# siddC/nbmf_mm

Hardware: AMD Instinct MI355X
Metric: MM-iterations/sec (higher is better)
Workload: dtype f64

## Files before the change

nbmf_mm_amd/csrc/nbmf_hip.hip:

```cpp

#include <hip/hip_runtime.h>
#include <hip/hip_ext.h>

#include <dlfcn.h>
#include <unistd.h>
#include <algorithm>
#include <atomic>
#include <cmath>
#include <cstdarg>
#include <cstdint>
#include <cstdio>
#include <cstdlib>
#include <cstring>
#include <chrono>
#include <condition_variable>
#include <map>
#include <mutex>
#include <string>
#include <type_traits>
#include <vector>

#include "../../include/nbmf_hip.h"

#ifndef NBMF_NO_MFMA
#define NBMF_NO_MFMA 0
#endif
#ifndef NBMF_HAZARD_SEED
#define NBMF_HAZARD_SEED 0
#endif

namespace {

thread_local std::string g_err;
std::atomic<long long> g_engine_persistent_served{0}, g_engine_persistent_aborted{0}, g_engine_persistent_declined{0},
    g_engine_launches_served{0};

int fail(int code, const char* fmt, ...) {
  char buf[1024];
  va_list ap;
  va_start(ap, fmt);
  vsnprintf(buf, sizeof buf, fmt, ap);
  va_end(ap);
  g_err = buf;
  if (code == NBMF_ERR_HIP) (void)hipGetLastError();
  return code;
}

#define HIPCHK(call)                                                                              \
  do {                                                                                            \
    hipError_t e_ = (call);                                                                       \
    if (e_ != hipSuccess)                                                                         \
      return fail(NBMF_ERR_HIP, "%s failed: %s (%s:%d)", #call, hipGetErrorString(e_), __FILE__,  \
                  __LINE__);                                                                      \
  } while (0)

inline int64_t round_up(int64_t x, int64_t a) { return (x + a - 1) / a * a; }

inline bool env_set(const char* name) { return getenv(name) != nullptr; }
template <typename T>
T env_int(const char* name, T dflt) {
  const char* e = getenv(name);
  return e ? (T)atoll(e) : dflt;
}
inline double env_double(const char* name, double dflt) {
  const char* e = getenv(name);
  return e ? atof(e) : dflt;
}

typedef double d4 __attribute__((ext_vector_type(4)));

enum { DATA_BIN = 0, DATA_F64 = 1, DATA_F64M = 2 };
enum { MODE_H = 0, MODE_W = 1, MODE_L = 2, MODE_T = 3 };

enum : unsigned { CB_YM = 1u, CB_ZOBS = 2u, CB_VALID = 4u };

constexpr int SLICE_K = 128;
constexpr int PAD = 128;
constexpr int WG_WAVES = 4;
constexpr size_t PASS_SLACK = 65536;
constexpr int STAGE_BYTES = 32768;

__device__ __forceinline__ double rcp_nr(double d) {
  double r = __builtin_amdgcn_rcp(d);
  const double e = __builtin_fma(-d, r, 1.0);
  const double p = __builtin_fma(e, e, e);
  return __builtin_fma(r, p, r);
}

__device__ __forceinline__ double mk_double(uint32_t lo, uint32_t hi) {
  return __hiloint2double((int)hi, (int)lo);
}

__device__ __forceinline__ double max0(double x) {
  double r;
  __asm__("v_max_f64 %0, %1, 0" : "=v"(r) : "v"(x));
  return r;
}
constexpr int LOG_TABLE_BYTES = 256 * 16;
template <int TB>
__device__ __forceinline__ double2 log_table_entry(int j) {
  const double c = 1.0 / (0.5 + ((double)j + 0.5) * (1.0 / (double)(2 << TB)));
  return double2{c, -log(c)};
}
__device__ __forceinline__ void log_table_fill(double2* tab ) {
  if (threadIdx.x < 256) tab[threadIdx.x] = log_table_entry<8>(threadIdx.x);
}
template <bool GUARD, int TB = 8, bool LDS_ABS = false, typename TAB = const double2*>
__device__ __forceinline__ double log_tab(double x, TAB tab, double c3 = 0.33333333333333331483, double c4 = -0.25) {
  static_assert(TB == 8 || TB == 10, "256 or 1024 entries");
  if (GUARD && __builtin_expect(!__builtin_amdgcn_class(x, 0x100), 0)) return log(x);
  const uint32_t hi = (uint32_t)__double2hiint(x);
  const double m = __builtin_amdgcn_frexp_mant(x);
  const uint32_t off = (hi >> (16 - TB)) & (((1u << TB) - 1u) << 4);
  double2 e;
  if constexpr (LDS_ABS) {
    typedef double d2raw __attribute__((ext_vector_type(2)));
    const d2raw v = *(const __attribute__((address_space(3))) d2raw*)(uintptr_t)(off + (uint32_t)tab);
    e = double2{v[0], v[1]};
  } else {
    e = *(const double2*)((const char*)tab + off);
  }
  const double r = __builtin_fma(m, e.x, -1.0);
  double p;
  if (TB == 8) {
    p = __builtin_fma(r, 0.2, -0.25);
    p = __builtin_fma(r, p, c3);
  } else {
    p = __builtin_fma(r, c4, c3);
  }
  p = __builtin_fma(r, p, -0.5);
  p = __builtin_fma(r, p, 1.0);
  const double k = (double)__builtin_amdgcn_frexp_exp(x);
  return __builtin_fma(r, p, __builtin_fma(k, 0.69314718055994530942, e.y));
}
__global__ __launch_bounds__(256) void log_table_kernel(double2* tab) {
  const int j = blockIdx.x * 256 + threadIdx.x;
  tab[j] = log_table_entry<10>(j);
}

__device__ __forceinline__ double log_of_product(double prod, int pexp) {
  const double m = __builtin_amdgcn_frexp_mant(prod);
  if (__builtin_expect(!(m >= 0.5 && m < 1.0), 0))
    return log(prod) + (double)pexp * 0.6931471805599453094;
  int e = __builtin_amdgcn_frexp_exp(prod) + pexp;
  const bool low = m < 0.70710678118654752440;
  const double m2 = low ? m + m : m;
  e -= low ? 1 : 0;
  const double s = (m2 - 1.0) * rcp_nr(m2 + 1.0);
  const double w = s * s;
  double p = __builtin_fma(w, 1.0 / 19.0, 1.0 / 17.0);
  p = __builtin_fma(w, p, 1.0 / 15.0);
  p = __builtin_fma(w, p, 1.0 / 13.0);
  p = __builtin_fma(w, p, 1.0 / 11.0);
  p = __builtin_fma(w, p, 1.0 / 9.0);
  p = __builtin_fma(w, p, 1.0 / 7.0);
  p = __builtin_fma(w, p, 0.2);
  p = __builtin_fma(w, p, 0.33333333333333331483);
  p = __builtin_fma(w, p, 1.0);
  return __builtin_fma(s + s, p, (double)e * 0.69314718055994530942);
}

typedef unsigned long long lanemask_t;
__device__ __forceinline__ void byte_set4(uint32_t x, lanemask_t (&m)[4]) {
  const uint32_t zero = 0u;
  __asm__("v_cmp_ne_u32_sdwa %0, %4, %5 src0_sel:BYTE_0 src1_sel:DWORD\n\t"
          "v_cmp_ne_u32_sdwa %1, %4, %5 src0_sel:BYTE_1 src1_sel:DWORD\n\t"
          "v_cmp_ne_u32_sdwa %2, %4, %5 src0_sel:BYTE_2 src1_sel:DWORD\n\t"
          "v_cmp_ne_u32_sdwa %3, %4, %5 src0_sel:BYTE_3 src1_sel:DWORD"
          : "=&s"(m[0]), "=&s"(m[1]), "=&s"(m[2]), "=&s"(m[3])
          : "v"(x), "v"(zero));
}
__device__ __forceinline__ void byte_set8(uint32_t x, uint32_t y, lanemask_t (&m)[4], lanemask_t (&n)[4]) {
  const uint32_t zero = 0u;
  __asm__("v_cmp_ne_u32_sdwa %0, %8, %10 src0_sel:BYTE_0 src1_sel:DWORD\n\t"
          "v_cmp_ne_u32_sdwa %1, %8, %10 src0_sel:BYTE_1 src1_sel:DWORD\n\t"
          "v_cmp_ne_u32_sdwa %2, %8, %10 src0_sel:BYTE_2 src1_sel:DWORD\n\t"
          "v_cmp_ne_u32_sdwa %3, %8, %10 src0_sel:BYTE_3 src1_sel:DWORD\n\t"
          "v_cmp_ne_u32_sdwa %4, %9, %10 src0_sel:BYTE_0 src1_sel:DWORD\n\t"
          "v_cmp_ne_u32_sdwa %5, %9, %10 src0_sel:BYTE_1 src1_sel:DWORD\n\t"
          "v_cmp_ne_u32_sdwa %6, %9, %10 src0_sel:BYTE_2 src1_sel:DWORD\n\t"
          "v_cmp_ne_u32_sdwa %7, %9, %10 src0_sel:BYTE_3 src1_sel:DWORD"
          : "=&s"(m[0]), "=&s"(m[1]), "=&s"(m[2]), "=&s"(m[3]), "=&s"(n[0]), "=&s"(n[1]), "=&s"(n[2]), "=&s"(n[3])
          : "v"(x), "v"(y), "v"(zero));
}
__device__ __forceinline__ lanemask_t byte_set(uint32_t x, int byte) {
  lanemask_t m;
  const uint32_t zero = 0u;
  switch (byte) {
    case 0: __asm__("v_cmp_ne_u32_sdwa %0, %1, %2 src0_sel:BYTE_0 src1_sel:DWORD" : "=s"(m) : "v"(x), "v"(zero)); break;
    case 1: __asm__("v_cmp_ne_u32_sdwa %0, %1, %2 src0_sel:BYTE_1 src1_sel:DWORD" : "=s"(m) : "v"(x), "v"(zero)); break;
    case 2: __asm__("v_cmp_ne_u32_sdwa %0, %1, %2 src0_sel:BYTE_2 src1_sel:DWORD" : "=s"(m) : "v"(x), "v"(zero)); break;
    default: __asm__("v_cmp_ne_u32_sdwa %0, %1, %2 src0_sel:BYTE_3 src1_sel:DWORD" : "=s"(m) : "v"(x), "v"(zero)); break;
  }
  return m;
}
__device__ __forceinline__ double sel64(lanemask_t m, double a, double b) { return __builtin_amdgcn_inverse_ballot_w64(m) ? a : b; }
__device__ __forceinline__ double sel64_or0(lanemask_t m, double a) { return __builtin_amdgcn_inverse_ballot_w64(m) ? a : 0.0; }
__device__ __forceinline__ double sel64_0or(lanemask_t m, double b) { return __builtin_amdgcn_inverse_ballot_w64(m) ? 0.0 : b; }
__device__ __forceinline__ double sel64_neg(lanemask_t m, double a, double b) {
  const uint32_t alo = (uint32_t)__double2loint(a), ahi = (uint32_t)__double2hiint(a);
  const uint32_t blo = (uint32_t)__double2loint(b), bhi = (uint32_t)__double2hiint(b);
  uint32_t lo, hi;
  __asm__("v_cndmask_b32_e64 %0, %1, %2, %3" : "=v"(lo) : "v"(blo), "v"(alo), "s"(m));
  __asm__("v_cndmask_b32_e64 %0, -%1, %2, %3" : "=v"(hi) : "v"(bhi), "v"(ahi), "s"(m));
  return mk_double(lo, hi);
}

__device__ __forceinline__ double wave_sum(double v) {
#pragma unroll
  for (int off = 32; off >= 1; off >>= 1) v += __shfl_xor(v, off, 64);
  return v;
}

#include "nbmf_pass_kernel.inc"
#include "nbmf_update_kernels.inc"
#include "nbmf_pack_kernels.inc"
#include "nbmf_peer_kernels.inc"
#include "nbmf_small_kernel.inc"
#include "nbmf_predict_kernels.inc"
#include "nbmf_score_kernels.inc"
#include "nbmf_hist_kernels.inc"
#include "nbmf_rank_kernels.inc"
#include "nbmf_eval_kernels.inc"
#include "nbmf_bits_kernels.inc"
#include "nbmf_theta_bits_kernels.inc"
#include "nbmf_holdout_kernels.inc"

}

struct nbmf_ctx {
  int device = 0;
  int cus = 256;
  hipStream_t stream = nullptr;
  int64_t m = 0, n = 0, mA = 0, nA = 0;
  int k = 0, KP = 0, KB = 0;
  int KS = 1;
  double* theta = nullptr;
  int data_kind = -1;
  int storage = NBMF_STORAGE_AUTO;
  void *dataA = nullptr, *dataB = nullptr, *maskA = nullptr, *maskB = nullptr;
  unsigned long long *bitsA = nullptr, *bitsB = nullptr;
  double n_obs = 0, n_obs_global = 0;
  double* rowcnt = nullptr;
  double *Wn = nullptr, *WT = nullptr, *WG = nullptr, *Hn = nullptr, *HT = nullptr, *HG = nullptr;
  bool have_factors = false;
  bool padB_ones = false;
  bool w_free = false;
  bool factors_in_range = false;
  int chunksH = 0, CH_H = 0, chunksW = 0, CH_W = 0;
  int *cstartH = nullptr, *cstartW = nullptr;
  double *slabH = nullptr, *slabW = nullptr, *Pbuf = nullptr, *lossbuf = nullptr, *prior = nullptr, *scal = nullptr;
  double* lossfin = nullptr;
  int n_prior_blocks = 0;
  int* flags = nullptr;
  double* losses_d = nullptr;
  int losses_cap = 0;
  double* stage = nullptr;
  size_t stage_bytes = 0;
  unsigned long long* stats = nullptr;
  double alpha = 1.2, beta = 1.2, eps = 1e-8;
  int projection = NBMF_PROJ_NORMALIZE;
  void* comm = nullptr;
  nbmf_host_allreduce_fn host_reduce = nullptr;
  void* host_reduce_user = nullptr;
  double* host_buf = nullptr;
  size_t host_buf_count = 0;
  int nranks = 1, rank = 0;
  int shard_axis = 0;
  double n_div_global = 0;
  double* Qbuf = nullptr;
  double* sbuf = nullptr;
  const double* ll_ptr = nullptr;
  int npanel = 1;
  int panels_wanted = 0;
  double peer_timeout_ms = 0;
  long long pc0[3] = {0, 0, 0};
  size_t pbase[2] = {0, 0};
  size_t ll_index = 0;
  int wsplit = 0;
  std::vector<int> bW_host;
  hipStream_t stream2 = nullptr;
  hipEvent_t evH = nullptr, evF = nullptr, ev1 = nullptr;
  const double* prior_src = nullptr;
  int n_prior_src = 0;
  double* arena = nullptr;
  unsigned long long* pflags = nullptr;
  size_t arena_doubles = 0;
  int arena_axis = -1;
  struct ArenaSlotRef { void* p = nullptr; } arena_slot;
  bool peer = false;
  PeerView pv{};
  std::vector<void*> peer_mapped;
  unsigned long long epoch = 0, hseq = 0;
  long long offHX = 0, offPR = 0, offSC = 0, x_doubles = 0;
  long long sl_c0 = 0, sl_wp = 0;
  long long psl_c0[2] = {0, 0}, psl_wp[2] = {0, 0};
  double *Pbuf_own = nullptr, *sbuf_own = nullptr, *Qbuf_own = nullptr;
  struct SmallWs {
    double *Wn = nullptr, *WT = nullptr, *WG = nullptr, *Hn = nullptr, *HT = nullptr, *HG = nullptr;
    double *snapW = nullptr, *snapH = nullptr, *ll_part = nullptr, *prior_part = nullptr;
    unsigned long long* sync = nullptr;
    int* result = nullptr;
    double *part_buf = nullptr, *part_ll = nullptr;
    unsigned long long* part_flag = nullptr;
    char* slab = nullptr;
    bool ready = false, disabled = false;
    int runs = 0, aborted = 0;
  } small;
  struct SmallBatchWs {
    char* slab = nullptr;
    double* table = nullptr;
    double* io = nullptr;
    int cap = 0, losses_cap = 0;
    size_t io_doubles = 0;
    int launches = 0, problems = 0;
  } small_batch;
  nbmf_progress_fn progress = nullptr;
  void* progress_user = nullptr;
  int progress_every = 0;
  struct EvalWs {
    int64_t count = 0;
    int every = 0, patience = 0;
    int *rows = nullptr, *cols = nullptr;
    unsigned char* x = nullptr;
    double *Wk = nullptr, *Hk = nullptr;
    double* partials = nullptr;
    double* eval_ll_d = nullptr;
    int ll_cap = 0;
    double *bestW = nullptr, *bestH = nullptr;
    bool have_best = false;
    std::vector<int> iters;
    std::vector<double> logliks;
    int best_iter = 0, stopped_early = 0;
    bool held_out = false;
  } eval;
  std::atomic<int> cancelled{0};
  bool timing = false;
  int timing_stride = 1;
  int timing_it = 0;
  std::vector<hipEvent_t> ev;
  std::vector<int> ev_kind;
  size_t ev_used = 0;
  double t_ms[2] = {0, 0};
  int t_n[2] = {0, 0};
};

namespace {

struct DevPool {
  std::mutex mu;
  struct Key {
    int device;
    size_t bytes;
    bool operator<(const Key& o) const { return device != o.device ? device < o.device : bytes < o.bytes; }
  };
  std::multimap<Key, void*> free_blocks;
  std::map<void*, Key> live;
  size_t held = 0;
} g_pool;

template <typename T>
hipError_t dmalloc(T** out, size_t bytes) {
  *out = nullptr;
  if (bytes == 0) bytes = 256;
  int dev = 0;
  hipGetDevice(&dev);
  const DevPool::Key key{dev, (bytes + 255) / 256 * 256};
  {
    std::lock_guard<std::mutex> lk(g_pool.mu);
    auto it = g_pool.free_blocks.find(key);
    if (it != g_pool.free_blocks.end()) {
      *out = (T*)it->second;
      g_pool.held -= key.bytes;
      g_pool.free_blocks.erase(it);
      g_pool.live[(void*)*out] = key;
      return hipSuccess;
    }
  }
  void* p = nullptr;
  hipError_t e = hipMalloc(&p, key.bytes);
  if (e != hipSuccess) {
    (void)hipGetLastError();
// ... 531 lines not shown
    }
  }
  c->ev_used = 0;
}

int all_reduce_inplace(nbmf_ctx* c, double* p, size_t count, hipStream_t st = nullptr) {
  if (c->comm) {
    NCCLCHK(g_rccl.AllReduce(p, p, count, kNcclFloat64, kNcclSum, c->comm, st ? st : c->stream));
  } else if (c->peer) {
    const long long off = p - c->arena;
    if (off < 0 || (size_t)off + count > c->arena_doubles) return fail(NBMF_ERR_STATE, "internal: peer exchange outside the arena");
    hipStream_t s = st ? st : c->stream;
    const unsigned long long e = ++c->epoch;
    const long long slice = ((long long)count + c->pv.nranks - 1) / c->pv.nranks;
    const unsigned grid = (unsigned)std::min<long long>(128, std::max<long long>(1, (slice + 1023) / 1024));
    static const bool fault = env_int("NBMF_PEER_FAULT", 0) != 0;
    if (!(fault && c->pv.nranks > 1 && c->pv.rank == c->pv.nranks - 1))
      hipLaunchKernelGGL(peer_reduce_kernel, dim3(grid), dim3(256), 0, s, c->pv, e, off, (long long)count, c->flags);
    HIPCHK(hipGetLastError());
    hipLaunchKernelGGL(peer_wait_kernel, dim3(1), dim3(64), 0, s, c->pv, e, c->flags);
    HIPCHK(hipGetLastError());
  } else if (c->host_reduce) {
    if (count > c->host_buf_count) return fail(NBMF_ERR_STATE, "internal: host exchange buffer too small");
    HIPCHK(hipMemcpyAsync(c->host_buf, p, count * sizeof(double), hipMemcpyDeviceToHost, c->stream));
    HIPCHK(hipStreamSynchronize(c->stream));
    if (c->host_reduce(c->host_reduce_user, c->host_buf, (int64_t)count) != 0)
      return fail(NBMF_ERR_COMM, "host all-reduce callback failed");
    HIPCHK(hipMemcpyAsync(p, c->host_buf, count * sizeof(double), hipMemcpyHostToDevice, c->stream));
  }
  return NBMF_OK;
}

inline bool is_sharded(const nbmf_ctx* c) { return c->comm || c->host_reduce || c->peer; }

inline const void* sweep_image(const nbmf_ctx* c, int image) {
  if (c->data_kind == DATA_BIN) return image == 0 ? (const void*)c->bitsA : (const void*)c->bitsB;
  return image == 0 ? c->dataA : c->dataB;
}

inline int wg_strips(const nbmf_ctx*) { return WG_WAVES; }

int tiny_a(const nbmf_ctx* c) {
  return c->eps < 1e-70 || !(c->eps >= 1e-12 && c->factors_in_range) || (c->data_kind == DATA_BIN && !(c->eps < 0x1p-22));
}
double pform_inv12(const nbmf_ctx* c) {
  if (c->data_kind != DATA_BIN || c->KS != 1 || tiny_a(c)) return 0.0;
  return 1.0 / ((1.0 + c->eps) + c->eps);
}

double ll_pad_of(const nbmf_ctx* c, int strict = 0) {
  if (strict) return 0.0;
  const double n_pad = (double)c->mA * (double)c->nA - (double)c->m * (double)c->n;
  return n_pad * log(1.0 + c->eps);
}

int enqueue_exchange_after_sweep(nbmf_ctx* c, const PassArgs& a, bool with_products, int strict) {
  const int n_loss = c->chunksH * (a.Cb / wg_strips(c));
  const double pad = ll_pad_of(c, strict);
  if (!is_sharded(c)) {
    c->ll_ptr = nullptr;
    return NBMF_OK;
  }
  if (c->shard_axis == 0 && with_products)
    return fail(NBMF_ERR_STATE, "internal: the row-split H-step exchange is driven by enqueue_iteration_rows");
  hipLaunchKernelGGL(ll_reduce_kernel, dim3(1), dim3(256), 0, c->stream, (const double*)c->lossbuf, n_loss, pad, c->sbuf,
                     c->flags);
  HIPCHK(hipGetLastError());
  size_t cnt = 1;
  if (c->shard_axis == 1) {
    hipLaunchKernelGGL(prior_reduce_kernel, dim3(1), dim3(256), 0, c->stream, (const double*)c->prior, c->n_prior_blocks,
                       c->sbuf + 1, c->flags);
    HIPCHK(hipGetLastError());
    cnt = 3;
  }
  if (int rc = all_reduce_inplace(c, c->sbuf, cnt)) return rc;
  c->ll_ptr = c->sbuf;
  return NBMF_OK;
}

PassArgs h_pass_args(nbmf_ctx* c) {
  PassArgs a{};
  a.data = sweep_image(c, 0);
  a.mask = c->maskA;
  a.LT = c->WT;
  a.LG = c->WG;
  a.RfT = c->HT;
  a.out1 = c->slabH;
  a.out2 = c->slabH + (size_t)c->chunksH * c->KP * c->nA;
  a.lossbuf = c->lossbuf;
  a.done = c->flags;
  a.Rb = (int)(c->mA / 16);
  a.Cb = (int)(c->nA / 16);
  a.chunk_start = c->cstartH;
  a.C_alloc = c->nA;
  a.eps = c->eps;
  a.tiny_eps = tiny_a(c);
  a.ksteps = (c->k + 3) / 4;
  a.kblocks = (c->k + 15) / 16;
  return a;
}
PassArgs w_pass_args(nbmf_ctx* c) {
  PassArgs a{};
  a.data = sweep_image(c, 1);
  a.mask = c->maskB;
  a.LT = c->HT;
  a.LG = c->HG;
  a.RfT = c->WT;
  a.out1 = c->slabW;
  a.out2 = nullptr;
  a.lossbuf = nullptr;
  a.done = c->flags;
  a.Rb = (int)(c->nA / 16);
  a.Cb = (int)(c->mA / 16);
  a.chunk_start = c->cstartW;
  a.C_alloc = c->mA;
  a.eps = c->eps;
  a.tiny_eps = tiny_a(c) || c->w_free;
  a.full = c->data_kind == DATA_BIN && c->n_obs == (double)c->m * (double)c->n && (c->nA == c->n || c->padB_ones);
  a.ksteps = (c->k + 3) / 4;
  a.kblocks = (c->k + 15) / 16;
  return a;
}

void at_slice(const nbmf_ctx* c, PassArgs& a, int image, int sl) {
  const size_t offW = (size_t)sl * SLICE_K * c->mA, offH = (size_t)sl * SLICE_K * c->nA;
  a.LT = image == 0 ? c->WT + offW : c->HT + offH;
  a.LG = image == 0 ? c->WG + offW : c->HG + offH;
  a.RfT = image == 0 ? c->HT + offH : c->WT + offW;
  const size_t slab_off = image == 0 ? (size_t)c->chunksH * offH : (size_t)c->chunksW * offW;
  if (a.out1) a.out1 += slab_off;
  if (a.out2) a.out2 += slab_off;
}

int enqueue_theta(nbmf_ctx* c, int image) {
  for (int sl = 0; sl < c->KS - 1; ++sl) {
    PassArgs a{};
    at_slice(c, a, image, sl);
    a.theta = c->theta;
    a.accum = sl > 0;
    a.done = c->flags;
    a.Rb = (int)((image == 0 ? c->mA : c->nA) / 16);
    a.Cb = (int)((image == 0 ? c->nA : c->mA) / 16);
    a.chunk_start = image == 0 ? c->cstartH : c->cstartW;
    a.C_alloc = image == 0 ? c->nA : c->mA;
    a.eps = c->eps;
    a.tiny_eps = c->eps < 1e-70;
    HIPCHK(launch_theta(a, image == 0 ? c->chunksH : c->chunksW, c->stream));
  }
  return NBMF_OK;
}

int enqueue_a_sweeps_sliced(nbmf_ctx* c, bool with_products, int strict, int clip) {
  if (int rc = enqueue_theta(c, 0)) return rc;
  const int last = c->KS - 1;
  for (int step = 0; step < (with_products ? c->KS : 1); ++step) {
    const int sl = step == 0 ? last : step - 1;
    PassArgs a = h_pass_args(c);
    at_slice(c, a, 0, sl);
    if (step != 0) a.lossbuf = nullptr;
    a.strict = strict;
    a.clip = clip;
    a.theta = c->theta;
    hipError_t e;
    if (with_products)
      e = step == 0 ? launch_pass_slice<MODE_H, 2>(c->data_kind, a, c->chunksH, c->stream)
                    : launch_pass_slice<MODE_H, 1>(c->data_kind, a, c->chunksH, c->stream);
    else
      e = launch_pass_slice<MODE_L, 2>(c->data_kind, a, c->chunksH, c->stream);
    HIPCHK(e);
  }
  return NBMF_OK;
}

__global__ void fill_u64_kernel(unsigned long long* p, size_t n, unsigned long long v) {
  const size_t i = (size_t)blockIdx.x * blockDim.x + threadIdx.x;
  if (i < n) p[i] = v;
}
int fill_ll_empty(nbmf_ctx* c) {
  const size_t n = (size_t)c->chunksH * (c->nA / 16 / WG_WAVES);
  if (!c->lossfin || !n) return NBMF_OK;
  hipLaunchKernelGGL(fill_u64_kernel, dim3((unsigned)((n + 255) / 256)), dim3(256), 0, c->stream, (unsigned long long*)c->lossfin, n, LL_EMPTY);
  HIPCHK(hipGetLastError());
  return NBMF_OK;
}
bool fin_fusable(const nbmf_ctx* c) { return !is_sharded(c) && c->KS == 1 && !env_set("NBMF_NO_FUSED_FINALIZE"); }
void fin_fill(nbmf_ctx* c, PassArgs& a, int t, double tol, int strict) {
  a.fin.on = 1;
  a.fin.wait_ticks = LL_WAIT_TICKS;
  const int fault = env_int("NBMF_PASSFIN_FAULT", 0);
  if (fault == 2) {
    a.fin.wait_ticks = 0;
  } else if (fault != 0) {
    a.fin.on = 2;
    a.fin.wait_ticks = 20000000ull;
  }
  a.lossbuf = c->lossfin;
  a.fin.t = t;
  a.fin.n_ll = c->chunksH * (int)(c->nA / 16 / wg_strips(c));
  a.fin.n_prior = c->n_prior_src;
  a.fin.ll_pad = ll_pad_of(c, strict);
  a.fin.am1 = c->alpha - 1.0;
  a.fin.bm1 = c->beta - 1.0;
  a.fin.n_obs = c->n_obs_global;
  a.fin.tol = tol;
  a.fin.prior = c->prior_src;
  a.fin.losses = c->losses_d;
  a.fin.scal = c->scal;
  a.fin.flags = c->flags;
}

int enqueue_a_sweep(nbmf_ctx* c, bool with_products, int strict = 0, int clip = 0, int fin_t = -1, double tol = 0.0) {
  PassArgs a = h_pass_args(c);
  if (c->KS > 1) {
    if (with_products) {
      EvScope ev(c, 0);
      if (int rc = enqueue_a_sweeps_sliced(c, true, 0, 0)) return rc;
    } else {
      if (int rc = enqueue_a_sweeps_sliced(c, false, strict, clip)) return rc;
    }
    return enqueue_exchange_after_sweep(c, a, with_products, strict);
  }
  a.strict = strict;
  a.clip = clip;
  if (!with_products) a.out2 = nullptr;
  if (fin_t >= 0) fin_fill(c, a, fin_t, tol, strict);
  if (with_products) {
    EvScope ev(c, 0, true, true);
    HIPCHK(launch_pass<MODE_H>(c->KB, c->data_kind, a, c->chunksH, c->stream));
  } else {
    HIPCHK(launch_pass<MODE_L>(c->KB, c->data_kind, a, c->chunksH, c->stream));
  }
  return enqueue_exchange_after_sweep(c, a, with_products, strict);
}

int enqueue_finalize(nbmf_ctx* c, int t, double tol, bool loglik_only = false, int strict = 0) {
  const bool sh = is_sharded(c) && c->ll_ptr;
  const double* ll_src = sh ? c->ll_ptr : c->lossbuf;
  const int n_ll = sh ? 1 : c->chunksH * (int)(c->nA / 16 / wg_strips(c));
  const double pad = sh ? 0.0 : ll_pad_of(c, strict);
  const bool prior_x = sh && c->shard_axis == 1;
  hipLaunchKernelGGL(finalize_kernel, dim3(1), dim3(256), 0, c->stream, ll_src, n_ll, pad,
                     prior_x ? (const double*)(c->sbuf + 1) : c->prior_src,
                     loglik_only ? 0 : (prior_x ? 1 : c->n_prior_src),
                     loglik_only ? 0.0 : c->alpha - 1.0, loglik_only ? 0.0 : c->beta - 1.0,
                     loglik_only ? -1.0 : c->n_obs_global, c->losses_d, t, tol, c->scal, c->flags);
  HIPCHK(hipGetLastError());
  return NBMF_OK;
}

void launch_h_update(nbmf_ctx* c, const double* src, int chunks, size_t chunk_stride, long long c0, long long wp, int sl,
                     double pform, hipStream_t st) {
  const int KSK = std::min(c->KP, SLICE_K);
  const size_t per = (size_t)KSK * c->nA;
  const long long blk0 = (long long)KSK * (sl * c->nA + c0) / 256;
  hipLaunchKernelGGL(h_update_kernel, dim3((unsigned)((long long)KSK * wp / 256)), dim3(256), 0, st, src,
                     src + (size_t)chunks * c->KP * wp, chunks, chunk_stride, wp, c0, c0, wp, c->Hn + sl * per, c->HT + sl * per,
                     c->HG + sl * per, c->prior + 2 * (size_t)blk0, std::min(KSK, c->k - sl * KSK), KSK, (long long)c->n,
                     (long long)c->nA, c->alpha - 1.0, c->beta - 1.0, c->eps, c->flags, pform);
}

void launch_reduce_h(nbmf_ctx* c, int sl, long long c0, long long wp, double* dst, long long dst_ld, double* ll_dst, hipStream_t st) {
  const int KSK = std::min(c->KP, SLICE_K);
  const size_t per = (size_t)KSK * c->nA;
  const int n_loss = c->chunksH * (int)(c->nA / 16 / wg_strips(c));
  hipLaunchKernelGGL(reduce_h_kernel, dim3((unsigned)(((long long)KSK * wp + 255) / 256)), dim3(256), 0, st,
                     (const double*)(c->slabH + (size_t)sl * c->chunksH * per),
                     (const double*)(c->slabH + (size_t)(c->KS + sl) * c->chunksH * per), c->chunksH, (long long)per,
                     (long long)c->nA, c0, wp, dst_ld, KSK, dst, dst + (size_t)c->KP * dst_ld, (const double*)c->lossbuf, n_loss,
                     ll_pad_of(c), ll_dst, c->flags, pform_inv12(c));
}

int enqueue_h_update_from(nbmf_ctx* c, const double* src, bool slabs, hipStream_t st) {
  const size_t per = (size_t)std::min(c->KP, SLICE_K) * c->nA;
  const int chunks = slabs ? c->chunksH : 1;
  for (int sl = 0; sl < c->KS; ++sl) {
    launch_h_update(c, src + (size_t)sl * chunks * per, chunks, slabs ? per : 0, 0, c->nA, sl, slabs ? pform_inv12(c) : 0.0, st);
    HIPCHK(hipGetLastError());
  }
  c->prior_src = c->prior;
  c->n_prior_src = c->n_prior_blocks;
  return NBMF_OK;
}
int enqueue_h_update(nbmf_ctx* c) { return enqueue_h_update_from(c, c->slabH, true, c->stream); }

template <int GROUPS>
int launch_w_update(nbmf_ctx* c, const double* q, int chunks, double n_div, int projection) {
  const size_t lds_bytes = sizeof(double) * ((size_t)c->KP + 2) * WU_COLS;
  if (lds_bytes > 65536)
    HIPCHK(hipFuncSetAttribute((const void*)w_update_kernel<GROUPS>, hipFuncAttributeMaxDynamicSharedMemorySize, (int)lds_bytes));
  hipLaunchKernelGGL(w_update_kernel<GROUPS>, dim3((unsigned)(c->mA / WU_COLS)), dim3(WU_COLS * GROUPS), lds_bytes, c->stream, q,
                     chunks, c->Wn, c->WT, c->WG, c->k, c->KP, std::min(c->KP, SLICE_K), (long long)c->m, (long long)c->mA, n_div,
                     c->rowcnt, projection, c->flags);
  HIPCHK(hipGetLastError());
  return NBMF_OK;
}
int enqueue_w_update(nbmf_ctx* c, const double* q, int chunks, double n_div, int projection) {
  return c->mA / WU_COLS <= 4LL * c->cus ? launch_w_update<32>(c, q, chunks, n_div, projection)
                                        : launch_w_update<8>(c, q, chunks, n_div, projection);
}

int enqueue_reduce_h_all(nbmf_ctx* c, double* dst, hipStream_t st) {
  const size_t per = (size_t)std::min(c->KP, SLICE_K) * c->nA, tot = (size_t)c->KP * c->nA;
  for (int sl = 0; sl < c->KS; ++sl) {
    launch_reduce_h(c, sl, 0, c->nA, dst + sl * per, c->nA, sl == 0 ? dst + 2 * tot : (double*)nullptr, st);
    HIPCHK(hipGetLastError());
  }
  return NBMF_OK;
}

int enqueue_w_step(nbmf_ctx* c, int projection);

int enqueue_iteration_rows_peer(nbmf_ctx* c, int it, double tol) {
  const size_t per = (size_t)c->KP * c->nA;
  {
    EvScope ev(c, 0, true, c->KS == 1);
    if (c->KS > 1) {
      if (int rc = enqueue_a_sweeps_sliced(c, true, 0, 0)) return rc;
    } else {
      HIPCHK(launch_pass<MODE_H>(c->KB, c->data_kind, h_pass_args(c), c->chunksH, c->stream));
    }
  }
  double* X = c->arena;
  const unsigned long long hs = ++c->hseq;
  const int slots_per_panel = PEER_H_WGS * c->pv.nranks;
  const long long offPR_now = c->offPR + (long long)(hs & 1) * 2 * 2 * PEER_H_WGS * PEER_MAX_RANKS;
  double* ll_slot = c->scal + 4;
  const long long offPR_prev = c->prior_src ? (long long)(c->prior_src - c->arena) : 0;
  const bool prev_in_arena = c->prior_src >= c->arena && c->prior_src < c->arena + c->arena_doubles;
  const int fin_t = (it > 0 && prev_in_arena) ? it - 1 : -1;
  auto exchange_panel = [&](int p, hipStream_t st, unsigned long long e) -> int {
    const long long c0 = c->pc0[p], wp = c->pc0[p + 1] - c0;
    if (c->KS > 1) {
      if (int rc = enqueue_reduce_h_all(c, X, st)) return rc;
    } else {
      launch_reduce_h(c, 0, c0, wp, X + c0, c->nA, p == 0 ? X + 2 * per : (double*)nullptr, st);
      HIPCHK(hipGetLastError());
    }
    PeerView pv = c->pv;
    pv.fbase = p * PF_SLOT;
    hipLaunchKernelGGL(peer_h_kernel, dim3(PEER_H_WGS), dim3(256), 0, st, pv, e, (long long)per, p == 0 ? (long long)(2 * per) : -1LL,
                       c->offHX, offPR_now, p * slots_per_panel + PEER_H_WGS * c->pv.rank, c->psl_c0[p], c->psl_wp[p],
                       (const double*)c->Hn, c->k, c->KP, (long long)c->n, (long long)c->nA, c->alpha - 1.0, c->beta - 1.0, c->eps,
                       ll_slot, c->flags, p == 0 ? fin_t : -1, offPR_prev, c->n_prior_src, c->n_obs_global, c->losses_d, tol,
                       c->scal, 0.0);
    HIPCHK(hipGetLastError());
    return NBMF_OK;
  };
  auto apply_panel = [&](int p, hipStream_t st, unsigned long long e) -> int {
    PeerView pv = c->pv;
    pv.fbase = p * PF_SLOT;
    hipLaunchKernelGGL(peer_h_apply_kernel, dim3(PEER_H_WGS), dim3(256), 0, st, pv, e, c->offHX, c->Hn, c->HT, c->HG, c->KP,
                       std::min(c->KP, SLICE_K), (long long)c->nA, c->pc0[p], c->pc0[p + 1] - c->pc0[p], c->flags);
    HIPCHK(hipGetLastError());
    return NBMF_OK;
  };
  const bool two = c->npanel == 2 && c->stream2;
  hipStream_t s0 = c->stream, s1 = two ? c->stream2 : c->stream;
  const unsigned long long e0 = ++c->epoch, e1 = two ? ++c->epoch : 0;
  if (int rc = exchange_panel(0, s0, e0)) return rc;
  c->ll_ptr = ll_slot;
  if (it > 0 && fin_t < 0)
    if (int rc = enqueue_finalize(c, it - 1, tol)) return rc;
  c->prior_src = c->arena + offPR_now;
  c->n_prior_src = c->npanel * slots_per_panel;
  if (!two) {
    if (int rc = apply_panel(0, s0, e0)) return rc;
    return enqueue_w_step(c, c->projection);
  }
  HIPCHK(hipEventRecord(c->evF, s0));
  HIPCHK(hipStreamWaitEvent(s1, c->evF, 0));
  if (int rc = exchange_panel(1, s1, e1)) return rc;
  if (int rc = apply_panel(1, s1, e1)) return rc;
  PassArgs w = w_pass_args(c);
  {
    PassArgs w1 = w;
    w1.chunk0 = c->wsplit;
    HIPCHK(launch_pass<MODE_W>(c->KB, c->data_kind, w1, c->chunksW - c->wsplit, s1));
    HIPCHK(hipEventRecord(c->ev1, s1));
  }
  if (int rc = apply_panel(0, s0, e0)) return rc;
  {
    EvScope ev(c, 1);
    HIPCHK(launch_pass<MODE_W>(c->KB, c->data_kind, w, c->wsplit, s0));
    HIPCHK(hipStreamWaitEvent(s0, c->ev1, 0));
  }
  return enqueue_w_update(c, c->slabW, c->chunksW, (double)c->n, c->projection);
}

int enqueue_iteration_rows(nbmf_ctx* c, int it, double tol) {
  if (c->peer) return enqueue_iteration_rows_peer(c, it, tol);
  if (c->KS > 1) {
    const size_t tot = (size_t)c->KP * c->nA;
    {
      EvScope ev(c, 0);
      if (int rc = enqueue_a_sweeps_sliced(c, true, 0, 0)) return rc;
    }
    if (int rc = enqueue_reduce_h_all(c, c->Pbuf, c->stream)) return rc;
    if (int rc = all_reduce_inplace(c, c->Pbuf, 2 * tot + 1)) return rc;
    c->ll_ptr = c->Pbuf + 2 * tot;
    if (it > 0)
      if (int rc = enqueue_finalize(c, it - 1, tol)) return rc;
    if (int rc = enqueue_h_update_from(c, c->Pbuf, false, c->stream)) return rc;
    return enqueue_w_step(c, c->projection);
  }
  hipStream_t s0 = c->stream;
  const bool two_streams = c->npanel == 2 && c->comm && c->stream2;
  hipStream_t s1 = two_streams ? c->stream2 : s0;
  {
    EvScope ev(c, 0, true, true);
    HIPCHK(launch_pass<MODE_H>(c->KB, c->data_kind, h_pass_args(c), c->chunksH, s0));
  }
  if (two_streams) HIPCHK(hipEventRecord(c->evH, s0));
  auto reduce_panel = [&](int p, hipStream_t st) -> int {
    const long long c0 = c->pc0[p], wp = c->pc0[p + 1] - c0;
    double* d1 = c->Pbuf + c->pbase[p];
    launch_reduce_h(c, 0, c0, wp, d1, wp, p == 0 ? c->Pbuf + c->ll_index : (double*)nullptr, st);
    HIPCHK(hipGetLastError());
    return all_reduce_inplace(c, d1, 2 * (size_t)c->KP * wp + (p == 0 ? 1 : 0), st);
  };
  auto update_panel = [&](int p, hipStream_t st) -> int {
    const long long c0 = c->pc0[p], wp = c->pc0[p + 1] - c0;
    launch_h_update(c, c->Pbuf + c->pbase[p], 1, 0, c0, wp, 0, 0.0, st);
    HIPCHK(hipGetLastError());
    c->prior_src = c->prior;
    c->n_prior_src = c->n_prior_blocks;
    return NBMF_OK;
  };
  if (int rc = reduce_panel(0, s0)) return rc;
  c->ll_ptr = c->Pbuf + c->ll_index;
  if (it > 0)
    if (int rc = enqueue_finalize(c, it - 1, tol)) return rc;
  if (two_streams) HIPCHK(hipEventRecord(c->evF, s0));
  PassArgs w = w_pass_args(c);
  const int first = c->npanel == 2 ? c->wsplit : c->chunksW;
  if (c->npanel == 2) {
    if (two_streams) HIPCHK(hipStreamWaitEvent(s1, c->evH, 0));
    if (int rc = reduce_panel(1, s1)) return rc;
    if (two_streams) HIPCHK(hipStreamWaitEvent(s1, c->evF, 0));
    if (int rc = update_panel(1, s1)) return rc;
    if (two_streams) {
      PassArgs w1 = w;
      w1.chunk0 = first;
      HIPCHK(launch_pass<MODE_W>(c->KB, c->data_kind, w1, c->chunksW - first, s1));
      HIPCHK(hipEventRecord(c->ev1, s1));
    }
  }
  if (int rc = update_panel(0, s0)) return rc;
  {
    EvScope ev(c, 1);
    HIPCHK(launch_pass<MODE_W>(c->KB, c->data_kind, w, first, s0));
    if (c->npanel == 2) {
      if (two_streams) {
        HIPCHK(hipStreamWaitEvent(s0, c->ev1, 0));
      } else {
        w.chunk0 = first;
        HIPCHK(launch_pass<MODE_W>(c->KB, c->data_kind, w, c->chunksW - first, s0));
      }
    }
  }
  return enqueue_w_update(c, c->slabW, c->chunksW, (double)c->n, c->projection);
}

int enqueue_w_step(nbmf_ctx* c, int projection) {
  if (c->KS > 1) {
    {
      EvScope ev(c, 1);
      if (int rc = enqueue_theta(c, 1)) return rc;
      for (int step = 0; step < c->KS; ++step) {
        const int sl = step == 0 ? c->KS - 1 : step - 1;
        PassArgs w = w_pass_args(c);
        at_slice(c, w, 1, sl);
        w.theta = c->theta;
        if (step == 0)
          HIPCHK((launch_pass_slice<MODE_W, 2>(c->data_kind, w, c->chunksW, c->stream)));
        else
          HIPCHK((launch_pass_slice<MODE_W, 1>(c->data_kind, w, c->chunksW, c->stream)));
      }
    }
    if (is_sharded(c) && c->shard_axis == 1) {
      const long long per = (long long)SLICE_K * c->mA;
      for (int sl = 0; sl < c->KS; ++sl) {
        hipLaunchKernelGGL(reduce_w_kernel, dim3((unsigned)((per + 255) / 256)), dim3(256), 0, c->stream,
                           (const double*)(c->slabW + (size_t)sl * c->chunksW * per), c->Qbuf + sl * per, c->chunksW, per, c->flags);
        HIPCHK(hipGetLastError());
      }
      if (int rc = all_reduce_inplace(c, c->Qbuf, (size_t)c->KP * c->mA)) return rc;
      return enqueue_w_update(c, c->Qbuf, 1, c->n_div_global, projection);
    }
    return enqueue_w_update(c, c->slabW, c->chunksW, (double)c->n, projection);
  }
  PassArgs a = w_pass_args(c);
  {
    EvScope ev(c, 1, true, true);
    HIPCHK(launch_pass<MODE_W>(c->KB, c->data_kind, a, c->chunksW, c->stream));
  }
  const double* q = c->slabW;
  int chunks = c->chunksW;
  double n_div = (double)c->n;
  if (is_sharded(c) && c->shard_axis == 1) {
    const long long per = (long long)c->KP * c->mA;
    hipLaunchKernelGGL(reduce_w_kernel, dim3((unsigned)((per + 255) / 256)), dim3(256), 0, c->stream,
                       (const double*)c->slabW, c->Qbuf, c->chunksW, per, c->flags);
    HIPCHK(hipGetLastError());
    if (int rc = all_reduce_inplace(c, c->Qbuf, (size_t)per)) return rc;
    q = c->Qbuf;
    chunks = 1;
    n_div = c->n_div_global;
  }
  return enqueue_w_update(c, q, chunks, n_div, projection);
}

__global__ void expand_factor_kernel(const double* __restrict__ Fn, double* __restrict__ FT, double* __restrict__ FG, int KP,
                                     int KS, long long lenA) {
  const long long idx = (long long)blockIdx.x * blockDim.x + threadIdx.x;
  if (idx >= (long long)KP * lenA) return;
  const long long k = idx / lenA, x = idx % lenA;
  FT[t_index(k, x, KS, lenA)] = Fn[idx];
  FG[g_index(k, x, KS, lenA)] = Fn[idx];
}

void launch_set_factor(const nbmf_ctx* c, bool h, const double* src, double* Fn, double* FT, double* FG) {
  const long long len = h ? c->n : c->m, lenA = h ? c->nA : c->mA, tot = (long long)c->KP * lenA;
  hipLaunchKernelGGL(set_factor_kernel, dim3((unsigned)((tot + 255) / 256)), dim3(256), 0, c->stream, src, Fn, FT, FG, c->k, c->KP,
                     std::min(c->KP, SLICE_K), len, lenA);
}
void launch_get_factor(const nbmf_ctx* c, bool h, const double* Fn, double* dst) {
  const long long len = h ? c->n : c->m, lenA = h ? c->nA : c->mA, tot = (long long)c->k * len;
  hipLaunchKernelGGL(get_factor_kernel, dim3((unsigned)((tot + 255) / 256)), dim3(256), 0, c->stream, Fn, dst, c->k, len, lenA);
}
void launch_expand_factor(const nbmf_ctx* c, bool h) {
  const long long lenA = h ? c->nA : c->mA, tot = (long long)c->KP * lenA;
  hipLaunchKernelGGL(expand_factor_kernel, dim3((unsigned)((tot + 255) / 256)), dim3(256), 0, c->stream, (const double*)(h ? c->Hn : c->Wn),
                     h ? c->HT : c->WT, h ? c->HG : c->WG, c->KP, c->KP, lenA);
}

constexpr int SMALL_MAX_WGS = 256;
int small_parts(const nbmf_ctx* c, long long sweep_blocks, long long strips) {
  const int NW = sm_waves(c->KB);
  long long pp = (sweep_blocks + 2 * NW - 1) / (2 * NW);
  pp = std::min<long long>(pp, std::min<long long>(8, std::min(c->cus, SMALL_MAX_WGS) / std::max<long long>(1, strips)));
  return (int)std::max<long long>(1, pp);
}

bool small_eligible(const nbmf_ctx* c, int cus) {
  if (is_sharded(c) || c->KS != 1 || c->KB > 2 || c->timing) return false;
  cus = std::min(cus, SMALL_MAX_WGS);
  if (env_int("NBMF_PERSISTENT", 1) == 0) return false;
  const long long Rbe = (c->m + 15) / 16, Cbe = (c->n + 15) / 16;
  const long long max_tiles = env_int("NBMF_SMALL_TILES", 32768LL);
  const int NW = sm_waves(c->KB), PH = small_parts(c, Rbe, Cbe), PW = small_parts(c, Cbe, Rbe);
  const bool fits = (Rbe + (long long)PH * NW - 1) / ((long long)PH * NW) <= SM_TPW && (Cbe + (long long)PW * NW - 1) / ((long long)PW * NW) <= SM_TPW;
  if (!(fits && Cbe <= 128 && Cbe * PH <= cus && Rbe * PW <= cus && Rbe * Cbe <= max_tiles)) return false;
  if (c->small.disabled) {
    g_engine_persistent_declined.fetch_add(1, std::memory_order_relaxed);
    return false;
  }
  return true;
}

struct SmallAdmission {
  std::mutex mu;
  std::condition_variable cv;
  int busy[64] = {0};
} g_small_admission;

struct SmallReservation {
  int device, n;
  SmallReservation(int device_, int n_, int capacity) : device(device_ & 63), n(n_) {
    std::unique_lock<std::mutex> lk(g_small_admission.mu);
    g_small_admission.cv.wait(lk, [&] { return g_small_admission.busy[device] + n <= capacity || g_small_admission.busy[device] == 0; });
    g_small_admission.busy[device] += n;
  }
  ~SmallReservation() {
    {
      std::lock_guard<std::mutex> lk(g_small_admission.mu);
      g_small_admission.busy[device] -= n;
    }
    g_small_admission.cv.notify_all();
  }
};

int small_prepare(nbmf_ctx* c) {
  if (c->small.ready) return NBMF_OK;
  const size_t fw = (size_t)c->KP * c->mA * sizeof(double), fh = (size_t)c->KP * c->nA * sizeof(double);
  const size_t g_max = 16 * SM_TPW;
  const size_t sync_b = round_up(sizeof(unsigned long long) * (SMALL_MAX_WGS + 8), 256), ll_b = round_up(sizeof(double) * 2 * g_max, 256),
               pr_b = sizeof(double) * 3 * g_max * 8 * 2, res_b = 256;
  const size_t g_all = SMALL_MAX_WGS;
  const size_t pb_b = sizeof(double) * g_all * 2 * 16 * (size_t)c->KP, pl_b = sizeof(double) * g_all, pf_b = sizeof(unsigned long long) * g_all;
  const size_t total = 4 * fw + 4 * fh + sync_b + ll_b + pr_b + res_b + pb_b + pl_b + pf_b;
  char* base = nullptr;
  HIPCHK(dmalloc(&base, total));
  HIPCHK(hipMemsetAsync(base, 0, total, c->stream));
  c->small.slab = base;
  char* p = base;
  for (double** q : {&c->small.Wn, &c->small.WT, &c->small.WG, &c->small.snapW}) {
    *q = (double*)p;
    p += fw;
  }
  for (double** q : {&c->small.Hn, &c->small.HT, &c->small.HG, &c->small.snapH}) {
    *q = (double*)p;
    p += fh;
  }
  c->small.sync = (unsigned long long*)p;
  p += sync_b;
  c->small.ll_part = (double*)p;
  p += ll_b;
  c->small.prior_part = (double*)p;
  p += pr_b;
  c->small.result = (int*)p;
  p += res_b;
  c->small.part_buf = (double*)p;
  p += pb_b;
  c->small.part_ll = (double*)p;
  p += pl_b;
  c->small.part_flag = (unsigned long long*)p;
  c->small.ready = true;
  return NBMF_OK;
}

struct SmallKernel {
  const void* f = nullptr;
  int NW = 0;
  size_t lds_bytes = 0;
};
template <int KB, bool SPLIT, bool BATCH>
const void* small_ptr(int data_kind) {
  switch (data_kind) {
    case DATA_BIN: return (const void*)small_fit_kernel<KB, DATA_BIN, SPLIT, BATCH>;
    case DATA_F64: return (const void*)small_fit_kernel<KB, DATA_F64, SPLIT, BATCH>;
    case DATA_F64M: return (const void*)small_fit_kernel<KB, DATA_F64M, SPLIT, BATCH>;
  }
  return nullptr;
}
template <int KB>
const void* small_ptr(int data_kind, bool split, bool batch) {
  if (batch) return split ? small_ptr<KB, true, true>(data_kind) : small_ptr<KB, false, true>(data_kind);
  return split ? small_ptr<KB, true, false>(data_kind) : small_ptr<KB, false, false>(data_kind);
}
int small_kernel(const nbmf_ctx* c, bool split, bool batch, SmallKernel* k) {
  k->f = c->KB == 1 ? small_ptr<1>(c->data_kind, split, batch) : small_ptr<2>(c->data_kind, split, batch);
  if (!k->f) return NBMF_OK;
  k->NW = sm_waves(c->KB);
  k->lds_bytes = sizeof(double) * ((size_t)k->NW * 2 * c->KB * 4 * 64 + k->NW * 16 + 64 + 2 * c->KP * 16) + LOG_TABLE_BYTES;
  HIPCHK(hipFuncSetAttribute(k->f, hipFuncAttributeMaxDynamicSharedMemorySize, (int)k->lds_bytes));
  return NBMF_OK;
}

void small_common_args(const nbmf_ctx* c, int max_iter, double tol, SmallArgs* out) {
  SmallArgs& a = *out;
  a.dataA = c->dataA;
  a.maskA = c->maskA;
  a.dataB = c->dataB;
  a.maskB = c->maskB;
  a.rowcnt = c->rowcnt;
  a.m = c->m; a.n = c->n; a.mA = c->mA; a.nA = c->nA;
  a.K = c->k;
  a.RbA = (int)(c->mA / 16);
  a.CbA = (int)(c->nA / 16);
  a.Rbe = (int)((c->m + 15) / 16);
  a.Cbe = (int)((c->n + 15) / 16);
  a.PH = small_parts(c, a.Rbe, a.Cbe);
  a.PW = small_parts(c, a.Cbe, a.Rbe);
  if (const char* e = getenv("NBMF_SMALL_PARTS")) {
    int x = 0, y = 0;
    const int cap = std::min(c->cus, SMALL_MAX_WGS);
    if (sscanf(e, "%d,%d", &x, &y) == 2 && x >= a.PH && y >= a.PW && x <= 8 && y <= 8 && a.Cbe * x <= cap && a.Rbe * y <= cap) {
      a.PH = x;
      a.PW = y;
    }
  }
  a.G = std::max(a.Cbe * a.PH, a.Rbe * a.PW);
  a.max_iter = max_iter;
  a.projection = c->projection;
  a.tiny_eps = c->eps < 1e-70;
  a.tol = tol;
  a.eps = c->eps;
  a.am1 = c->alpha - 1.0;
  a.bm1 = c->beta - 1.0;
  a.n_obs = c->n_obs_global;
  a.n_div = (double)c->n;
  a.ll_pad = (256.0 * a.Rbe * a.Cbe - (double)c->m * (double)c->n) * log(1.0 + c->eps);
  a.timeout = (unsigned long long)(std::max(1.0, env_double("NBMF_SMALL_TIMEOUT_MS", 2000.0)) * 1e5);
  a.fenced = env_int("NBMF_SMALL_FENCED", 0) != 0;
}

int loss_by_launches(nbmf_ctx* c, double* out);
bool small_guard_on() {
  static const bool on = env_int("NBMF_SMALL_GUARD", 1) != 0;
  return on;
}
int small_guard(nbmf_ctx* c, double reported, bool* ok) {
  double chk = 0.0;
  if (int rc = loss_by_launches(c, &chk)) return rc;
  if (env_set("NBMF_SMALL_GUARD_FAULT")) chk += 1e-6 * std::max(std::fabs(chk), 1.0);
  *ok = (std::isnan(chk) && std::isnan(reported)) || chk == reported ||
        std::fabs(chk - reported) <= 1e-12 * std::max({std::fabs(chk), std::fabs(reported), 1.0});
  if (!*ok && env_set("NBMF_DEBUG"))
    fprintf(stderr, "[nbmf] single-launch guard: reported loss %.17g, recomputed %.17g: redone by the launches\n", reported, chk);
  return NBMF_OK;
}

void small_give_up(nbmf_ctx* c, bool disable, const char* fmt = nullptr, ...) {
  ++c->small.aborted;
  g_engine_persistent_aborted.fetch_add(1, std::memory_order_relaxed);
  if (disable) c->small.disabled = true;
  if (fmt && env_set("NBMF_DEBUG")) {
    va_list ap;
    va_start(ap, fmt);
    vfprintf(stderr, fmt, ap);
    va_end(ap);
  }
}

struct DrainGuard {
  hipStream_t st;
  ~DrainGuard() { hipStreamSynchronize(st); }
};

int run_small(nbmf_ctx* c, int max_iter, double tol, double* losses, int* n_iter, bool* handled) {
  *handled = false;
  if (!small_eligible(c, c->cus)) return NBMF_OK;
  if (int rc = small_prepare(c)) return rc;
  auto& w = c->small;
  const size_t fw = (size_t)c->KP * c->mA * sizeof(double), fh = (size_t)c->KP * c->nA * sizeof(double);
  SmallArgs a{};
  small_common_args(c, max_iter, tol, &a);
  a.Wn[0] = w.Wn; a.WT[0] = w.WT; a.WG[0] = w.WG; a.Hn[0] = w.Hn; a.HT[0] = w.HT; a.HG[0] = w.HG;
  a.Wn[1] = c->Wn; a.WT[1] = c->WT; a.WG[1] = c->WG; a.Hn[1] = c->Hn; a.HT[1] = c->HT; a.HG[1] = c->HG;
  a.sync = w.sync;
  a.ll_part = w.ll_part;
  a.prior_part = w.prior_part;
  a.losses = c->losses_d;
  a.result = w.result;
  a.part_buf = w.part_buf;
  a.part_ll = w.part_ll;
  a.part_flag = w.part_flag;
  SmallKernel k;
  if (int rc = small_kernel(c, a.PH > 1 || a.PW > 1, false, &k)) return rc;
  if (!k.f) return NBMF_OK;
  HIPCHK(hipMemcpyAsync(w.snapW, c->Wn, fw, hipMemcpyDeviceToDevice, c->stream));
  HIPCHK(hipMemcpyAsync(w.snapH, c->Hn, fh, hipMemcpyDeviceToDevice, c->stream));
  HIPCHK(hipMemsetAsync(w.sync, 0, sizeof(unsigned long long) * (a.G + 1), c->stream));
  HIPCHK(hipMemsetAsync(w.part_flag, 0, sizeof(unsigned long long) * SMALL_MAX_WGS, c->stream));
  HIPCHK(hipMemsetAsync(w.result, 0, sizeof(int) * 4, c->stream));
  if (env_set("NBMF_SMALL_FORCE_ABORT")) {
    const unsigned long long one = 1;
    HIPCHK(hipMemcpyAsync(w.sync + a.G, &one, sizeof one, hipMemcpyHostToDevice, c->stream));
  }
  unsigned long long *dbg = nullptr, *place = nullptr;
  struct DiagGuard {
    unsigned long long *&a, *&b;
    ~DiagGuard() {
      if (a) dfree(a);
      if (b) dfree(b);
    }
  } diag_guard{dbg, place};
  if (env_set("NBMF_SMALL_DEBUG")) {
    HIPCHK(dmalloc(&dbg, sizeof(unsigned long long) * 64 * 16));
    HIPCHK(hipMemsetAsync(dbg, 0, sizeof(unsigned long long) * 64 * 16, c->stream));
    a.dbg = dbg;
  }
  if (env_set("NBMF_SMALL_PLACEMENT")) {
    HIPCHK(dmalloc(&place, sizeof(unsigned long long) * a.G));
    a.place = place;
  }
  void* params[] = {&a};
  SmallReservation cus_held(c->device, a.G, std::min(c->cus, SMALL_MAX_WGS));
  DrainGuard drain_guard{c->stream};
  HIPCHK(hipLaunchKernel(k.f, dim3(a.G), dim3(64 * k.NW), params, k.lds_bytes, c->stream));
  if (place) {
    std::vector<unsigned long long> h(a.G);
    HIPCHK(hipMemcpyAsync(h.data(), place, sizeof(unsigned long long) * a.G, hipMemcpyDeviceToHost, c->stream));
    HIPCHK(hipStreamSynchronize(c->stream));
    fprintf(stderr, "[nbmf] placement (xcd.se.cu):");
    for (int i = 0; i < a.G; ++i)
      fprintf(stderr, " %u.%u.%u", (unsigned)(h[i] >> 32) & 15u, (unsigned)(h[i] >> 13) & 7u, (unsigned)(h[i] >> 8) & 15u);
    fprintf(stderr, "\n");
  }
  if (dbg) {
    unsigned long long h[64 * 16];
    HIPCHK(hipMemcpyAsync(h, dbg, sizeof h, hipMemcpyDeviceToHost, c->stream));
    HIPCHK(hipStreamSynchronize(c->stream));
    double acc[8] = {0}, fine[7] = {0};
    int cnt = 0;
    for (int t = 8; t < 63 && t + 1 < max_iter; ++t) {
      if (!h[t * 16 + 7] || !h[(t + 1) * 16]) continue;
      for (int p = 0; p < 7; ++p) acc[p] += (double)(h[t * 16 + p + 1] - h[t * 16 + p]) * 0.01;
      acc[7] += (double)(h[(t + 1) * 16] - h[t * 16 + 7]) * 0.01;
      fine[0] += (double)(h[t * 16 + 8] - h[t * 16 + 3]) * 0.01;
      fine[1] += (double)(h[t * 16 + 9] - h[t * 16 + 8]) * 0.01;
      fine[2] += (double)(h[t * 16 + 10] - h[t * 16 + 9]) * 0.01;
      fine[3] += (double)(h[t * 16 + 11] - h[t * 16 + 10]) * 0.01;
      fine[4] += (double)(h[t * 16 + 12] - h[t * 16 + 1]) * 0.01;
      fine[5] += (double)(h[t * 16 + 13] - h[t * 16 + 12]) * 0.01;
      fine[6] += (double)(h[t * 16 + 2] - h[t * 16 + 13]) * 0.01;
      ++cnt;
    }
    if (cnt)
      fprintf(stderr, "[nbmf]   W tiles of wave 0 in detail: issue %.2f | operands land %.2f | tile A %.2f | tile B %.2f;  H reduce+update: "
                      "wait for all waves %.2f | update %.2f | prior sums %.2f\n", fine[0] / cnt, fine[1] / cnt, fine[2] / cnt, fine[3] / cnt,
              fine[4] / cnt, fine[5] / cnt, fine[6] / cnt);
    if (h[15] && h[63 * 16 + 15] > h[15])
      fprintf(stderr, "[nbmf]   on the device from the first instruction to the last: %.3f ms\n", (double)(h[63 * 16 + 15] - h[15]) * 1e-5);
    if (h[8 * 16 + 14] && h[62 * 16 + 14] && h[62 * 16] > h[8 * 16])
      fprintf(stderr, "[nbmf]   shader clock over iterations 8..62: %.0f MHz (%llu cycles in %.2f us)\n",
              (double)(h[62 * 16 + 14] - h[8 * 16 + 14]) / ((double)(h[62 * 16] - h[8 * 16]) * 0.01),
              (unsigned long long)(h[62 * 16 + 14] - h[8 * 16 + 14]), (double)(h[62 * 16] - h[8 * 16]) * 0.01);
    if (cnt)
      fprintf(stderr, "[nbmf] persistent fit, workgroup 0, us per iteration part (mean of %d): H tiles %.2f | H reduce+update %.2f | barrier %.2f | "
                      "W tiles %.2f | W reduce+update %.2f | loss %.2f | barrier %.2f | loop %.2f\n", cnt, acc[0] / cnt, acc[1] / cnt,
              acc[2] / cnt, acc[3] / cnt, acc[4] / cnt, acc[5] / cnt, acc[6] / cnt, acc[7] / cnt);
  }
  int res[4] = {0, 0, 0, 0};
  unsigned long long abort_word = 0;
  HIPCHK(hipMemcpyAsync(res, w.result, sizeof res, hipMemcpyDeviceToHost, c->stream));
  HIPCHK(hipMemcpyAsync(&abort_word, w.sync + a.G, sizeof abort_word, hipMemcpyDeviceToHost, c->stream));
  HIPCHK(stream_wait_spin(c->stream));
  ++w.runs;
  auto back_to_entry = [&]() -> int {
    HIPCHK(hipMemcpyAsync(c->Wn, w.snapW, fw, hipMemcpyDeviceToDevice, c->stream));
    HIPCHK(hipMemcpyAsync(c->Hn, w.snapH, fh, hipMemcpyDeviceToDevice, c->stream));
    launch_expand_factor(c, false);
    HIPCHK(hipGetLastError());
    launch_expand_factor(c, true);
    HIPCHK(hipGetLastError());
    HIPCHK(hipStreamSynchronize(c->stream));
    return NBMF_OK;
  };
  if (res[2] != 0 || abort_word != 0 || res[0] < 1 || res[0] > max_iter) {
    small_give_up(c, true, "[nbmf] persistent fit abandoned (status %d, abort word %llu): five-kernel path\n", res[2], abort_word);
    return back_to_entry();
  }
  if (res[1] == 0) {
    HIPCHK(hipMemcpyAsync(c->Wn, w.Wn, fw, hipMemcpyDeviceToDevice, c->stream));
    HIPCHK(hipMemcpyAsync(c->WT, w.WT, fw, hipMemcpyDeviceToDevice, c->stream));
    HIPCHK(hipMemcpyAsync(c->WG, w.WG, fw, hipMemcpyDeviceToDevice, c->stream));
    HIPCHK(hipMemcpyAsync(c->Hn, w.Hn, fh, hipMemcpyDeviceToDevice, c->stream));
    HIPCHK(hipMemcpyAsync(c->HT, w.HT, fh, hipMemcpyDeviceToDevice, c->stream));
    HIPCHK(hipMemcpyAsync(c->HG, w.HG, fh, hipMemcpyDeviceToDevice, c->stream));
  }
  HIPCHK(hipMemcpyAsync(losses, c->losses_d, sizeof(double) * (size_t)res[0], hipMemcpyDeviceToHost, c->stream));
  HIPCHK(stream_wait_spin(c->stream));
  if (small_guard_on()) {
    bool ok = true;
    if (int rc = small_guard(c, losses[res[0] - 1], &ok)) return rc;
    if (!ok) {
      small_give_up(c, false);
      return back_to_entry();
    }
  }
  *n_iter = res[0];
  *handled = true;
  g_engine_persistent_served.fetch_add(1, std::memory_order_relaxed);
  if (c->progress && c->progress_every > 0)
    for (int first = 0; first < res[0]; first += c->progress_every)
      c->progress(c->progress_user, first, std::min(c->progress_every, res[0] - first), losses + first);
  return NBMF_OK;
}

struct SmallBatchLayout {
  size_t fw, fh, factors, ll_b, pr_b, pb_b, pl_b, sync_b, res_b, pf_b, control, off_partials, off_control, off_losses, stride;
};
SmallBatchLayout small_batch_layout(const nbmf_ctx* c, int losses_cap) {
  SmallBatchLayout L{};
  const size_t g_max = 16 * SM_TPW;
  L.fw = (size_t)c->KP * c->mA * sizeof(double);
  L.fh = (size_t)c->KP * c->nA * sizeof(double);
  L.factors = 2 * (3 * L.fw + 3 * L.fh);
  L.ll_b = round_up(sizeof(double) * 2 * g_max, 256);
  L.pr_b = sizeof(double) * 3 * g_max * 8 * 2;
  L.pb_b = sizeof(double) * SMALL_MAX_WGS * 2 * 16 * (size_t)c->KP;
  L.pl_b = round_up(sizeof(double) * SMALL_MAX_WGS, 256);
  L.sync_b = round_up(sizeof(unsigned long long) * (SMALL_MAX_WGS + 8), 256);
  L.res_b = 256;
  L.pf_b = round_up(sizeof(unsigned long long) * SMALL_MAX_WGS, 256);
  L.control = L.sync_b + L.res_b + L.pf_b;
  L.off_partials = L.factors;
  L.off_control = L.off_partials + L.ll_b + L.pr_b + L.pb_b + L.pl_b;
  L.off_losses = L.off_control + L.control;
  L.stride = round_up(L.off_losses + sizeof(double) * (size_t)losses_cap, 256);
  return L;
}

int small_batch_prepare(nbmf_ctx* c, int cap, int max_iter) {
  auto& b = c->small_batch;
  if (cap > b.cap || max_iter > b.losses_cap) {
    cap = std::max(cap, b.cap);
    const int lcap = std::max(max_iter, b.losses_cap);
    for (void* p : {(void*)b.slab, (void*)b.table, (void*)b.io})
      if (p) HIPCHK(dfree(p));
    b.slab = nullptr;
    b.table = nullptr;
    b.io = nullptr;
    b.cap = b.losses_cap = 0;
    const SmallBatchLayout L = small_batch_layout(c, lcap);
    const size_t total = (size_t)cap * L.stride;
    HIPCHK(dmalloc(&b.slab, total));
    HIPCHK(hipMemsetAsync(b.slab, 0, total, c->stream));
    HIPCHK(dmalloc(&b.table, sizeof(double) * 2 * (size_t)cap));
    b.io_doubles = (size_t)cap * ((size_t)c->k * c->m + (size_t)c->k * c->n);
    HIPCHK(dmalloc(&b.io, sizeof(double) * b.io_doubles));
    b.cap = cap;
    b.losses_cap = lcap;
  }
  return NBMF_OK;
}

int run_small_batch(nbmf_ctx* c, int nprob, const double* alpha, const double* beta, const double* W0, const double* H0,
                    int max_iter, double tol, double* losses, int* n_iter, double* W_out, double* H_out, bool* handled) {
  *handled = false;
  if (!small_eligible(c, c->cus)) return NBMF_OK;
  SmallArgs a{};
  small_common_args(c, max_iter, tol, &a);
  const int cap_cus = std::min(c->cus, SMALL_MAX_WGS);
  int B = std::max(1, cap_cus / a.G);
  B = std::max(1, std::min(B, env_int("NBMF_BATCH_MAX", B)));
  B = std::min(B, nprob);
  if (int rc = small_batch_prepare(c, B, max_iter)) return rc;
  auto& b = c->small_batch;
  const SmallBatchLayout L = small_batch_layout(c, b.losses_cap);
  SmallKernel k;
  if (int rc = small_kernel(c, a.PH > 1 || a.PW > 1, true, &k)) return rc;
  if (!k.f) return NBMF_OK;
  const size_t wsz = (size_t)c->k * c->m, hsz = (size_t)c->k * c->n;
  {
    char* q = b.slab;
    for (int par = 0; par < 2; ++par) {
      a.Wn[par] = (double*)q; q += L.fw;
      a.WT[par] = (double*)q; q += L.fw;
      a.WG[par] = (double*)q; q += L.fw;
      a.Hn[par] = (double*)q; q += L.fh;
      a.HT[par] = (double*)q; q += L.fh;
      a.HG[par] = (double*)q; q += L.fh;
    }
    a.ll_part = (double*)q; q += L.ll_b;
    a.prior_part = (double*)q; q += L.pr_b;
    a.part_buf = (double*)q; q += L.pb_b;
    a.part_ll = (double*)q;
    char* ctl = b.slab + L.off_control;
    a.sync = (unsigned long long*)ctl;
    a.result = (int*)(ctl + L.sync_b);
    a.part_flag = (unsigned long long*)(ctl + L.sync_b + L.res_b);
    a.losses = (double*)(b.slab + L.off_losses);
    a.prob_stride = L.stride;
    a.am1s = (const double*)b.table;
    a.bm1s = (const double*)b.table + b.cap;
  }
  auto prob = [&](auto* p0, int p) { return (decltype(p0))((char*)p0 + (size_t)p * L.stride); };
  std::vector<int> res((size_t)B * 4);
  std::vector<unsigned long long> abort_words((size_t)B);
  std::vector<double> priors((size_t)2 * b.cap);
  for (int p0 = 0; p0 < nprob; p0 += B) {
    const int Bc = std::min(B, nprob - p0);
    for (int p = 0; p < Bc; ++p) {
      priors[(size_t)p] = alpha[p0 + p] - 1.0;
      priors[(size_t)b.cap + p] = beta[p0 + p] - 1.0;
    }
    HIPCHK(hipMemcpyAsync(b.table, priors.data(), sizeof(double) * priors.size(), hipMemcpyHostToDevice, c->stream));
    HIPCHK(hipMemcpyAsync(b.io, W0 + (size_t)p0 * wsz, sizeof(double) * wsz * Bc, hipMemcpyHostToDevice, c->stream));
    HIPCHK(hipMemcpyAsync(b.io + wsz * Bc, H0 + (size_t)p0 * hsz, sizeof(double) * hsz * Bc, hipMemcpyHostToDevice, c->stream));
    for (int p = 0; p < Bc; ++p) {
      launch_set_factor(c, false, b.io + wsz * p, prob(a.Wn[1], p), prob(a.WT[1], p), prob(a.WG[1], p));
      launch_set_factor(c, true, b.io + wsz * Bc + hsz * p, prob(a.Hn[1], p), prob(a.HT[1], p), prob(a.HG[1], p));
    }
    HIPCHK(hipGetLastError());
    HIPCHK(hipMemset2DAsync(b.slab + L.off_control, L.stride, 0, L.control, (size_t)Bc, c->stream));
    if (env_set("NBMF_SMALL_FORCE_ABORT")) {
      const unsigned long long one = 1;
      HIPCHK(hipMemcpyAsync(a.sync + a.G, &one, sizeof one, hipMemcpyHostToDevice, c->stream));
    }
    void* params[] = {&a};
    {
      SmallReservation cus_held(c->device, a.G * Bc, cap_cus);
      DrainGuard drain_guard{c->stream};
      HIPCHK(hipLaunchKernel(k.f, dim3(a.G, Bc), dim3(64 * k.NW), params, k.lds_bytes, c->stream));
      HIPCHK(hipMemcpy2DAsync(res.data(), sizeof(int) * 4, a.result, L.stride, sizeof(int) * 4, (size_t)Bc, hipMemcpyDeviceToHost, c->stream));
      HIPCHK(hipMemcpy2DAsync(abort_words.data(), sizeof(unsigned long long), a.sync + a.G, L.stride, sizeof(unsigned long long), (size_t)Bc,
                              hipMemcpyDeviceToHost, c->stream));
      HIPCHK(stream_wait_spin(c->stream));
    }
    ++b.launches;
    b.problems += Bc;
    for (int p = 0; p < Bc; ++p)
      if (res[(size_t)p * 4 + 2] != 0 || abort_words[(size_t)p] != 0 || res[(size_t)p * 4] < 1 || res[(size_t)p * 4] > max_iter) {
        small_give_up(c, true, "[nbmf] batched persistent fit abandoned (problem %d): one by one\n", p0 + p);
        return NBMF_OK;
      }
    if (small_guard_on()) {
      const int ps = (int)(b.launches % Bc), par = res[(size_t)ps * 4 + 1], nit = res[(size_t)ps * 4];
      double reported = 0.0;
      HIPCHK(hipMemcpyAsync(&reported, (const char*)a.losses + (size_t)ps * L.stride + sizeof(double) * (size_t)(nit - 1), sizeof(double),
                            hipMemcpyDeviceToHost, c->stream));
      HIPCHK(hipStreamSynchronize(c->stream));
      struct Lend {
        nbmf_ctx* c;
        double *Wn, *WT, *WG, *Hn, *HT, *HG, alpha, beta;
        ~Lend() {
          c->Wn = Wn; c->WT = WT; c->WG = WG; c->Hn = Hn; c->HT = HT; c->HG = HG;
          c->alpha = alpha; c->beta = beta;
        }
      } lend{c, c->Wn, c->WT, c->WG, c->Hn, c->HT, c->HG, c->alpha, c->beta};
      c->Wn = prob(a.Wn[par], ps); c->WT = prob(a.WT[par], ps); c->WG = prob(a.WG[par], ps);
      c->Hn = prob(a.Hn[par], ps); c->HT = prob(a.HT[par], ps); c->HG = prob(a.HG[par], ps);
      c->alpha = alpha[p0 + ps];
      c->beta = beta[p0 + ps];
      bool ok = true;
      if (int rc = small_guard(c, reported, &ok)) return rc;
      if (!ok) {
        small_give_up(c, false);
        return NBMF_OK;
      }
    }
    for (int p = 0; p < Bc; ++p) {
      const int par = res[(size_t)p * 4 + 1];
      launch_get_factor(c, false, prob(a.Wn[par], p), b.io + wsz * p);
      launch_get_factor(c, true, prob(a.Hn[par], p), b.io + wsz * Bc + hsz * p);
      n_iter[p0 + p] = res[(size_t)p * 4];
    }
    HIPCHK(hipGetLastError());
    HIPCHK(hipMemcpy2DAsync(losses + (size_t)p0 * max_iter, sizeof(double) * (size_t)max_iter, a.losses, L.stride, sizeof(double) * (size_t)max_iter,
                            (size_t)Bc, hipMemcpyDeviceToHost, c->stream));
    HIPCHK(hipMemcpyAsync(W_out + (size_t)p0 * wsz, b.io, sizeof(double) * wsz * Bc, hipMemcpyDeviceToHost, c->stream));
    HIPCHK(hipMemcpyAsync(H_out + (size_t)p0 * hsz, b.io + wsz * Bc, sizeof(double) * hsz * Bc, hipMemcpyDeviceToHost, c->stream));
    HIPCHK(stream_wait_spin(c->stream));
  }
  c->small.runs += nprob;
  g_engine_persistent_served.fetch_add(nprob, std::memory_order_relaxed);
  *handled = true;
  return NBMF_OK;
}

int ensure_losses(nbmf_ctx* c, int cap) {
  if (cap <= c->losses_cap) return NBMF_OK;
  if (c->losses_d) HIPCHK(dfree(c->losses_d));
  c->losses_d = nullptr;
  HIPCHK(dmalloc(&c->losses_d, sizeof(double) * (size_t)cap));
  c->losses_cap = cap;
  return NBMF_OK;
}

int ensure_eval_slots(nbmf_ctx* c, int cap) {
  auto& ev = c->eval;
  if (cap <= ev.ll_cap) return NBMF_OK;
  if (ev.eval_ll_d) HIPCHK(dfree(ev.eval_ll_d));
  ev.eval_ll_d = nullptr;
  ev.ll_cap = 0;
  HIPCHK(dmalloc(&ev.eval_ll_d, sizeof(double) * (size_t)cap));
  ev.ll_cap = cap;
  return NBMF_OK;
}

int enqueue_eval(nbmf_ctx* c, int slot) {
  auto& ev = c->eval;
  for (const bool h : {false, true}) {
    const long long len = h ? c->n : c->m, lenA = h ? c->nA : c->mA;
    hipLaunchKernelGGL(k_major_kernel, dim3((unsigned)((len + PT_TILE - 1) / PT_TILE), (unsigned)((c->k + PT_TILE - 1) / PT_TILE)),
                       dim3(PT_TILE * 8), 0, c->stream, (const double*)(h ? c->Hn : c->Wn), h ? ev.Hk : ev.Wk, c->k, len, lenA);
    HIPCHK(hipGetLastError());
  }
  const long long nparts = (ev.count + EV_PAIRS - 1) / EV_PAIRS;
  hipLaunchKernelGGL(eval_pairs_kernel, dim3((unsigned)nparts), dim3(EV_THREADS), 0, c->stream, (const double*)ev.Wk,
                     (const double*)ev.Hk, c->k, (const int*)ev.rows, (const int*)ev.cols, (const unsigned char*)ev.x,
                     (long long)ev.count, c->eps, ev.partials);
  HIPCHK(hipGetLastError());
  hipLaunchKernelGGL(eval_fold_kernel, dim3(1), dim3(EV_FOLD), 0, c->stream, (const double*)ev.partials, nparts,
                     ev.eval_ll_d + slot);
  HIPCHK(hipGetLastError());
  return NBMF_OK;
}

void eval_release(nbmf_ctx* c) {
  auto& ev = c->eval;
  void* ptrs[] = {ev.rows, ev.cols, ev.x, ev.Wk, ev.Hk, ev.partials};
  for (void* p : ptrs)
    if (p) dfree(p);
  ev.rows = ev.cols = nullptr;
  ev.x = nullptr;
  ev.Wk = ev.Hk = ev.partials = nullptr;
  ev.count = 0;
}

int mark_pad_rows_b(nbmf_ctx* c) {
  c->padB_ones = false;
  if (c->data_kind != DATA_BIN || !c->bitsB || c->n_obs != (double)c->m * (double)c->n || c->nA == c->n) return NBMF_OK;
  const long long RbB = c->nA / 16, CbB = c->mA / 16, nblk = RbB - (c->n >> 4);
  const long long threads = CbB * nblk * 4;
// ... 232 lines not shown
}

hipError_t launch_hist_panel(nbmf_ctx* c, const RowPanels& pl, long long p0, long long pn, int bins, const unsigned char* x_d,
                             const unsigned char* m_d, int copies, unsigned long long* total_d) {
  const size_t lds = sizeof(unsigned int) * PR_WAVES * (2 * (size_t)bins + 2);
  hipLaunchKernelGGL(theta_hist_kernel, pl.grid(p0, pn), dim3(PR_WAVES * 64), lds, c->stream, (const double*)c->Wn,
                     (const double*)c->Hn, c->k, (long long)c->mA, (long long)c->nA, (long long)c->n, p0, pn, pl.ldp, bins, x_d, m_d,
                     copies, total_d);
  return hipGetLastError();
}

}

extern "C" {

int nbmf_abi_version(void) { return 4; }
#ifndef NBMF_SRC_HASH
#define NBMF_SRC_HASH "unstamped"
#endif
const char* nbmf_source_hash(void) { return NBMF_SRC_HASH; }

const char* nbmf_last_error(void) { return g_err.c_str(); }

int nbmf_device_bus_id(int device, char* buf, int len) {
  if (!buf || len < 16) return fail(NBMF_ERR_ARG, "buffer of at least 16 bytes expected");
  int n = 0;
  if (hipGetDeviceCount(&n) != hipSuccess || device < 0 || device >= n) return fail(NBMF_ERR_HIP, "no HIP device %d", device);
  HIPCHK(hipDeviceGetPCIBusId(buf, len, device));
  return NBMF_OK;
}

int nbmf_device_count(int* count) {
  if (!count) return fail(NBMF_ERR_ARG, "count is NULL");
  int n = 0;
  hipError_t e = hipGetDeviceCount(&n);
  if (e != hipSuccess) {
    *count = 0;
    return fail(NBMF_ERR_HIP, "hipGetDeviceCount: %s", hipGetErrorString(e));
  }
  *count = n;
  return NBMF_OK;
}

int nbmf_create(int64_t m, int64_t n, int k, int device, nbmf_ctx** out) {
  if (!out) return fail(NBMF_ERR_ARG, "out is NULL");
  *out = nullptr;
  if (m < 1 || n < 1) return fail(NBMF_ERR_ARG, "m and n must be >= 1 (got %lld x %lld)", (long long)m, (long long)n);
  if (k < 1 || k > NBMF_MAX_K) return fail(NBMF_ERR_ARG, "n_components must be in [1, %d] (got %d)", NBMF_MAX_K, k);
  int ndev = 0;
  hipError_t e = hipGetDeviceCount(&ndev);
  if (e != hipSuccess || ndev < 1)
    return fail(NBMF_ERR_HIP, "no HIP device available (%s): libnbmf_hip needs an MI355X (gfx950)",
                e == hipSuccess ? "device count 0" : hipGetErrorString(e));
  if (device < 0 || device >= ndev) return fail(NBMF_ERR_ARG, "device %d out of range (have %d)", device, ndev);
  HIPCHK(hipSetDevice(device));
  DevInfo info;
  HIPCHK(device_info(device, &info));
  if (!info.gfx950) return fail(NBMF_ERR_HIP, "device %d is %s; this library is built for gfx950 only", device, info.arch);

  nbmf_ctx* c = new nbmf_ctx();
  c->cus = info.cus;
  struct CtxGuard {
    nbmf_ctx* p;
    ~CtxGuard() {
      if (p) nbmf_destroy(p);
    }
  } ctx_guard{c};
  c->device = device;
  c->m = m;
  c->n = n;
  c->k = k;
  c->mA = round_up(m, PAD);
  c->nA = round_up(n, PAD);
  c->KB = k <= 16 ? 1 : k <= 32 ? 2 : k <= 64 ? 4 : 8;
  c->KS = (k + SLICE_K - 1) / SLICE_K;
  c->KP = c->KS > 1 ? SLICE_K * c->KS : 16 * c->KB;
  if (c->KS > 1) HIPCHK(dmalloc(&c->theta, sizeof(double) * (size_t)c->mA * c->nA));
  HIPCHK(stream_acquire(device, &c->stream));
  HIPCHK(log_table_build(device, c->stream));

  const size_t fw = (size_t)c->KP * c->mA * sizeof(double), fh = (size_t)c->KP * c->nA * sizeof(double);
  HIPCHK(dmalloc(&c->Wn, fw));
  HIPCHK(dmalloc(&c->WT, fw + PASS_SLACK));
  HIPCHK(dmalloc(&c->WG, fw + PASS_SLACK));
  HIPCHK(dmalloc(&c->Hn, fh));
  HIPCHK(dmalloc(&c->HT, fh + PASS_SLACK));
  HIPCHK(dmalloc(&c->HG, fh + PASS_SLACK));
  HIPCHK(dmalloc(&c->Pbuf, 2 * fh + 64));
  c->n_prior_blocks = (int)(((size_t)c->KP * c->nA + 255) / 256);
  HIPCHK(dmalloc(&c->prior, sizeof(double) * 2 * (size_t)c->n_prior_blocks));
  c->prior_src = c->prior;
  c->n_prior_src = c->n_prior_blocks;
  HIPCHK(dmalloc(&c->scal, sizeof(double) * 8));
  HIPCHK(dmalloc(&c->sbuf, sizeof(double) * 8));
  HIPCHK(dmalloc(&c->flags, sizeof(int) * 8));
  HIPCHK(dmalloc(&c->stats, sizeof(unsigned long long) * 8));
  HIPCHK(dmalloc(&c->rowcnt, sizeof(double) * (size_t)c->mA));
  HIPCHK(hipMemset(c->flags, 0, sizeof(int) * 8));
  HIPCHK(hipMemset(c->scal, 0, sizeof(double) * 8));
  c->stage_bytes = (fw > fh ? fw : fh);
  HIPCHK(dmalloc(&c->stage, c->stage_bytes));
  ctx_guard.p = nullptr;
  *out = c;
  return NBMF_OK;
}

int nbmf_destroy(nbmf_ctx* c) {
  if (!c) return NBMF_OK;
  hipSetDevice(c->device);
  if (c->stream) hipStreamSynchronize(c->stream);
  comm_release(c);
  if (c->host_buf) hipHostFree(c->host_buf);
  arena_release((ArenaSlot*)c->arena_slot.p);
  void* ptrs[] = {c->dataA, c->dataB, c->maskA, c->maskB, c->rowcnt, c->Wn, c->WT, c->WG, c->Hn, c->HT, c->HG,
                  c->slabH, c->slabW, c->Pbuf, c->lossbuf, c->lossfin, c->prior, c->scal, c->flags, c->losses_d, c->stage, c->stats,
                  c->sbuf, c->Qbuf, c->cstartH, c->cstartW, c->theta, c->small.slab, c->small_batch.slab, c->small_batch.table,
                  c->small_batch.io, c->bitsA, c->bitsB, c->eval.rows, c->eval.cols, c->eval.x, c->eval.Wk, c->eval.Hk,
                  c->eval.partials, c->eval.eval_ll_d, c->eval.bestW, c->eval.bestH};
  for (void* p : ptrs)
    if (p) dfree(p);
  for (hipEvent_t e : c->ev) hipEventDestroy(e);
  for (hipEvent_t e : {c->evH, c->evF, c->ev1})
    if (e) hipEventDestroy(e);
  if (c->stream2) {
    hipStreamSynchronize(c->stream2);
    hipStreamDestroy(c->stream2);
  }
  if (c->stream) stream_release(c->device, c->stream);
  delete c;
  return NBMF_OK;
}

int nbmf_set_hyper(nbmf_ctx* c, double alpha, double beta, double eps, int projection) {
  if (!c) return fail(NBMF_ERR_ARG, "null context");
  if (projection != NBMF_PROJ_NORMALIZE && projection != NBMF_PROJ_DUCHI)
    return fail(NBMF_ERR_ARG, "unknown projection %d", projection);
  if (!(eps >= 2.2250738585072014e-308 && eps <= 1.7976931348623157e308))
    return fail(NBMF_ERR_ARG, "eps must be a positive normal number");
  c->alpha = alpha;
  c->beta = beta;
  c->eps = eps;
  c->projection = projection;
  return NBMF_OK;
}

int nbmf_upload(nbmf_ctx* c, const double* x, int64_t ldx, int transposed, const void* mask, int mask_kind,
                int64_t ldmask, int* out_flags) {
  return nbmf_upload_v(c, x, NBMF_DATA_F64, ldx, transposed, mask, mask_kind, ldmask, out_flags);
}

int nbmf_upload_v(nbmf_ctx* c, const void* xv, int x_kind, int64_t ldx, int transposed, const void* mask, int mask_kind,
                  int64_t ldmask, int* out_flags) {
  if (!c || !xv) return fail(NBMF_ERR_ARG, "null context or data");
  if (x_kind != NBMF_DATA_F64 && x_kind != NBMF_DATA_U8 && x_kind != NBMF_DATA_F32 && x_kind != NBMF_DATA_BITS)
    return fail(NBMF_ERR_ARG, "x_kind must be NBMF_DATA_F64, NBMF_DATA_U8, NBMF_DATA_F32 or NBMF_DATA_BITS");
  if (mask && (mask_kind < NBMF_MASK_NONE || mask_kind > NBMF_MASK_BITS)) return fail(NBMF_ERR_ARG, "unknown mask_kind %d", mask_kind);
  const bool xbits = x_kind == NBMF_DATA_BITS, mbits = mask && mask_kind == NBMF_MASK_BITS;
  const size_t xsz = x_kind == NBMF_DATA_U8 || xbits ? 1 : (x_kind == NBMF_DATA_F32 ? 4 : 8);
  const double* x = (const double*)xv;
  const unsigned char* xb = (const unsigned char*)xv;
  if (mask_kind != NBMF_MASK_NONE && !mask) return fail(NBMF_ERR_ARG, "mask_kind set but mask is NULL");
  if (!mask) mask_kind = NBMF_MASK_NONE;
  if (is_sharded(c)) return fail(NBMF_ERR_STATE, "upload before attaching a communicator");
  if (int rc = set_device(c)) return rc;
  const int64_t U = transposed ? c->n : c->m, V = transposed ? c->m : c->n;
  if (xbits && ldx < packed_ld(V))
    return fail(NBMF_ERR_ARG, "ldx %lld is less than ceil(n / 8) = %lld", (long long)ldx, (long long)packed_ld(V));
  if (mbits && ldmask < packed_ld(V))
    return fail(NBMF_ERR_ARG, "ldmask %lld is less than ceil(n / 8) = %lld", (long long)ldmask, (long long)packed_ld(V));
  if ((!xbits && ldx < V) || (mask && !mbits && ldmask < V)) return fail(NBMF_ERR_ARG, "leading dimension smaller than the row length");

  bool guess_bin = c->storage == NBMF_STORAGE_AUTO && env_int("NBMF_FORCE_F64", 0) == 0;
  bool guess_mask_bin = true;
  {
    const int64_t rows = U < 8 ? U : 8;
    for (int64_t u = 0; u < rows && (guess_bin || guess_mask_bin); ++u) {
      const int64_t uu = (U - 1) * u / (rows > 1 ? rows - 1 : 1);
      for (int64_t v = 0; v < V && v < 4096; ++v) {
        const double xe = xbits ? 0.0
                          : x_kind == NBMF_DATA_U8 ? (double)xb[uu * ldx + v]
                          : x_kind == NBMF_DATA_F32 ? (double)((const float*)xv)[uu * ldx + v] : x[uu * ldx + v];
        if (xe != 0.0 && xe != 1.0) guess_bin = false;
        if (mask_kind == NBMF_MASK_F64) {
          const double mk = ((const double*)mask)[uu * ldmask + v];
          if (mk != 0.0 && mk != 1.0) guess_mask_bin = false;
        }
      }
    }
    if (!guess_mask_bin) guess_bin = false;
  }

  const bool up_trace = env_set("NBMF_UPLOAD_TRACE");
  auto up_t0 = std::chrono::steady_clock::now();
  double up_copy = 0, up_pack = 0;
  auto up_mark = [&](const char* what) {
    if (!up_trace) return;
    hipStreamSynchronize(c->stream);
// ... 207 lines not shown
    *p = nullptr;
  }
  c->data_kind = -1;
  c->eval.held_out = false;
  const long long RbA = c->mA / 16, RbB = c->nA / 16;
  const size_t tiles = (size_t)RbA * RbB;
  HIPCHK(dmalloc(&c->dataA, tiles * 256 + PASS_SLACK));
  HIPCHK(dmalloc(&c->dataB, tiles * 256 + PASS_SLACK));
  HIPCHK(hipMemsetAsync(c->stats, 0, sizeof(unsigned long long) * 8, c->stream));
  const long long dwords = (long long)tiles * 64;
  hipLaunchKernelGGL(csr_fill_kernel, dim3((unsigned)((dwords + 255) / 256)), dim3(256), 0, c->stream, (uint32_t*)c->dataA,
                     (uint32_t*)c->dataB, RbA, RbB, (long long)c->m, (long long)c->n,
                     masked ? (unsigned)CB_VALID : (unsigned)(CB_VALID | CB_ZOBS));
  HIPCHK(hipGetLastError());
  struct DevBuf {
    void* p = nullptr;
    ~DevBuf() {
      if (p) dfree(p);
    }
  } d_ptr, d_idx;
  HIPCHK(dmalloc(&d_ptr.p, sizeof(int64_t) * (size_t)(U + 1)));
  const int64_t piece = std::max<int64_t>(1, env_int<int64_t>("NBMF_CSR_PIECE", 64ll << 20));
  HIPCHK(dmalloc(&d_idx.p, sizeof(int32_t) * (size_t)std::max<int64_t>(1, std::min<int64_t>(piece, std::max(nnz, mask_nnz)))));
  for (int what = masked ? 0 : 1; what <= 1; ++what) {
    const int64_t* ip = what == 0 ? mask_indptr : indptr;
    const int32_t* ix = what == 0 ? mask_indices : indices;
    const int64_t cnt = what == 0 ? mask_nnz : nnz;
    HIPCHK(hipMemcpyAsync(d_ptr.p, ip, sizeof(int64_t) * (size_t)(U + 1), hipMemcpyHostToDevice, c->stream));
    for (int64_t e0 = 0; e0 < cnt; e0 += piece) {
      const int64_t ne = std::min(piece, cnt - e0);
      HIPCHK(hipMemcpyAsync(d_idx.p, ix + e0, sizeof(int32_t) * (size_t)ne, hipMemcpyHostToDevice, c->stream));
      hipLaunchKernelGGL(csr_scatter_kernel, dim3((unsigned)((ne + 255) / 256)), dim3(256), 0, c->stream,
                         (const long long*)d_ptr.p, (const int*)d_idx.p - e0, (long long)U, (long long)V, (long long)e0,
                         (long long)(e0 + ne), transposed, what, (unsigned char*)c->dataA, (unsigned char*)c->dataB, RbA, RbB, c->stats);
      HIPCHK(hipGetLastError());
      HIPCHK(hipStreamSynchronize(c->stream));
    }
  }
  if (masked) {
    hipLaunchKernelGGL(count_observed_kernel, dim3(1024), dim3(256), 0, c->stream, (const uint32_t*)c->dataA, dwords, c->stats);
    HIPCHK(hipGetLastError());
  }
  unsigned long long st[2] = {0, 0};
  HIPCHK(hipMemcpyAsync(st, c->stats, sizeof st, hipMemcpyDeviceToHost, c->stream));
  HIPCHK(hipStreamSynchronize(c->stream));
  if (st[1] != 0) return fail(NBMF_ERR_ARG, "%llu column indices outside [0, %lld)", st[1], (long long)V);
  c->data_kind = DATA_BIN;
  if (int rc2 = setup_workspaces(c)) return rc2;
  c->n_obs = masked ? (double)st[0] : (double)c->m * (double)c->n;
  if (int rc2 = mark_pad_rows_b(c)) return rc2;
  c->n_obs_global = c->n_obs;
  hipLaunchKernelGGL(rowcount_kernel, dim3((unsigned)((c->m + 255) / 256)), dim3(256), 0, c->stream, c->dataB, c->maskB,
                     c->data_kind, (long long)(c->nA / 16), (long long)c->m, (long long)c->n, c->rowcnt);
  HIPCHK(hipGetLastError());
  HIPCHK(hipStreamSynchronize(c->stream));
  if (out_flags) *out_flags = NBMF_FLAG_BINARY_PATH;
  return NBMF_OK;
}

int nbmf_get_n_obs(nbmf_ctx* c, double* n_obs) {
  if (!c || !n_obs) return fail(NBMF_ERR_ARG, "null argument");
  if (c->data_kind < 0) return fail(NBMF_ERR_STATE, "nbmf_upload has not been called");
  *n_obs = c->n_obs;
  return NBMF_OK;
}

int check_factor_range(nbmf_ctx* c) {
  HIPCHK(hipMemsetAsync(c->flags + 5, 0, sizeof(int), c->stream));
  const long long tot = std::max((long long)c->mA, (long long)c->KP * c->nA);
  hipLaunchKernelGGL(factor_range_kernel, dim3((unsigned)((tot + 255) / 256)), dim3(256), 0, c->stream, (const double*)c->Wn,
                     (const double*)c->Hn, c->k, (long long)c->m, (long long)c->mA, (long long)c->n, (long long)c->nA, c->flags + 5);
  HIPCHK(hipGetLastError());
  int out_of_range = 1;
  HIPCHK(hipMemcpyAsync(&out_of_range, c->flags + 5, sizeof(int), hipMemcpyDeviceToHost, c->stream));
  HIPCHK(hipStreamSynchronize(c->stream));
  c->factors_in_range = out_of_range == 0;
  return NBMF_OK;
}

int nbmf_set_factors(nbmf_ctx* c, const double* W, const double* H) {
  if (!c || !W || !H) return fail(NBMF_ERR_ARG, "null argument");
  if (int rc = set_device(c)) return rc;
  HIPCHK(hipMemcpyAsync(c->stage, W, sizeof(double) * (size_t)c->k * c->m, hipMemcpyHostToDevice, c->stream));
  launch_set_factor(c, false, c->stage, c->Wn, c->WT, c->WG);
  HIPCHK(hipGetLastError());
  HIPCHK(hipStreamSynchronize(c->stream));
  HIPCHK(hipMemcpyAsync(c->stage, H, sizeof(double) * (size_t)c->k * c->n, hipMemcpyHostToDevice, c->stream));
  launch_set_factor(c, true, c->stage, c->Hn, c->HT, c->HG);
  HIPCHK(hipGetLastError());
  hipLaunchKernelGGL(prior_kernel, dim3(c->n_prior_blocks), dim3(256), 0, c->stream, c->Hn, c->prior, c->k, c->KP,
                     (long long)c->n, (long long)c->nA, c->eps);
  HIPCHK(hipGetLastError());
  if (int rc = check_factor_range(c)) return rc;
  c->prior_src = c->prior;
  c->n_prior_src = c->n_prior_blocks;
  c->have_factors = true;
  return NBMF_OK;
}

int nbmf_get_factors(nbmf_ctx* c, double* W, double* H) {
  if (!c) return fail(NBMF_ERR_ARG, "null context");
  if (!c->have_factors) return fail(NBMF_ERR_STATE, "no factors on the device");
  if (int rc = set_device(c)) return rc;
  for (const bool h : {false, true}) {
    double* out = h ? H : W;
    if (!out) continue;
    launch_get_factor(c, h, h ? c->Hn : c->Wn, c->stage);
    HIPCHK(hipGetLastError());
    HIPCHK(hipMemcpyAsync(out, c->stage, sizeof(double) * (size_t)c->k * (h ? c->n : c->m), hipMemcpyDeviceToHost, c->stream));
    HIPCHK(hipStreamSynchronize(c->stream));
  }
  return NBMF_OK;
}

int nbmf_run(nbmf_ctx* c, int max_iter, double tol, double* losses, int* n_iter) {
  if (int rc = ready(c)) return rc;
  if (max_iter < 1) return fail(NBMF_ERR_ARG, "max_iter must be >= 1");
  if (!losses || !n_iter) return fail(NBMF_ERR_ARG, "null output");
  if (c->cancelled.load(std::memory_order_relaxed)) return fail(NBMF_ERR_STATE, "cancelled (nbmf_cancel)");
  if (int rc = set_device(c)) return rc;
  if (int rc = ensure_losses(c, max_iter)) return rc;
  HIPCHK(hipMemsetAsync(c->flags, 0, sizeof(int) * 8, c->stream));
  HIPCHK(hipMemsetAsync(c->scal, 0, sizeof(double) * 8, c->stream));
  auto& ev = c->eval;
  const bool evaling = ev.count > 0;
  ev.iters.clear();
  ev.logliks.clear();
  ev.best_iter = 0;
  ev.stopped_early = 0;
  ev.have_best = false;
  if (evaling)
    if (int rc = ensure_eval_slots(c, 3 + max_iter / ev.every)) return rc;
  if (!evaling) {
    bool handled = false;
    if (int rc = run_small(c, max_iter, tol, losses, n_iter, &handled)) return rc;
    if (handled) return NBMF_OK;
  }
  g_engine_launches_served.fetch_add(1, std::memory_order_relaxed);

  const bool progress = c->progress && c->progress_every > 0;
  const int batch = progress ? c->progress_every : (tol > 0.0) ? 8 : max_iter;
  int reported = 0;
  std::vector<double> fresh;
  auto report = [&](int n_final) -> int {
    if (!progress || n_final <= reported) return NBMF_OK;
    fresh.resize((size_t)(n_final - reported));
    HIPCHK(hipMemcpy(fresh.data(), c->losses_d + reported, sizeof(double) * fresh.size(), hipMemcpyDeviceToHost));
    c->progress(c->progress_user, reported, n_final - reported, fresh.data());
    reported = n_final;
    return NBMF_OK;
  };
  int host_done = 0;
  int it = 0;
  const bool use_graph = env_set("NBMF_USE_GRAPH") && !is_sharded(c) && !c->timing && !progress && max_iter >= 8 && !evaling;
  int limit = max_iter;
  int since_best = 0;
  double ev_val = 0.0, ev_best = 0.0;
  bool fused_fin = fin_fusable(c) && !use_graph;
  int recoveries = 0;
  int fl[8];
  auto settle = [&](bool at_end, bool* resume) -> int {
    *resume = false;
    HIPCHK(hipMemcpyAsync(fl, c->flags, sizeof fl, hipMemcpyDeviceToHost, c->stream));
    HIPCHK(hipStreamSynchronize(c->stream));
    if (c->timing) timing_collect(c);
    if (int rc = peer_check(c)) return rc;
    if (!fl[6] || !fused_fin || recoveries >= 4 || (at_end && c->cancelled.load(std::memory_order_relaxed))) return NBMF_OK;
    ++recoveries;
    g_loss_assembly_recoveries.fetch_add(1, std::memory_order_relaxed);
    if (env_set("NBMF_DEBUG")) fprintf(stderr, "[nbmf] loss %d could not be assembled inside its sweep within the bound: resuming with separate launches\n", fl[1]);
    fused_fin = false;
// ... 1279 lines not shown
```

nbmf_mm_amd/csrc/nbmf_pass_kernel.inc:

```

#define NBMF_DIV(y_, d_) ((y_) * rcp_nr(d_))
#define NBMF_DIV2(ya_, da_, yb_, db_, qa_, qb_) \
  {                                             \
    const double it_ = rcp_nr((da_) * (db_));   \
    qa_ = (ya_) * (it_ * (db_));                \
    qb_ = (yb_) * (it_ * (da_));                \
  }

#if NBMF_NO_MFMA
__device__ __forceinline__ d4 mfma_stub(double a, double b, d4 c) {
  __asm__ volatile("" : "+v"(c) : "v"(a), "v"(b));
  return c;
}
#define NBMF_MFMA(a_, b_, c_, x_, y_, z_) mfma_stub((a_), (b_), (c_))
#else
#define NBMF_MFMA(a_, b_, c_, x_, y_, z_) __builtin_amdgcn_mfma_f64_16x16x4f64((a_), (b_), (c_), (x_), (y_), (z_))
#endif

typedef __attribute__((address_space(3))) char lds_char;
typedef const __attribute__((address_space(1))) char glb_char;
typedef const __attribute__((address_space(1))) uint32_t glb_u32;
template <int PPW>
__device__ __forceinline__ void dma_run(glb_char* g, lds_char* l) {
  static_assert(PPW == 2 || PPW == 4, "2 KiB or 4 KiB per wave and image");
  __builtin_amdgcn_global_load_lds(g, l, 16, 0, 0);
  __builtin_amdgcn_global_load_lds(g, l, 16, 1024, 0);
  if (PPW == 4) {
    __builtin_amdgcn_global_load_lds(g, l, 16, 2048, 0);
    __builtin_amdgcn_global_load_lds(g, l, 16, 3072, 0);
  }
}
__device__ __forceinline__ void dma_pair_interleaved(glb_char* base, unsigned lane_off, unsigned lane_off_4k, lds_char* l) {
  __builtin_amdgcn_global_load_lds(base + lane_off, l, 16, 0, 0);
  __builtin_amdgcn_global_load_lds(base + lane_off_4k, l + 4096, 16, 0, 0);
}

typedef const __attribute__((address_space(4))) unsigned long long tile_masks_t;

constexpr unsigned long long LL_EMPTY = 0x7FF8DEADC0DE0001ull;
constexpr unsigned long long LL_WAIT_TICKS = 300000000ull;
struct PassFin {
  int on;
  unsigned long long wait_ticks;
  int t;
  int n_ll, n_prior;
  double ll_pad, am1, bm1, n_obs, tol;
  const double* prior;
  double* losses;
  double* scal;
  int* flags;
};
template <bool SC1>
__device__ __forceinline__ void finalize_block(const double* ll_src, int n_ll, double ll_pad, const double* prior, int n_prior,
                                               double am1, double bm1, double n_obs, double* __restrict__ losses, int t,
                                               double tol, double* __restrict__ scal, int* __restrict__ flags, double (*sh)[4]);

struct PassArgs {
  const void* data;
  const void* mask;
  const double2* ltab_g;
  const double* LT;
  const double* LG;
  const double* RfT;
  double* out1;
  double* out2;
  double* lossbuf;
  const int* done;
  int Rb;
  int Cb;
  const int* chunk_start;
  int chunk0;
  long long C_alloc;
  double eps;
  int strict;
  int clip;
  double* theta;
  int accum;
  int tiny_eps;
  int ksteps, kblocks;
  int full;
  PassFin fin;
  unsigned long long* trace;
};

constexpr int pass_log_bits(int KB) { return KB == 8 ? 8 : 10; }
constexpr int pass_lds_bytes(int KB, int DATA, int MODE) {
  return (KB <= 4 ? STAGE_BYTES : 2 * STAGE_BYTES) + ((DATA != DATA_BIN && MODE != MODE_W && MODE != MODE_T) ? (16 << pass_log_bits(KB)) : 0);
}
constexpr int pass_wgs_per_cu(int KB, int DATA, int MODE) {
  if (KB == 8) return (MODE == MODE_H && DATA != DATA_BIN) ? 1 : 2;
  if (DATA != DATA_BIN && MODE == MODE_H) return 2;
  if (DATA == DATA_F64 && MODE == MODE_L && KB == 1) return 2;
  return 3;
}
template <int KB, int DATA, int MODE, int TH = 0, bool TINY = false, bool RAG = false, bool FULL = false>
__global__ __launch_bounds__(64 * WG_WAVES, pass_wgs_per_cu(KB, DATA, MODE)) void pass_kernel(PassArgs a) {
  static_assert(TH == 0 || MODE != MODE_T, "a Theta sweep does not read Theta");
  static_assert(!FULL || (MODE == MODE_W && DATA == DATA_BIN && TH == 0 && !TINY), "the two-state variant: W sweeps of the binary path's plain variant");
  static_assert(!TINY || MODE != MODE_T, "eps does not change the code of the Theta sweeps");
  static_assert(!RAG || (TH == 0 && !TINY && MODE != MODE_T && KB <= 4), "the ragged-K variant: one slice, plain variant, fused sweeps, up to the K = 64 layout");
  [[maybe_unused]] const int ksteps = a.ksteps, kblocks = a.kblocks;
  constexpr bool PRODUCTS = (MODE == MODE_H || MODE == MODE_W);
  constexpr int K = 16 * KB;
  constexpr int S = K / 4;
  constexpr int NB = (KB >= 4) ? 1 : 4 / KB;
  constexpr int BLK = K * 16;
  constexpr int STAGE_D = 2 * NB * BLK;
  constexpr int N2 = NB * BLK / 2;
  extern __shared__ __attribute__((aligned(16))) double lds[];

  [[maybe_unused]] unsigned long long tr0 = 0, tr1 = 0, tr2 = 0, trc = 0;
  if (a.trace) tr0 = wall_clock64();
  const int stop_now = *a.done;
  constexpr bool GEN = DATA != DATA_BIN && MODE != MODE_T;
  constexpr int TB = pass_log_bits(KB);
  constexpr uint32_t LTAB_BYTE = 2u * STAGE_D * 8u;
  if (GEN && __builtin_amdgcn_groupstaticsize() != 0) return;
  if (GEN && MODE != MODE_W) {
    if (TB == 8) {
      log_table_fill((double2*)(lds + 2 * STAGE_D));
    } else {
      for (int i = threadIdx.x; i < (1 << TB); i += 64 * WG_WAVES) ((double2*)(lds + 2 * STAGE_D))[i] = a.ltab_g[i];
    }
  }
  constexpr bool ZE_K = DATA == DATA_BIN && !TINY && TH == 0 && (MODE == MODE_H || MODE == MODE_L);
  constexpr bool ZE_W = DATA == DATA_BIN && !TINY && TH == 0 && MODE == MODE_W;
  constexpr bool EPSACC = (GEN && TH == 0) || ZE_K || ZE_W;
  [[maybe_unused]] const double c12 = (1.0 + a.eps) + a.eps;
  [[maybe_unused]] const bool l_plain = MODE == MODE_L && (a.clip || (DATA == DATA_BIN && a.strict));
  [[maybe_unused]] const double addeps = (MODE == MODE_L && a.clip) ? a.eps : 0.0;
  const double acc0 = (EPSACC && !l_plain) ? a.eps : 0.0;

  const int lane = threadIdx.x & 63;
  const int wave = __builtin_amdgcn_readfirstlane(threadIdx.x >> 6);
  unsigned bx = blockIdx.x, by = blockIdx.y;
  if ((gridDim.y & 7u) == 0u) {
    const unsigned id = blockIdx.x + gridDim.x * blockIdx.y;
    const unsigned xcd = id & 7u, slot = id >> 3;
    bx = slot % gridDim.x;
    by = xcd + 8u * (slot / gridDim.x);
  }
  const int cb = (int)bx * WG_WAVES + wave;
  const int chunk = (int)by + a.chunk0;
  const int rb0 = a.chunk_start[chunk];
  const int rb1 = a.chunk_start[chunk + 1];
  if (stop_now) return;
  const double eps = a.eps;

  double rf[S];
  if (TH != 1) {
#pragma unroll
    for (int s = 0; s < S; ++s) rf[s] = a.RfT[((size_t)cb * S + s) * 64 + lane];
  }

  d4 acc1[KB], acc2[KB];
#pragma unroll
  for (int i = 0; i < KB; ++i) {
    acc1[i] = d4{0, 0, 0, 0};
    acc2[i] = d4{0, 0, 0, 0};
  }
  double prod = 1.0;
  int pexp = 0;
  bool negative = false;
  int t2hmin = 0x3FF00000;
  double llsum = 0.0;
  double s2 = 0.0;

  [[maybe_unused]] tile_masks_t* tmask = (tile_masks_t*)a.data + (size_t)cb * a.Rb * 8;
  const d4* yv = (const d4*)a.data + (size_t)cb * a.Rb * 64 + lane;
  const d4* mv = (const d4*)a.mask + (size_t)cb * a.Rb * 64 + lane;
  [[maybe_unused]] unsigned lane32 = (unsigned)lane * 32u;
  d4* thp = (d4*)a.theta + (size_t)cb * a.Rb * 64 + lane;
  const bool th_in = (TH != 0) || (MODE == MODE_T && a.accum != 0);

  d4 tnext[NB];
  [[maybe_unused]] d4 ybuf[2], mbuf[2];
  unsigned lane16 = (unsigned)lane * 16u;
  constexpr int PPW = N2 * 16 / WG_WAVES / 1024;
  constexpr bool ILV = PPW == 2;
  constexpr int PW_BYTES = ILV ? 1024 : N2 * 16 / WG_WAVES;
  [[maybe_unused]] unsigned lane16b = (unsigned)lane * 16u + 4096u;
  constexpr unsigned long long STRIDE_TG = (unsigned long long)NB * BLK * 8;
  auto scalar64 = [](unsigned long long v) {
    return ((unsigned long long)(unsigned)__builtin_amdgcn_readfirstlane((int)(v >> 32)) << 32) |
           (unsigned long long)(unsigned)__builtin_amdgcn_readfirstlane((int)(unsigned)v);
  };
  unsigned long long pT = scalar64((unsigned long long)(a.LT + (size_t)rb0 * BLK) + (unsigned long long)wave * PW_BYTES);
  unsigned long long pG = scalar64((unsigned long long)(a.LG + (size_t)rb0 * BLK) + (unsigned long long)wave * PW_BYTES);
#define STAGE_DMA(RB, BUF)                                                                         \
  {                                                                                                \
    lds_char* lT_ = (lds_char*)(lds + (BUF) * STAGE_D) + wave * PW_BYTES;                          \
     \
     \
     \
    __asm__ volatile("" : "+s"(pT), "+s"(pG));                                                     \
    __asm__ volatile("" : "+v"(lane16));                                                           \
    if (ILV) __asm__ volatile("" : "+v"(lane16b));                                                 \
    const unsigned l16_ = lane16;                                                                  \
    if (TH != 1) {                                   \
      if (ILV) dma_pair_interleaved((glb_char*)pT, l16_, lane16b, lT_);                            \
      else dma_run<PPW>((glb_char*)pT + l16_, lT_);                                                \
    }                                                                                              \
    if (PRODUCTS) {                              \
      if (ILV) dma_pair_interleaved((glb_char*)pG, l16_, lane16b, lT_ + N2 * 16);                  \
      else dma_run<PPW>((glb_char*)pG + l16_, lT_ + N2 * 16);                                      \
    }                                                                                              \
    if (TH != 0 || MODE == MODE_T) {                                                               \
      if (th_in) {                                                                                 \
        _Pragma("unroll") for (int b_ = 0; b_ < NB; ++b_) tnext[b_] = thp[(size_t)((RB) + b_) * 64]; \
      }                                                                                            \
    }                                                                                              \
  }

  d4 tcurT[NB];
  if (DATA != DATA_BIN && MODE != MODE_T) {
    ybuf[0] = yv[(size_t)rb0 * 64];
    if (DATA == DATA_F64M) mbuf[0] = mv[(size_t)rb0 * 64];
  }
  STAGE_DMA(rb0, 0);
#pragma unroll
  for (int b = 0; b < NB; ++b) {
    tcurT[b] = tnext[b];
  }
  __syncthreads();

  [[maybe_unused]] lanemask_t lm[2][8];
#define MASKS_REQUEST(DST, PTR)                                                           \
  if (DATA == DATA_BIN && MODE != MODE_T) {                                               \
    tile_masks_t* rec_ = (PTR);                                                           \
    _Pragma("unroll") for (int r_ = 0; r_ < (((MODE == MODE_W && !FULL) || MODE == MODE_L) ? 8 : 4); ++r_) DST[r_] = rec_[r_]; \
  }
  [[maybe_unused]] tile_masks_t* pM = tmask + (size_t)rb0 * 8;
  MASKS_REQUEST(lm[0], pM);
  pM += 8;
  constexpr int MASK_PREFETCH = 8;
  [[maybe_unused]] double zc[4] = {0.0, 0.0, 0.0, 0.0}, cc[4] = {0.0, 0.0, 0.0, 0.0};
  if ((MODE == MODE_H || MODE == MODE_W || ZE_K) && DATA == DATA_BIN && !TINY) {
#pragma unroll
    for (int r = 0; r < 4; ++r) {
      if (ZE_K || ZE_W) zc[r] = mk_double((uint32_t)__double2loint(c12), 0u);
      __asm__ volatile("" : "+v"(zc[r]));
      if (MODE == MODE_W) __asm__ volatile("" : "+v"(cc[r]));
    }
  }
  [[maybe_unused]] uint32_t pf_val = 0, pf_sink = 0;
  [[maybe_unused]] unsigned lane4 = (unsigned)lane * 4u;
  [[maybe_unused]] unsigned long long pPF = 0;
  if (DATA == DATA_BIN && MODE != MODE_T)
    pPF = scalar64((unsigned long long)((const unsigned long long*)a.data + ((size_t)cb * a.Rb + rb0 + MASK_PREFETCH) * 8));
  constexpr int UNR = (MODE != MODE_T && TH == 0 && NB <= 2) ? 2 : 1;
  [[maybe_unused]] unsigned long long pY = 0, pMk = 0;
  typedef const __attribute__((address_space(1))) d4 glb_d4;
  if (GEN) {
    pY = scalar64((unsigned long long)((const d4*)a.data + ((size_t)cb * a.Rb + rb0 + 1) * 64));
    if (DATA == DATA_F64M) pMk = scalar64((unsigned long long)((const d4*)a.mask + ((size_t)cb * a.Rb + rb0 + 1) * 64));
  }
  [[maybe_unused]] double third = 0.33333333333333331483, mquarter = -0.25;
  [[maybe_unused]] d4 acc0q = {acc0, acc0, acc0, acc0};
  if (GEN) __asm__ volatile("" : "+v"(third), "+v"(mquarter));
  if (EPSACC) __asm__ volatile("" : "+v"(acc0q));
  constexpr bool RENORM_TRIP = !TINY && UNR * NB <= 4 && (MODE == MODE_H || MODE == MODE_L);
  [[maybe_unused]] int bufv = 0;
  if (a.trace) {
    tr1 = wall_clock64();
    trc = (unsigned long long)clock64();
  }
  for (int rbo = rb0; rbo < rb1; rbo += UNR * NB) {
#pragma unroll
  for (int u = 0; u < UNR; ++u) {
    const int rb = rbo + u * NB;
    if (u > 0 && rb >= rb1) break;
    const int buf = (UNR == 2) ? u : bufv;
    if (DATA == DATA_BIN && MODE != MODE_T) {
      pf_sink ^= pf_val;
      __asm__ volatile("" : "+v"(pf_sink));
      __asm__ volatile("" : "+s"(pPF));
      __asm__ volatile("" : "+v"(lane4));
      pf_val = *(glb_u32*)((glb_char*)pPF + lane4);
      pPF += 64ull * NB;
    }
    pT += STRIDE_TG;
    pG += STRIDE_TG;
    STAGE_DMA(min(rb + NB, a.Rb - NB), buf ^ 1);
    __builtin_amdgcn_sched_barrier(0);
    const double* base = lds + buf * STAGE_D;

    constexpr int GRP = 2;
    constexpr int GT = (S < GRP) ? S : GRP;
    constexpr int NGT = S / GT;
    constexpr int PB = 4 * KB;
    constexpr int GB = (PB < GRP) ? PB : GRP;
    constexpr int NGB = PB / GB;
    double tcur[GT];
    if (TH != 1) {
#pragma unroll
      for (int i = 0; i < GT; ++i) tcur[i] = base[i * 64 + lane];
    }

#pragma unroll
    for (int b = 0; b < NB; ++b) {
      constexpr bool LM_ALT = (NB % 2 == 0) || (UNR == 2);
      const int lm_i = (NB % 2 == 0) ? (b & 1) : u;
      [[maybe_unused]] lanemask_t(&lmcur)[8] = lm[LM_ALT ? lm_i : 0];
      [[maybe_unused]] lanemask_t(&lmnxt)[8] = lm[LM_ALT ? (lm_i ^ 1) : 1];
      [[maybe_unused]] d4& ycur = ybuf[LM_ALT ? lm_i : 0];
      [[maybe_unused]] d4& ynx = ybuf[LM_ALT ? (lm_i ^ 1) : 1];
      [[maybe_unused]] d4& mcur = mbuf[LM_ALT ? lm_i : 0];
      [[maybe_unused]] d4& mnx = mbuf[LM_ALT ? (lm_i ^ 1) : 1];
      const double* ldsT = base + b * BLK;
      const double* ldsG = base + NB * BLK + b * BLK;

      constexpr bool DUAL = KB == 8 && MODE == MODE_H && DATA != DATA_BIN;
      d4 th = EPSACC ? acc0q : d4{0, 0, 0, 0}, th2 = {0, 0, 0, 0};
      if (DATA != DATA_BIN && MODE != MODE_T) {
        __asm__ volatile("" : "+s"(pY));
        __asm__ volatile("" : "+v"(lane32));
        ynx = *(glb_d4*)((glb_char*)pY + lane32);
        pY += 2048ull;
        if (DATA == DATA_F64M) {
          __asm__ volatile("" : "+s"(pMk));
          mnx = *(glb_d4*)((glb_char*)pMk + lane32);
          pMk += 2048ull;
        }
      }
      if (TH != 0 || MODE == MODE_T) {
        if (th_in) th = tcurT[b];
      }
#pragma unroll
      for (int g = 0; g < NGT && TH != 1; ++g) {
        double tnxt[GT];
        if (g + 1 < NGT) {
#pragma unroll
          for (int i = 0; i < GT; ++i) tnxt[i] = ldsT[((g + 1) * GT + i) * 64 + lane];
          __builtin_amdgcn_sched_barrier(0);
        }
#pragma unroll
        for (int i = 0; i < GT; i += 2) {
          if (RAG) {
            if (g * GT + i < ksteps) th = NBMF_MFMA(tcur[i], rf[g * GT + i], th, 0, 0, 0);
            if (g * GT + i + 1 < ksteps) th = NBMF_MFMA(tcur[i + 1], rf[g * GT + i + 1], th, 0, 0, 0);
            continue;
          }
          th = NBMF_MFMA(tcur[i], rf[g * GT + i], th, 0, 0, 0);
          if (DUAL) {
            th2 = NBMF_MFMA(tcur[i + 1], rf[g * GT + i + 1], th2, 0, 0, 0);
          } else {
            th = NBMF_MFMA(tcur[i + 1], rf[g * GT + i + 1], th, 0, 0, 0);
          }
        }
        if (g + 1 < NGT) {
#pragma unroll
          for (int i = 0; i < GT; ++i) tcur[i] = tnxt[i];
        }
      }
      if (DUAL) th += th2;
      if (TH == 2) thp[(size_t)(rb + b) * 64] = th;
      if (MODE == MODE_T) {
        thp[(size_t)(rb + b) * 64] = th;
        if (b + 1 < NB) {
#pragma unroll
          for (int i = 0; i < GT; ++i) tcur[i] = base[(b + 1) * BLK + i * 64 + lane];
        }
        continue;
      }
      if (MODE == MODE_L && a.clip) {
#pragma unroll
        for (int r = 0; r < 4; ++r) th[r] = fmin(fmax(th[r], 0.0), 1.0);
      }

      double gcur[GB];
      if (PRODUCTS) {
#pragma unroll
        for (int i = 0; i < GB; ++i) gcur[i] = ldsG[((i % KB) * 4 + (i / KB)) * 64 + lane];
      } else if (b + 1 < NB && TH != 1) {
#pragma unroll
        for (int i = 0; i < GT; ++i) tcur[i] = base[(b + 1) * BLK + i * 64 + lane];
      }
      __builtin_amdgcn_sched_barrier(0);

      constexpr bool PRIO = KB <= 2 || (MODE == MODE_W && KB == 4);
      if (PRIO) __builtin_amdgcn_s_setprio(1);
      double R1[4], R2[4];
      {
      if (DATA == DATA_BIN) {
        {
          MASKS_REQUEST(lmnxt, pM);
          pM += 8;
          __builtin_amdgcn_sched_barrier(0);
        }
        lanemask_t ym[4], zo[4];
#pragma unroll
        for (int r = 0; r < 4; ++r) {
          ym[r] = lmcur[r];
          zo[r] = lmcur[((MODE == MODE_W && !FULL) || MODE == MODE_L) ? 4 + r : r];
        }
        double dd[4];
        if (MODE == MODE_L) {
          if (ZE_K && !l_plain) {
#pragma unroll
            for (int r = 0; r < 4; ++r) {
              zc[r] = mk_double((uint32_t)__double2loint(zc[r]), __builtin_amdgcn_inverse_ballot_w64(ym[r]) ? 0u : 0x3FF00000u);
              dd[r] = __builtin_fabs(th[r] - zc[r]);
            }
          } else {
#pragma unroll
            for (int r = 0; r < 4; ++r) {
              const double dr = sel64(ym[r], th[r], 1.0 - th[r]) + eps;
              dd[r] = a.strict ? sel64(ym[r] | zo[r], dr, 1.0) : dr;
            }
          }
        } else {
          double d[4], r0[4], e[4], rr[4];
          constexpr bool ZT = (MODE == MODE_H || MODE == MODE_W) && !TINY;
          [[maybe_unused]] double z[4];
#pragma unroll
          for (int r = 0; r < 4; ++r) {
            if (ZT) {
              const uint32_t zhi = ZE_W ? (FULL ? (__builtin_amdgcn_inverse_ballot_w64(ym[r]) ? 0u : 0xBFF00000u)
                                                : (__builtin_amdgcn_inverse_ballot_w64(zo[r]) ? 0xBFF00000u : 0u))
                                   : (MODE == MODE_W) ? (__builtin_amdgcn_inverse_ballot_w64(zo[r]) ? 0x3FF00000u : 0u)
                                                      : (__builtin_amdgcn_inverse_ballot_w64(ym[r]) ? 0u : 0x3FF00000u);
              zc[r] = mk_double((uint32_t)__double2loint(zc[r]), zhi);
              z[r] = zc[r];
              d[r] = ZE_W ? th[r] + z[r] : ZE_K ? __builtin_fabs(th[r] - z[r]) : __builtin_fabs(th[r] - z[r]) + eps;
            } else {
              d[r] = sel64(ym[r], th[r], 1.0 - th[r]) + eps;
            }
          }
          constexpr bool batch = !TINY;
          if (batch) {
            const double p01 = d[0] * d[1], p23 = d[2] * d[3];
            const double ip = rcp_nr(p01 * p23);
            const double i01 = ip * p23, i23 = ip * p01;
            rr[0] = i01 * d[1];
            rr[1] = i01 * d[0];
            rr[2] = i23 * d[3];
            rr[3] = i23 * d[2];
          } else {
#pragma unroll
            for (int r = 0; r < 4; ++r) r0[r] = __builtin_amdgcn_rcp(d[r]);
#pragma unroll
            for (int r = 0; r < 4; ++r) e[r] = __builtin_fma(-d[r], r0[r], 1.0);
#pragma unroll
            for (int r = 0; r < 4; ++r) e[r] = __builtin_fma(e[r], e[r], e[r]);
#pragma unroll
            for (int r = 0; r < 4; ++r) rr[r] = __builtin_fma(r0[r], e[r], r0[r]);
          }
#pragma unroll
          for (int r = 0; r < 4; ++r) {
            dd[r] = d[r];
            if (ZT && MODE == MODE_H) {
              double rr_ = rr[r];
              __asm__("" : "+v"(rr_));
              if (ZE_K) {
                R2[r] = rr_ * z[r];
                R1[r] = rr_;
              } else {
                R2[r] = rr_ * z[r];
                R1[r] = rr_ - R2[r];
// ... 139 lines not shown
            }
            p = __builtin_fma(rr_, p, -0.5);
            p = __builtin_fma(rr_, p, 1.0);
            const double lg = __builtin_fma(rr_, p, __builtin_fma(kk[r], 0.69314718055994530942, ev[r][1]));
            llsum = __builtin_fma(ymv[r], lg, llsum);
          }
        } else
#pragma unroll
        for (int r = 0; r < 4; ++r) {
          const double y = y4[r];
          const double it1 = ipp[r] * t2v[r];
          const double it2 = ipp[r] * t1v[r];
          if (MODE == MODE_L || MODE == MODE_H) {
            double ym;
            if (MODE == MODE_L && a.strict) {
              if (DATA == DATA_F64M) {
                ym = y * m4[r];
                llsum = __builtin_fma(m4[r], log_tab<false, TB, true>(t2v[r], LTAB_BYTE, third, mquarter), llsum);
                t2p[r] = 1.0;
              } else {
                ym = y;
                t2p[r] = __double2hiint(y) >= 0 ? t2v[r] : 1.0;
              }
            } else {
              ym = (DATA == DATA_F64M) ? y * m4[r] : y;
              t2p[r] = t2v[r];
            }
            if (MODE == MODE_H) {
              R1[r] = ym * it1;
              R2[r] = __builtin_fma(-ym, it2, it2);
            }
            llsum = __builtin_fma(ym, log_tab<false, TB, true>(t1v[r] * it2, LTAB_BYTE, third, mquarter), llsum);
          } else {
            const double yo = (DATA == DATA_F64M) ? y * m4[r] : max0(y);
            double s2e;
            if (DATA == DATA_F64M) {
              s2e = ((1.0 - y) * m4[r]) * it2;
              __asm__("" : "+v"(s2e));
            } else {
              if (TINY) {
                s2e = max0(1.0 - y) * it2;
                __asm__("" : "+v"(s2e));
              } else {
                s2e = max0(__builtin_fma(-y, it2, it2));
              }
            }
            R1[r] = __builtin_fma(yo, it1, -s2e);
            s2 += s2e;
          }
        }
        if (MODE == MODE_L || MODE == MODE_H) {
          if (TINY) {
#pragma unroll
            for (int r = 0; r < 4; ++r) {
              int e;
              prod = frexp(prod * t2p[r], &e);
              pexp += e;
            }
          } else {
            prod *= (t2p[0] * t2p[1]) * (t2p[2] * t2p[3]);
            if (!RENORM_TRIP) {
              int e;
              prod = frexp(prod, &e);
              pexp += e;
            }
          }
        }
      }
      }
      if (DATA == DATA_BIN && !LM_ALT) {
#pragma unroll
        for (int r = 0; r < 8; ++r) lmcur[r] = lmnxt[r];
      }

      if (PRIO) __builtin_amdgcn_s_setprio(0);
      if (PRODUCTS) {
#pragma unroll
      for (int g = 0; g < NGB; ++g) {
        double gnxt[GB];
        if (g + 1 < NGB) {
#pragma unroll
          for (int i = 0; i < GB; ++i) {
            const int p = (g + 1) * GB + i;
            gnxt[i] = ldsG[((p % KB) * 4 + (p / KB)) * 64 + lane];
          }
          __builtin_amdgcn_sched_barrier(0);
        } else if (b + 1 < NB && TH != 1) {
#pragma unroll
          for (int i = 0; i < GT; ++i) tcur[i] = base[(b + 1) * BLK + i * 64 + lane];
          __builtin_amdgcn_sched_barrier(0);
        }
#pragma unroll
        for (int i = 0; i < GB; ++i) {
          const int p = g * GB + i, r = p / KB, kb = p % KB;
          if (RAG && KB >= 4 && kb >= kblocks) continue;
          acc1[kb] = NBMF_MFMA(gcur[i], R1[r], acc1[kb], 0, 0, 0);
          if (MODE == MODE_H) acc2[kb] = NBMF_MFMA(gcur[i], R2[r], acc2[kb], 0, 0, 0);
        }
        if (g + 1 < NGB) {
#pragma unroll
          for (int i = 0; i < GB; ++i) gcur[i] = gnxt[i];
        }
      }
      }
    }

#pragma unroll
    for (int b = 0; b < NB; ++b) {
      tcurT[b] = tnext[b];
    }
    __syncthreads();
    bufv ^= 1;
  }
    if (RENORM_TRIP) {
      int e;
      prod = frexp(prod, &e);
      pexp += e;
    }
  }
  if (DATA == DATA_BIN && MODE != MODE_T && (pf_sink ^ pf_val) == 0x5A17C0DEu && a.Rb < 0)
    ((uint32_t*)a.out1)[lane] = pf_sink;

#undef STAGE_DMA
#undef MASKS_REQUEST
  if (a.trace) {
    tr2 = wall_clock64();
    trc = (unsigned long long)clock64() - trc;
  }
  constexpr bool LOSS = (MODE == MODE_H || MODE == MODE_L);
  if (LOSS && a.lossbuf) {
    double ll;
    if (DATA == DATA_BIN)
      ll = negative ? __builtin_nan("") : log_of_product(prod, pexp);
    else
      ll = t2hmin < 0 ? __builtin_nan("") : (t2hmin < 0x00100000 ? -__builtin_inf() : llsum + log_of_product(prod, pexp));
    ll = wave_sum(ll);
    __syncthreads();
    if (lane == 0) lds[wave] = ll;
    __syncthreads();
    if (threadIdx.x == 0) {
      double t = lds[0];
#pragma unroll
      for (int w_ = 1; w_ < WG_WAVES; ++w_) t += lds[w_];
      if (!(a.fin.on == 2 && blockIdx.x == 0 && blockIdx.y == 0))
        __hip_atomic_store(a.lossbuf + (size_t)chunk * gridDim.x + bx, t, __ATOMIC_RELAXED, __HIP_MEMORY_SCOPE_AGENT);
    }
  }

  [[maybe_unused]] unsigned long long tr3 = 0, tr4 = 0;
  if (a.trace) tr3 = wall_clock64();
  const int q = lane >> 4, c = lane & 15;
  {
    if (MODE == MODE_W) {
      s2 += __shfl_xor(s2, 16, 64);
      s2 += __shfl_xor(s2, 32, 64);
    }
    [[maybe_unused]] const double inv12 = 1.0 / c12;
    double* o1 = a.out1 + (size_t)chunk * K * a.C_alloc + (size_t)cb * 16 + c;
    double* o2 = (MODE == MODE_H) ? a.out2 + (size_t)chunk * K * a.C_alloc + (size_t)cb * 16 + c : nullptr;
    if (PRODUCTS) {
#pragma unroll
      for (int kb = 0; kb < KB; ++kb) {
#pragma unroll
        for (int r = 0; r < 4; ++r) {
          const size_t k = 16 * kb + 4 * r + q;
          if (MODE == MODE_H) {
            o1[k * a.C_alloc] = acc1[kb][r];
            o2[k * a.C_alloc] = acc2[kb][r];
          } else {
            o1[k * a.C_alloc] = ZE_W ? __builtin_fma(s2, inv12, acc1[kb][r]) : acc1[kb][r] + s2;
          }
        }
      }
    }
  }
  if (a.trace) tr4 = wall_clock64();
  if (LOSS && a.lossbuf && a.fin.on && blockIdx.x == gridDim.x - 1 && blockIdx.y == gridDim.y - 1) {
    const unsigned long long* slots = (const unsigned long long*)a.lossbuf;
    const unsigned long long t0 = (unsigned long long)wall_clock64();
    for (;;) {
      int missing = 0;
      for (int j = threadIdx.x; j < a.fin.n_ll; j += 64 * WG_WAVES)
        missing |= __hip_atomic_load(slots + j, __ATOMIC_RELAXED, __HIP_MEMORY_SCOPE_AGENT) == LL_EMPTY;
      const bool expired = (unsigned long long)wall_clock64() - t0 > a.fin.wait_ticks;
      volatile int* again = (volatile int*)lds + 17;
      volatile int* some_missing = (volatile int*)lds + 18;
      __syncthreads();
      if (threadIdx.x == 0) {
        *again = 0;
        *some_missing = 0;
      }
      __syncthreads();
      if (missing) {
        *some_missing = 1;
        if (!expired) *again = 1;
      }
      __syncthreads();
      if (!*again) {
        if (*some_missing) {
          if (threadIdx.x == 0) {
            a.fin.flags[0] = 1;
            a.fin.flags[6] = 1;
          }
          return;
        }
        break;
// ... 26 lines not shown
```

nbmf_mm_amd/csrc/nbmf_peer_kernels.inc:

```

constexpr int PEER_MAX_RANKS = 16;
constexpr int PEER_H_WGS = 128;
constexpr int PF_IN = 0, PF_OUT = PEER_MAX_RANKS, PF_COUNT = 2 * PEER_MAX_RANKS, PF_SLOT = 40, PF_ERR = 2 * PF_SLOT, PF_WORDS = 128;

struct PeerView {
  double* arena[PEER_MAX_RANKS];
  unsigned long long* flag[PEER_MAX_RANKS];
  int nranks, rank;
  int fbase;
  unsigned long long timeout;
};

__device__ __forceinline__ void peer_signal(const PeerView& pv, int word0, unsigned long long epoch) {
  const int j = threadIdx.x;
  if (j < pv.nranks) __hip_atomic_store(pv.flag[j] + pv.fbase + word0 + pv.rank, epoch, __ATOMIC_RELEASE, __HIP_MEMORY_SCOPE_SYSTEM);
}

__device__ __forceinline__ bool peer_wait(const PeerView& pv, int word0, unsigned long long epoch, int* stop_flags) {
  __shared__ int ok;
  if (threadIdx.x == 0) ok = 1;
  __syncthreads();
  if ((int)threadIdx.x < pv.nranks) {
    unsigned long long* f = pv.flag[pv.rank] + pv.fbase + word0 + threadIdx.x;
    const unsigned long long t0 = wall_clock64();
// ... 59 lines not shown
                                                     const double* __restrict__ Hn, int K, int KP, long long n, long long nA,
                                                     double am1, double bm1, double eps, double* __restrict__ ll_out,
                                                     int* stop_flags, int fin_t ,
                                                     long long offPR_prev, int n_prior_prev, double n_obs,
                                                     double* __restrict__ losses, double tol, double* __restrict__ scal,
                                                     double pform ) {
  if (stop_flags[0]) return;
  if (blockIdx.x == 0 && threadIdx.x < 64) peer_signal(pv, PF_IN, epoch);
  if (!peer_wait(pv, PF_IN, epoch, stop_flags)) return;
  double la = 0, lb = 0;
  for (long long idx = (long long)blockIdx.x * 256 + threadIdx.x; idx < (long long)KP * wp; idx += (long long)gridDim.x * 256) {
    const long long k = idx / wp, j = c0 + idx % wp;
    double h = 0.0;
    const long long nat = k * nA + j;
    if (k < K && j < n) {
      double p1 = 0, p2 = 0;
      for (int base = 0; base < pv.nranks; base += 8) {
        double v1[8], v2[8];
#pragma unroll
        for (int u = 0; u < 8; ++u) {
          const bool on = base + u < pv.nranks;
          v1[u] = on ? pv.arena[base + u][nat] : 0.0;
          v2[u] = on ? pv.arena[base + u][offP2 + nat] : 0.0;
        }
#pragma unroll
        for (int u = 0; u < 8; ++u)
          if (base + u < pv.nranks) {
            p1 += v1[u];
            p2 += v2[u];
          }
      }
      if (pform != 0.0) {
        p2 *= pform;
        p1 -= p2;
      }
      const double hold = Hn[nat];
      const double num = hold * p1 + am1;
      const double den = (1.0 - hold) * p2 + bm1;
      h = num / (num + den + eps);
      h = (h < eps) ? eps : ((h > 1.0 - eps) ? 1.0 - eps : h);
      la += log(h + eps);
      lb += log(1.0 - h + eps);
    }
    for (int r = 0; r < pv.nranks; ++r) pv.arena[r][offHX + nat] = h;
  }
  __shared__ double sh[2][4];
  __shared__ double shf[3][4];
  __shared__ double ll_total;
  la = wave_sum(la);
  lb = wave_sum(lb);
  if ((threadIdx.x & 63) == 0) {
    sh[0][threadIdx.x >> 6] = la;
    sh[1][threadIdx.x >> 6] = lb;
  }
  __syncthreads();
  if (threadIdx.x == 0) {
    double x = 0, y = 0;
    for (int i = 0; i < 4; ++i) {
      x += sh[0][i];
      y += sh[1][i];
    }
    const long long slot = offPR + 2 * (long long)(slot0 + blockIdx.x);
    for (int r = 0; r < pv.nranks; ++r) {
      pv.arena[r][slot] = x;
      pv.arena[r][slot + 1] = y;
    }
    if (blockIdx.x == 0 && ll_index >= 0) {
      double ll = 0.0;
      for (int r = 0; r < pv.nranks; ++r) ll += pv.arena[r][ll_index];
      *ll_out = ll;
      ll_total = ll;
    }
  }
  if (blockIdx.x == 0 && fin_t >= 0) {
    __syncthreads();
    finalize_block<false>(&ll_total, 1, 0.0, pv.arena[pv.rank] + offPR_prev, n_prior_prev, am1, bm1, n_obs, losses, fin_t, tol, scal,
                   stop_flags, shf);
  }
  peer_finish(pv, epoch);
}

__global__ __launch_bounds__(256) void peer_h_apply_kernel(PeerView pv, unsigned long long epoch, long long offHX,
                                                           double* __restrict__ Hn, double* __restrict__ HT,
                                                           double* __restrict__ HG, int KP,
                                                           int KS , long long nA,
                                                           long long c0, long long wp ,
                                                           int* stop_flags) {
  if (stop_flags[0]) return;
  if (!peer_wait(pv, PF_OUT, epoch, stop_flags)) return;
  const double* src = pv.arena[pv.rank] + offHX;
  for (long long i = (long long)blockIdx.x * 256 + threadIdx.x; i < (long long)KP * wp; i += (long long)gridDim.x * 256) {
    const long long k = i / wp, j = c0 + i % wp;
    const double h = src[k * nA + j];
    Hn[k * nA + j] = h;
    HT[t_index(k, j, KS, nA)] = h;
    HG[g_index(k, j, KS, nA)] = h;
  }
}

__global__ __launch_bounds__(256) void peer_selftest_fill_kernel(double* __restrict__ arena, long long cnt, int rank, int t) {
  for (long long i = (long long)blockIdx.x * 256 + threadIdx.x; i < cnt; i += (long long)gridDim.x * 256)
    arena[i] = (double)(rank + 1) * (double)((i + 7 * t) % 1021 + 1) + t;
}
__global__ __launch_bounds__(256) void peer_selftest_check_kernel(const double* __restrict__ arena, long long cnt, int nranks, int t,
                                                                  unsigned long long* __restrict__ bad) {
  const double tri = 0.5 * nranks * (nranks + 1);
  unsigned long long n = 0;
  for (long long i = (long long)blockIdx.x * 256 + threadIdx.x; i < cnt; i += (long long)gridDim.x * 256)
    n += arena[i] != tri * (double)((i + 7 * t) % 1021 + 1) + (double)t * nranks;
  if (n) atomicAdd(bad, n);
}
```

nbmf_mm_amd/csrc/nbmf_small_kernel.inc:

```

struct SmallArgs {
  unsigned long long prob_stride;
  const double *am1s, *bm1s;
  const void *dataA, *maskA, *dataB, *maskB;
  double *Wn[2], *WT[2], *WG[2];
  double *Hn[2], *HT[2], *HG[2];
  const double* rowcnt;
  unsigned long long* sync;
  double* ll_part;
  double* prior_part;
  double* losses;
  int* result;
  long long m, n, mA, nA;
  int K, RbA, CbA;
  int Rbe, Cbe;
  int G, max_iter, projection, tiny_eps;
  double tol, eps, am1, bm1, n_obs, n_div, ll_pad;
  unsigned long long timeout;
  int PH, PW;
  double* part_buf;
  double* part_ll;
  unsigned long long* part_flag;
  int fenced;
  unsigned long long* dbg;
  unsigned long long* place;
  __device__ int dbg_g() const { return 0; }
};

typedef const __attribute__((address_space(4))) struct SmallArgs sm_karg_t;
__device__ __forceinline__ sm_karg_t* sm_cold_args() {
  sm_karg_t* p = (sm_karg_t*)__builtin_amdgcn_kernarg_segment_ptr();
  __asm__ volatile("" : "+s"(p));
  return p;
}
#define SM_COLD(field_) (sm_cold_args()->field_)

constexpr int sm_waves(int KB) { return KB == 1 ? 16 : 8; }
constexpr int SM_TPW = 8;

__device__ __forceinline__ double ld_sc1(const double* p) {
  return __hip_atomic_load(p, __ATOMIC_RELAXED, __HIP_MEMORY_SCOPE_AGENT);
}
__device__ __forceinline__ void st_sc1(double* p, double v) {
  __hip_atomic_store(p, v, __ATOMIC_RELAXED, __HIP_MEMORY_SCOPE_AGENT);
}

__device__ __forceinline__ double dpp_add(double v, int ctrl_tag) {
  int lo = __double2loint(v), hi = __double2hiint(v), lo2, hi2;
  switch (ctrl_tag) {
    case 0: lo2 = __builtin_amdgcn_mov_dpp(lo, 0xB1, 0xF, 0xF, true); hi2 = __builtin_amdgcn_mov_dpp(hi, 0xB1, 0xF, 0xF, true); break;
    case 1: lo2 = __builtin_amdgcn_mov_dpp(lo, 0x4E, 0xF, 0xF, true); hi2 = __builtin_amdgcn_mov_dpp(hi, 0x4E, 0xF, 0xF, true); break;
    case 2: lo2 = __builtin_amdgcn_mov_dpp(lo, 0x141, 0xF, 0xF, true); hi2 = __builtin_amdgcn_mov_dpp(hi, 0x141, 0xF, 0xF, true); break;
    default: lo2 = __builtin_amdgcn_mov_dpp(lo, 0x140, 0xF, 0xF, true); hi2 = __builtin_amdgcn_mov_dpp(hi, 0x140, 0xF, 0xF, true); break;
  }
  return v + __hiloint2double(hi2, lo2);
}
__device__ __forceinline__ double wave_sum_fast(double v) {
  v = dpp_add(v, 0);
  v = dpp_add(v, 1);
  v = dpp_add(v, 2);
  v = dpp_add(v, 3);
  const int lo = __double2loint(v), hi = __double2hiint(v);
  const double r0 = __hiloint2double(__builtin_amdgcn_readlane(hi, 0), __builtin_amdgcn_readlane(lo, 0));
  const double r1 = __hiloint2double(__builtin_amdgcn_readlane(hi, 16), __builtin_amdgcn_readlane(lo, 16));
  const double r2 = __hiloint2double(__builtin_amdgcn_readlane(hi, 32), __builtin_amdgcn_readlane(lo, 32));
  const double r3 = __hiloint2double(__builtin_amdgcn_readlane(hi, 48), __builtin_amdgcn_readlane(lo, 48));
  return ((r0 + r1) + r2) + r3;
}

__device__ __forceinline__ void small_release() {
  __builtin_amdgcn_fence(__ATOMIC_RELEASE, "agent");
  __asm__ volatile("s_waitcnt vmcnt(0)" ::: "memory");
}
__device__ __forceinline__ void small_acquire() {
  __builtin_amdgcn_fence(__ATOMIC_ACQUIRE, "agent");
  __asm__ volatile("s_waitcnt vmcnt(0)" ::: "memory");
}
__device__ __forceinline__ void small_arrive(const SmallArgs& a, unsigned long long* sync, unsigned long long epoch, int* ok_lds) {
  __asm__ volatile("s_waitcnt vmcnt(0)" ::: "memory");
  __syncthreads();
  if (threadIdx.x == 0) {
    *ok_lds = 1;
    if (SM_COLD(fenced)) small_release();
    __hip_atomic_store(sync + blockIdx.x, epoch, __ATOMIC_RELAXED, __HIP_MEMORY_SCOPE_AGENT);
  }
}
__device__ __forceinline__ bool small_wait(const SmallArgs& a, unsigned long long* sync, unsigned long long epoch, int* ok_lds) {
  if (threadIdx.x < 64) {
    const unsigned long long t0 = wall_clock64();
    unsigned polls = 0;
    for (int j = threadIdx.x; j < a.G; j += 64) {
      while (__hip_atomic_load(sync + j, __ATOMIC_RELAXED, __HIP_MEMORY_SCOPE_AGENT) < epoch) {
        if ((++polls & 63u) == 0u && (wall_clock64() - t0 > SM_COLD(timeout) ||
                                      __hip_atomic_load(sync + a.G, __ATOMIC_RELAXED, __HIP_MEMORY_SCOPE_AGENT) != 0ull)) {
          __hip_atomic_store(sync + a.G, 1ull, __ATOMIC_RELAXED, __HIP_MEMORY_SCOPE_AGENT);
          *ok_lds = 0;
          break;
        }
      }
    }
    if (SM_COLD(fenced)) small_acquire();
  }
  __syncthreads();
  return *ok_lds != 0;
}
__device__ __forceinline__ bool small_barrier(const SmallArgs& a, unsigned long long* sync, unsigned long long epoch, int* ok_lds) {
  small_arrive(a, sync, epoch, ok_lds);
  return small_wait(a, sync, epoch, ok_lds);
}

template <int KB, bool WITH_G>
__device__ __forceinline__ void small_load(const double* __restrict__ LT, const double* __restrict__ LG, int rb, int lane,
                                           int n_components, double* lt, double* lg) {
  constexpr int S = 4 * KB;
#pragma unroll
  for (int s = 0; s < S; ++s) lt[s] = (4 * s < n_components) ? ld_sc1(LT + ((size_t)rb * S + s) * 64 + lane) : 0.0;
  if (WITH_G) {
#pragma unroll
    for (int i = 0; i < 4 * KB; ++i) lg[i] = ld_sc1(LG + ((size_t)rb * KB * 4 + i) * 64 + lane);
  }
}

struct SmallData {
  uint32_t code;
  const void *data, *mask;
  size_t index;
};
template <int DATA>
__device__ __forceinline__ SmallData small_data(const void* data, const void* mask, size_t tile_index) {
  SmallData d;
  d.data = data;
  d.mask = mask;
  d.index = tile_index;
  d.code = (DATA == DATA_BIN) ? ((const uint32_t*)data)[tile_index] : 0u;
  return d;
}

template <int KB, int DATA, int MODE>
__device__ __forceinline__ void small_tile(const SmallArgs& a, const double* lt, const double* lg, const double* rf,
                                           const SmallData& dt, const double2* ltab,
                                           d4* acc1, d4* acc2, double& s2, double& prod, int& pexp, double& llsum,
                                           double& t2min) {
  constexpr int K = 16 * KB, S = K / 4;
  const double eps = a.eps;
  const uint32_t code = dt.code;
  d4 y4 = {0, 0, 0, 0}, m4 = {1, 1, 1, 1};
  if (DATA != DATA_BIN) {
    y4 = ((const d4*)dt.data)[dt.index];
    if (DATA == DATA_F64M) m4 = ((const d4*)dt.mask)[dt.index];
  }
  d4 th = {0, 0, 0, 0};
#pragma unroll
  for (int s = 0; s < S; ++s)
    if (4 * s < a.K) th = __builtin_amdgcn_mfma_f64_16x16x4f64(lt[s], rf[s], th, 0, 0, 0);
  double R1[4], R2[4];
  if (DATA == DATA_BIN) {
    double dd[4];
    uint32_t ymb = code & 0x01010101u * CB_YM, zob = code & 0x01010101u * CB_ZOBS;
    __asm__("" : "+v"(ymb), "+v"(zob));
    lanemask_t ym[4], zo[4];
    if (MODE == MODE_W)
      byte_set8(ymb, zob, ym, zo);
    else
      byte_set4(ymb, ym);
#pragma unroll
    for (int r = 0; r < 4; ++r) dd[r] = sel64(ym[r], th[r], 1.0 - th[r]) + eps;
    if (MODE != MODE_L) {
      double rr[4];
      if (!a.tiny_eps) {
        const double p01 = dd[0] * dd[1], p23 = dd[2] * dd[3];
        const double ip = rcp_nr(p01 * p23);
        const double i01 = ip * p23, i23 = ip * p01;
        rr[0] = i01 * dd[1];
        rr[1] = i01 * dd[0];
        rr[2] = i23 * dd[3];
        rr[3] = i23 * dd[2];
      } else {
#pragma unroll
        for (int r = 0; r < 4; ++r) rr[r] = rcp_nr(dd[r]);
      }
#pragma unroll
      for (int r = 0; r < 4; ++r) {
        if (MODE == MODE_H) {
          R1[r] = sel64_or0(ym[r], rr[r]);
          double rr_ = rr[r];
          __asm__("" : "+v"(rr_));
          R2[r] = rr_ - R1[r];
        } else {
          const double nr = sel64_or0(zo[r], rr[r]);
          s2 += nr;
          R1[r] = sel64_neg(ym[r], rr[r], nr);
          __asm__("s_nop 1" : "+v"(R1[r]));
        }
      }
    }
    if (MODE != MODE_W) {
      if (a.tiny_eps) {
#pragma unroll
        for (int r = 0; r < 4; ++r) {
          int e;
          prod = frexp(prod * dd[r], &e);
          pexp += e;
// ... 55 lines not shown
        break;
      }
    }
  }
  if (threadIdx.x < 64 && SM_COLD(fenced)) small_acquire();
  __syncthreads();
  return *ok_lds != 0;
}
__device__ __forceinline__ void small_signal_part(unsigned long long* part_flag, int me, unsigned long long tag) {
  __asm__ volatile("s_waitcnt vmcnt(0)" ::: "memory");
  __syncthreads();
  if (threadIdx.x == 0) {
    if (SM_COLD(fenced)) small_release();
    __hip_atomic_store(part_flag + me, tag, __ATOMIC_RELAXED, __HIP_MEMORY_SCOPE_AGENT);
  }
}

template <typename T>
__device__ __forceinline__ T* small_pp(T* p, unsigned long long off) { return (T*)((char*)p + off); }

template <int KB, int DATA, bool SPLIT, bool BATCH>
__global__ __launch_bounds__(64 * sm_waves(KB), 1) void small_fit_kernel(SmallArgs a) {
  constexpr int K = 16 * KB, S = K / 4, SM_WAVES = sm_waves(KB);
  constexpr int RED = SM_WAVES * 2 * KB * 4 * 64;
  const unsigned long long poff = BATCH ? (unsigned long long)blockIdx.y * a.prob_stride : 0ull;
#define PP(ptr_) small_pp((ptr_), poff)
  const double am1 = BATCH ? SM_COLD(am1s)[blockIdx.y] : a.am1, bm1 = BATCH ? SM_COLD(bm1s)[blockIdx.y] : a.bm1;
  unsigned long long* const sync = PP(a.sync);
  const bool diag = !BATCH || blockIdx.y == 0;
  extern __shared__ __attribute__((aligned(16))) double lds[];
  double* red = lds;
  double* aux = lds + RED;
  double* ownH = aux + SM_WAVES * 16 + 64;
  double* ownW = ownH + K * 16;
  double2* ltab = (double2*)(ownW + K * 16);
  __shared__ int ok_lds;
  __shared__ double bc[4];
  const int g = blockIdx.x;
  const int PH = SPLIT ? a.PH : 1, PW = SPLIT ? a.PW : 1;
  const bool hrole = g < a.Cbe * PH, wrole = g < a.Rbe * PW;
  const int sh = g / PH, ph = g % PH, sw = g / PW, pw = g % PW;
  const bool hown = hrole && ph == 0, wown = wrole && pw == 0;
  const double eps = a.eps;
  if (SM_COLD(place) && diag && threadIdx.x == 0)
    SM_COLD(place)[g] = ((unsigned long long)__builtin_amdgcn_s_getreg((31 << 11) | 20) << 32) | (unsigned)__builtin_amdgcn_s_getreg((31 << 11) | 4);
  if (SM_COLD(dbg) && diag && g == a.dbg_g() && threadIdx.x == 0) SM_COLD(dbg)[15] = wall_clock64();
  log_table_fill(ltab);
  if (threadIdx.x < KB * 256) {
    const int k = threadIdx.x >> 4, cc = threadIdx.x & 15;
    ownH[threadIdx.x] = hown ? PP(a.Hn[1])[(size_t)k * a.nA + 16LL * sh + cc] : 0.0;
    ownW[threadIdx.x] = wown ? PP(a.Wn[1])[(size_t)k * a.mA + 16LL * sw + cc] : 0.0;
  }
  __syncthreads();

  unsigned long long epoch = 0;
  double prev_loss = 0.0;
  int p_cur = 1;
  for (int t = 0;; ++t) {
    int tid = threadIdx.x;
    __asm__ volatile("" : "+v"(tid));
    const int lane = tid & 63, wave = __builtin_amdgcn_readfirstlane(tid >> 6);
    const int q = lane >> 4, c = lane & 15;
    const int p_new = t & 1;
    const bool last = t == a.max_iter;
    const unsigned long long tagH = 2ull * t + 1, tagW = 2ull * t + 2;
    SM_MARK(0);
    if (SM_COLD(dbg) && diag && g == a.dbg_g() && threadIdx.x == 0 && t < 64) SM_COLD(dbg)[t * 16 + 14] = clock64();
    if (hrole) {
      double rf[S];
#pragma unroll
      for (int s = 0; s < S; ++s)
        rf[s] = (!SPLIT || hown) ? ownH[(4 * s + q) * 16 + c] : ((4 * s < a.K) ? ld_sc1(PP(a.HT[p_cur]) + ((size_t)sh * S + s) * 64 + lane) : 0.0);
      d4 acc1[KB], acc2[KB];
#pragma unroll
      for (int i = 0; i < KB; ++i) acc1[i] = acc2[i] = d4{0, 0, 0, 0};
      double s2 = 0.0, prod = 1.0, llsum = 0.0, t2min = 1.0;
      int pexp = 0;
      const int rb0 = ph + PH * wave;
#pragma unroll 1
      for (int rb = rb0; rb < a.Rbe; rb += PH * SM_WAVES) {
        double lt[S], lg[4 * KB];
        const size_t ti = ((size_t)sh * a.RbA + rb) * 64 + lane;
        if (last) {
          small_load<KB, false>(PP(a.WT[p_cur]), PP(a.WG[p_cur]), rb, lane, a.K, lt, lg);
          const SmallData dt = small_data<DATA>(a.dataA, a.maskA, ti);
          small_tile<KB, DATA, MODE_L>(a, lt, lg, rf, dt, ltab, acc1, acc2, s2, prod, pexp, llsum, t2min);
        } else {
          small_load<KB, true>(PP(a.WT[p_cur]), PP(a.WG[p_cur]), rb, lane, a.K, lt, lg);
          const SmallData dt = small_data<DATA>(a.dataA, a.maskA, ti);
          small_tile<KB, DATA, MODE_H>(a, lt, lg, rf, dt, ltab, acc1, acc2, s2, prod, pexp, llsum, t2min);
        }
      }
      SM_MARK(1);
      double ll;
      if (DATA == DATA_BIN)
        ll = log_tab<false>(prod, ltab) + (double)pexp * 0.6931471805599453094;
      else
        ll = t2min < 0.0 ? __builtin_nan("") : (t2min < 2.2250738585072014e-308 ? -__builtin_inf() : llsum);
      ll = wave_sum_fast(ll);
      if (lane == 0) aux[SM_WAVES * 16 + wave] = (rb0 < a.Rbe) ? ll : 0.0;
      if (!last) {
#pragma unroll
        for (int kb = 0; kb < KB; ++kb)
#pragma unroll
          for (int r = 0; r < 4; ++r) {
            red[(((size_t)wave * 2 + 0) * KB * 4 + kb * 4 + r) * 64 + lane] = acc1[kb][r];
            red[(((size_t)wave * 2 + 1) * KB * 4 + kb * 4 + r) * 64 + lane] = acc2[kb][r];
          }
      }
      __syncthreads();
      if (SM_COLD(dbg)) SM_MARK(12);
      const int e = tid >> 6, ln = tid & 63;
      const int k = 16 * (e >> 2) + 4 * (e & 3) + (ln >> 4), cc = ln & 15;
      double p1 = 0.0, p2 = 0.0, sacc = 0.0;
      if (!last && tid < KB * 256) {
        double v1[SM_WAVES], v2[SM_WAVES];
#pragma unroll
        for (int w = 0; w < SM_WAVES; ++w) {
          v1[w] = red[(((size_t)w * 2 + 0) * KB * 4 + e) * 64 + ln];
          v2[w] = red[(((size_t)w * 2 + 1) * KB * 4 + e) * 64 + ln];
        }
#pragma unroll
        for (int w = 0; w < SM_WAVES; ++w) {
          p1 += v1[w];
          p2 += v2[w];
        }
      }
      if (tid == 64 * (SM_WAVES - 1)) {
        double sll[SM_WAVES];
#pragma unroll
        for (int w = 0; w < SM_WAVES; ++w) sll[w] = aux[SM_WAVES * 16 + w];
#pragma unroll
        for (int w = 0; w < SM_WAVES; ++w) sacc += sll[w];
      }
      if (SPLIT && PH > 1) {
        double* mine = PP(SM_COLD(part_buf)) + (size_t)g * 2 * K * 16;
        if (ph != 0) {
          if (!last && tid < KB * 256) {
            st_sc1(mine + tid, p1);
            st_sc1(mine + K * 16 + tid, p2);
          }
          if (tid == 64 * (SM_WAVES - 1)) st_sc1(PP(SM_COLD(part_ll)) + g, sacc);
          small_signal_part(PP(SM_COLD(part_flag)), g, tagH);
        } else {
          if (!small_wait_parts(a, sync, PP(SM_COLD(part_flag)), g, PH, tagH, &ok_lds)) break;
          for (int p = 1; p < PH; ++p) {
            const double* theirs = PP(SM_COLD(part_buf)) + (size_t)(g + p) * 2 * K * 16;
            if (!last && tid < KB * 256) {
              p1 += ld_sc1(theirs + tid);
              p2 += ld_sc1(theirs + K * 16 + tid);
            }
            if (tid == 64 * (SM_WAVES - 1)) sacc += ld_sc1(PP(SM_COLD(part_ll)) + g + p);
          }
        }
      }
      if (!SPLIT || hown) {
        if (tid == 64 * (SM_WAVES - 1)) st_sc1(PP(a.ll_part) + (size_t)p_new * a.Cbe + sh, sacc);
        if (!last) {
          double la = 0.0, lb = 0.0;
          if (tid < KB * 256) {
            const long long j = 16LL * sh + cc;
            double h = 0.0;
            if (k < a.K && j < a.n) {
              const double hold = ownH[k * 16 + cc];
              const double num = hold * p1 + am1;
              const double den = (1.0 - hold) * p2 + bm1;
              h = num * rcp_nr(num + den + eps);
              h = (h < eps) ? eps : ((h > 1.0 - eps) ? 1.0 - eps : h);
              la = log_tab<false>(h + eps, ltab);
              lb = log_tab<false>(1.0 - h + eps, ltab);
            }
            ownH[k * 16 + cc] = h;
            st_sc1(PP(a.Hn[p_new]) + (size_t)k * a.nA + j, h);
            st_sc1(PP(a.HT[p_new]) + ((size_t)sh * K + k) * 16 + cc, h);
            st_sc1(PP(a.HG[p_new]) + (size_t)sh * K * 16 + (k >> 4) * 256 + cc * 16 + (k & 15), h);
          }
          if (SM_COLD(dbg)) SM_MARK(13);
          const double pr = wave_sum_fast(__builtin_fma(am1, la, bm1 * lb));
          if (lane == 0 && wave < KB * 4)
            st_sc1(PP(a.prior_part) + ((size_t)(t % 3) * a.Cbe + sh) * (KB * 4) + wave, pr);
        }
      }
    }
    SM_MARK(2);
    if (!small_barrier(a, sync, ++epoch, &ok_lds)) break;
    SM_MARK(3);
    constexpr int NPR = KB * 4;
    const bool loss_wave = (tid >> 6) == (SPLIT ? 0 : 1);
    double l0 = 0.0, l1[NPR];
#pragma unroll
    for (int w = 0; w < NPR; ++w) l1[w] = 0.0;
#define SM_REQUEST_LOSS()                                                                               \
    if (t > 0 && loss_wave && lane < a.Cbe) {                                                           \
      l0 = ld_sc1(PP(a.ll_part) + (size_t)p_new * a.Cbe + lane);                                            \
      _Pragma("unroll") for (int w = 0; w < NPR; ++w)                                                   \
        l1[w] = ld_sc1(PP(a.prior_part) + ((size_t)((t + 2) % 3) * a.Cbe + lane) * NPR + w);                \
    }
    if (last || !wrole) SM_REQUEST_LOSS();
    if (!last && wrole) {
      double rf[S];
#pragma unroll
      for (int s = 0; s < S; ++s)
        rf[s] = (!SPLIT || wown) ? ownW[(4 * s + q) * 16 + c] : ((4 * s < a.K) ? ld_sc1(PP(a.WT[p_cur]) + ((size_t)sw * S + s) * 64 + lane) : 0.0);
      d4 acc1[KB], acc2[KB];
#pragma unroll
      for (int i = 0; i < KB; ++i) acc1[i] = acc2[i] = d4{0, 0, 0, 0};
      double s2 = 0.0, prod = 1.0, llsum = 0.0, t2min = 1.0;
      int pexp = 0;
#pragma unroll 1
      for (int rb = pw + PW * wave; rb < a.Cbe; rb += PW * SM_WAVES) {
        double lt[S], lg[4 * KB];
        const size_t ti = ((size_t)sw * a.CbA + rb) * 64 + lane;
        small_load<KB, true>(PP(a.HT[p_new]), PP(a.HG[p_new]), rb, lane, a.K, lt, lg);
        const SmallData dt = small_data<DATA>(a.dataB, a.maskB, ti);
        if (SM_COLD(dbg)) {
          SM_MARK(8);
          __asm__ volatile("s_waitcnt vmcnt(0)" ::: "memory");
          SM_MARK(9);
        }
        small_tile<KB, DATA, MODE_W>(a, lt, lg, rf, dt, ltab, acc1, acc2, s2, prod, pexp, llsum, t2min);
        if (SM_COLD(dbg)) SM_MARK(10);
      }
      SM_MARK(4);
      SM_REQUEST_LOSS();
      s2 += __shfl_xor(s2, 16, 64);
      s2 += __shfl_xor(s2, 32, 64);
#pragma unroll
      for (int kb = 0; kb < KB; ++kb)
#pragma unroll
        for (int r = 0; r < 4; ++r) red[((size_t)wave * KB * 4 + kb * 4 + r) * 64 + lane] = acc1[kb][r];
      if (lane < 16) aux[wave * 16 + lane] = s2;
      __syncthreads();
      double* tile = red + (size_t)SM_WAVES * KB * 4 * 64;
      double* par = tile + K * 16;
      const int e = tid >> 6, ln = tid & 63;
      const int k = 16 * (e >> 2) + 4 * (e & 3) + (ln >> 4), cc = ln & 15;
      double qv = 0.0, sv = 0.0;
      if (tid < KB * 256) {
        double vq[SM_WAVES], vs[SM_WAVES];
#pragma unroll
        for (int ww = 0; ww < SM_WAVES; ++ww) {
          vq[ww] = red[((size_t)ww * KB * 4 + e) * 64 + ln];
          vs[ww] = aux[ww * 16 + cc];
        }
#pragma unroll
        for (int ww = 0; ww < SM_WAVES; ++ww) {
          qv += vq[ww];
          sv += vs[ww];
        }
      }
      if (SPLIT && PW > 1) {
        double* mine = PP(SM_COLD(part_buf)) + (size_t)g * 2 * K * 16;
        if (pw != 0) {
          if (tid < KB * 256) st_sc1(mine + tid, qv);
          if (tid < 16) st_sc1(mine + K * 16 + tid, sv);
          small_signal_part(PP(SM_COLD(part_flag)), g, tagW);
        } else {
          if (!small_wait_parts(a, sync, PP(SM_COLD(part_flag)), g, PW, tagW, &ok_lds)) break;
          for (int p = 1; p < PW; ++p) {
            const double* theirs = PP(SM_COLD(part_buf)) + (size_t)(g + p) * 2 * K * 16;
            if (tid < KB * 256) {
              qv += ld_sc1(theirs + tid);
              sv += ld_sc1(theirs + K * 16 + cc);
            }
          }
        }
      }
      if (!SPLIT || wown) {
        const long long i = 16LL * sw + cc;
        if (tid < KB * 256) {
          double w = 0.0;
          if (k < a.K && i < a.m) {
            double div = a.n_div;
            if (a.projection == NBMF_PROJ_DUCHI) div = fmax(SM_COLD(rowcnt)[i], 1.0);
            w = (ownW[k * 16 + cc] * (qv + sv)) / div;
          }
          tile[k * 16 + cc] = w;
        }
        __syncthreads();
        if (a.projection == NBMF_PROJ_DUCHI) {
          if (tid < 16) {
            const int c2i = tid;
            double sum = 0.0;
            for (int kk = 0; kk < a.K; ++kk) sum += tile[kk * 16 + c2i];
            double tau = (sum - 1.0) / a.K;
            int cnt = a.K;
            for (int it = 0; it < a.K; ++it) {
              double s = 0.0;
              int c2 = 0;
              for (int kk = 0; kk < a.K; ++kk) {
                const double v = tile[kk * 16 + c2i];
                if (v > tau) {
                  s += v;
                  ++c2;
                }
              }
              if (c2 == 0) break;
              const bool same = (c2 == cnt);
              tau = (s - 1.0) / c2;
              cnt = c2;
              if (same) break;
            }
            par[16 + c2i] = tau;
          }
          __syncthreads();
        }
        if (tid < KB * 256) {
          double w = 0.0;
          const double v = tile[k * 16 + cc];
          if (a.projection == NBMF_PROJ_DUCHI) {
            w = fmax(v - par[16 + cc], 0.0);
          } else {
            double col[K];
#pragma unroll
            for (int kk = 0; kk < K; ++kk) col[kk] = tile[kk * 16 + cc];
            double sum = 0.0;
#pragma unroll
            for (int kk = 0; kk < K; ++kk) sum += col[kk];
            w = v / sum;
          }
          if (!(k < a.K && i < a.m)) w = 0.0;
          ownW[k * 16 + cc] = w;
          st_sc1(PP(a.Wn[p_new]) + (size_t)k * a.mA + i, w);
          st_sc1(PP(a.WT[p_new]) + ((size_t)sw * K + k) * 16 + cc, w);
          st_sc1(PP(a.WG[p_new]) + (size_t)sw * K * 16 + (k >> 4) * 256 + cc * 16 + (k & 15), w);
        }
      }
    }
    SM_MARK(5);
    if (!last) small_arrive(a, sync, ++epoch, &ok_lds);
    if (t > 0 && loss_wave) {
      double v = l0;
#pragma unroll
      for (int w = 0; w < NPR; ++w) v += l1[w];
      if (lane + 64 < a.Cbe) {
        const int j = lane + 64;
        double b0 = ld_sc1(PP(a.ll_part) + (size_t)p_new * a.Cbe + j), b1[NPR];
#pragma unroll
        for (int w = 0; w < NPR; ++w) b1[w] = ld_sc1(PP(a.prior_part) + ((size_t)((t + 2) % 3) * a.Cbe + j) * NPR + w);
#pragma unroll
        for (int w = 0; w < NPR; ++w) b0 += b1[w];
        v += b0;
      }
      const double sv = wave_sum_fast(v);
      const double loss = -(sv - SM_COLD(ll_pad)) / SM_COLD(n_obs);
      const bool stop_now = t - 1 > 0 && fabs(prev_loss - loss) / fabs(prev_loss) < SM_COLD(tol);
      prev_loss = loss;
      if (lane == 0) {
        bc[0] = loss;
        bc[1] = stop_now ? 1.0 : 0.0;
      }
    }
    SM_MARK(6);
    if (last) {
      __syncthreads();
    } else if (!small_wait(a, sync, epoch, &ok_lds)) {
      break;
    }
    SM_MARK(7);
    bool stop = false;
    if (t > 0) {
      if (g == 0 && tid == 0) PP(SM_COLD(losses))[t - 1] = bc[0];
      stop = bc[1] != 0.0;
    }
    if (stop || last) {
      if (SM_COLD(dbg) && diag && g == a.dbg_g() && tid == 0) SM_COLD(dbg)[63 * 16 + 15] = wall_clock64();
      if (g == 0 && tid == 0) {
        PP(SM_COLD(result))[0] = t;
        PP(SM_COLD(result))[1] = p_cur;
      }
      return;
    }
    p_cur = p_new;
  }
#undef SM_REQUEST_LOSS
  if (threadIdx.x == 0) PP(SM_COLD(result))[2] = 1;
#undef PP
}
```

nbmf_mm_amd/csrc/nbmf_update_kernels.inc:

```

__device__ __forceinline__ size_t t_index(long long k, long long x, int KS, long long lenA) {
  return (size_t)(k / KS) * KS * lenA + (size_t)((x >> 4) * KS + (k % KS)) * 16 + (x & 15);
}
__device__ __forceinline__ size_t g_index(long long k, long long x, int KS, long long lenA) {
  const long long kk = k % KS;
  return (size_t)(k / KS) * KS * lenA + (size_t)(x >> 4) * KS * 16 + (kk >> 4) * 256 + (x & 15) * 16 + (kk & 15);
}

__device__ __forceinline__ double ordered_sum256(const double* __restrict__ p, int n, int stride, double* sh4) {
  double s = 0.0;
  for (int j = threadIdx.x; j < n; j += 256) s += p[(size_t)j * stride];
  s = wave_sum(s);
  __syncthreads();
  if ((threadIdx.x & 63) == 0) sh4[threadIdx.x >> 6] = s;
  __syncthreads();
  return ((sh4[0] + sh4[1]) + sh4[2]) + sh4[3];
}

__global__ __launch_bounds__(256) void reduce_h_kernel(const double* __restrict__ slab1, const double* __restrict__ slab2,
                                                       int chunks, long long per , long long nA,
                                                       long long c0, long long wp, long long dst_ld, int KP,
                                                       double* __restrict__ dst1, double* __restrict__ dst2,
                                                       const double* __restrict__ lossbuf,
                                                       int n_loss, double ll_pad, double* __restrict__ ll_dst,
                                                       const int* done,
                                                       double pform ) {
  __shared__ double sh4[4];
  if (*done) return;
  const long long i = (long long)blockIdx.x * blockDim.x + threadIdx.x;
  if (i < (long long)KP * wp) {
    const long long k = i / wp, jj = i % wp;
    const size_t src = (size_t)k * nA + c0 + jj;
    double s1 = 0, s2 = 0;
    for (int ch = 0; ch < chunks; ++ch) {
      s1 += slab1[(size_t)ch * per + src];
      s2 += slab2[(size_t)ch * per + src];
    }
    if (pform != 0.0) {
      s2 *= pform;
      s1 -= s2;
    }
    dst1[k * dst_ld + jj] = s1;
    dst2[k * dst_ld + jj] = s2;
  }
  if (ll_dst && blockIdx.x == 0) {
    const double s = ordered_sum256(lossbuf, n_loss, 1, sh4);
    if (threadIdx.x == 0) *ll_dst = s - ll_pad;
  }
}

__global__ __launch_bounds__(256) void prior_reduce_kernel(const double* __restrict__ prior, int n_prior,
                                                           double* __restrict__ out2, const int* done) {
  __shared__ double sh4[4];
  if (*done) return;
  const double a = ordered_sum256(prior, n_prior, 2, sh4);
  const double b = ordered_sum256(prior + 1, n_prior, 2, sh4);
  if (threadIdx.x == 0) {
    out2[0] = a;
    out2[1] = b;
  }
}

__global__ __launch_bounds__(256) void reduce_w_kernel(const double* __restrict__ slab, double* __restrict__ Qbuf,
                                                       int chunks, long long per, const int* done) {
  if (*done) return;
  const long long i = (long long)blockIdx.x * blockDim.x + threadIdx.x;
  if (i >= per) return;
  double s = 0;
  for (int ch = 0; ch < chunks; ++ch) s += slab[(size_t)ch * per + i];
  Qbuf[i] = s;
}

__global__ __launch_bounds__(256) void ll_reduce_kernel(const double* __restrict__ lossbuf, int n_loss, double ll_pad,
                                                        double* __restrict__ out, const int* done) {
  __shared__ double sh4[4];
  if (*done) return;
  const double s = ordered_sum256(lossbuf, n_loss, 1, sh4);
  if (threadIdx.x == 0) *out = s - ll_pad;
}

__device__ __forceinline__ void block_sum2(double a, double b, double* out2) {
  __shared__ double sh[2][8];
  a = wave_sum(a);
  b = wave_sum(b);
  const int w = threadIdx.x >> 6;
  if ((threadIdx.x & 63) == 0) {
    sh[0][w] = a;
    sh[1][w] = b;
  }
  __syncthreads();
  if (threadIdx.x == 0) {
    double x = 0, y = 0;
    for (int i = 0; i < (int)(blockDim.x >> 6); ++i) {
      x += sh[0][i];
      y += sh[1][i];
    }
    out2[0] = x;
    out2[1] = y;
  }
}

__global__ __launch_bounds__(256) void h_update_kernel(const double* __restrict__ src1, const double* __restrict__ src2,
                                                       int chunks, size_t chunk_stride, long long src_ld, long long src_c0,
                                                       long long c0, long long wp, double* __restrict__ Hn,
                                                       double* __restrict__ HT, double* __restrict__ HG,
                                                       double* __restrict__ prior, int K, int KP, long long n,
                                                       long long nA, double am1, double bm1, double eps, const int* done,
                                                       double pform ) {
  if (*done) return;
  const long long idx = (long long)blockIdx.x * blockDim.x + threadIdx.x;
  const long long k = idx / wp, j = c0 + idx % wp;
  double la = 0, lb = 0;
  if (k < KP) {
    double h = 0.0;
    const size_t nat = (size_t)k * nA + j;
    if (k < K && j < n) {
      const size_t src = (size_t)k * src_ld + (j - src_c0);
      double p1 = 0, p2 = 0;
      for (int ch = 0; ch < chunks; ++ch) {
        p1 += src1[(size_t)ch * chunk_stride + src];
        p2 += src2[(size_t)ch * chunk_stride + src];
      }
      if (pform != 0.0) {
        p2 *= pform;
        p1 -= p2;
      }
      const double hold = Hn[nat];
      const double num = hold * p1 + am1;
      const double den = (1.0 - hold) * p2 + bm1;
      h = num / (num + den + eps);
      h = (h < eps) ? eps : ((h > 1.0 - eps) ? 1.0 - eps : h);
      la = log(h + eps);
      lb = log(1.0 - h + eps);
    }
    Hn[nat] = h;
    const long long jb = j >> 4, c = j & 15;
    HT[(jb * KP + k) * 16 + c] = h;
    HG[jb * KP * 16 + (k >> 4) * 256 + c * 16 + (k & 15)] = h;
  }
  block_sum2(la, lb, prior + 2 * (size_t)blockIdx.x);
}

__global__ __launch_bounds__(256) void prior_kernel(const double* __restrict__ Hn, double* __restrict__ prior, int K,
                                                    int KP, long long n, long long nA, double eps) {
  const long long idx = (long long)blockIdx.x * blockDim.x + threadIdx.x;
  const long long k = idx / nA, j = idx % nA;
  double la = 0, lb = 0;
  if (k < K && j < n) {
    const double h = Hn[idx];
    la = log(h + eps);
    lb = log(1.0 - h + eps);
  }
  block_sum2(la, lb, prior + 2 * (size_t)blockIdx.x);
}

template <bool SC1>
__device__ __forceinline__ void finalize_block(const double* ll_src, int n_ll, double ll_pad, const double* prior, int n_prior,
                                               double am1, double bm1, double n_obs, double* __restrict__ losses, int t,
                                               double tol, double* __restrict__ scal, int* __restrict__ flags,
                                               double (*sh)[4] ) {
  double s0 = 0.0, s1 = 0.0, s2 = 0.0;
  const int n_max = n_ll > n_prior ? n_ll : n_prior;
#pragma unroll 4
  for (int j = threadIdx.x; j < n_max; j += 256) {
    if (j < n_ll) s0 += SC1 ? __hip_atomic_load(ll_src + j, __ATOMIC_RELAXED, __HIP_MEMORY_SCOPE_AGENT) : ll_src[j];
    if (j < n_prior) {
      s1 += prior[2 * (size_t)j];
      s2 += prior[2 * (size_t)j + 1];
    }
  }
  s0 = wave_sum(s0);
  s1 = wave_sum(s1);
  s2 = wave_sum(s2);
  if ((threadIdx.x & 63) == 0) {
    sh[0][threadIdx.x >> 6] = s0;
    sh[1][threadIdx.x >> 6] = s1;
    sh[2][threadIdx.x >> 6] = s2;
  }
  __syncthreads();
  const double ll = (((sh[0][0] + sh[0][1]) + sh[0][2]) + sh[0][3]) - ll_pad;
  const double sa = ((sh[1][0] + sh[1][1]) + sh[1][2]) + sh[1][3];
  const double sb = ((sh[2][0] + sh[2][1]) + sh[2][2]) + sh[2][3];
  if (threadIdx.x == 0) {
    const double A = am1 * sa;
    const double B = bm1 * sb;
    const double loss = -(ll + A + B) / n_obs;
    losses[t] = loss;
    flags[1] = t + 1;
    flags[2] = t + 1;
    if (t > 0) {
      const double prev = scal[0];
      if (fabs(prev - loss) / fabs(prev) < tol) flags[0] = 1;
    }
    scal[0] = loss;
  }
}

__global__ __launch_bounds__(256) void finalize_kernel(const double* __restrict__ ll_src, int n_ll, double ll_pad,
                                                       const double* __restrict__ prior, int n_prior, double am1,
                                                       double bm1, double n_obs, double* __restrict__ losses, int t,
                                                       double tol, double* __restrict__ scal, int* __restrict__ flags) {
  if (flags[0]) return;
  if (t < 0) {
    const int armed = flags[3];
    __syncthreads();
    if (!armed) {
      if (threadIdx.x == 0) flags[3] = 1;
      return;
    }
    t = flags[2];
  }
  __shared__ double sh[3][4];
  finalize_block<false>(ll_src, n_ll, ll_pad, prior, n_prior, am1, bm1, n_obs, losses, t, tol, scal, flags, sh);
}

constexpr int WU_COLS = 32;
template <int WU_GROUPS>
__global__ __launch_bounds__(WU_COLS * WU_GROUPS) void w_update_kernel(const double* __restrict__ slab, int chunks, double* __restrict__ Wn,
                                                       double* __restrict__ WT, double* __restrict__ WG, int K, int KP,
                                                       int KS , long long m,
                                                       long long mA, double n_div,
                                                       const double* __restrict__ rowcnt, int projection,
                                                       const int* done) {
  extern __shared__ __attribute__((aligned(16))) double tile[];
  if (*done) return;
  const int c = threadIdx.x & (WU_COLS - 1), g = threadIdx.x / WU_COLS;
  const long long i = (long long)blockIdx.x * WU_COLS + c;
  const size_t per = (size_t)KS * mA;
  const bool live = i < m;
  double div = n_div;
  if (live && projection == NBMF_PROJ_DUCHI && rowcnt) div = fmax(rowcnt[i], 1.0);
  for (int k = g; k < K; k += WU_GROUPS) {
    double w = 0.0;
    if (live) {
      double qv = 0.0;
      const double* sk = slab + (size_t)(k / KS) * chunks * per + (size_t)(k % KS) * mA + i;
      for (int ch = 0; ch < chunks; ++ch) qv += sk[(size_t)ch * per];
      w = (Wn[(size_t)k * mA + i] * qv) / div;
    }
    tile[k * WU_COLS + c] = w;
  }
  __syncthreads();
  double* par = tile + (size_t)KP * WU_COLS;
  if (g == 0) {
    double sum = 0.0;
    for (int k = 0; k < K; ++k) sum += tile[k * WU_COLS + c];
    double tau = 0.0, scale = 1.0;
    if (projection == NBMF_PROJ_DUCHI) {
      tau = (sum - 1.0) / K;
      int cnt = K;
      for (int it = 0; it < K; ++it) {
        double s = 0.0;
        int c2 = 0;
        for (int k = 0; k < K; ++k) {
          const double v = tile[k * WU_COLS + c];
          if (v > tau) {
            s += v;
            ++c2;
          }
        }
        if (c2 == 0) break;
        const bool same = (c2 == cnt);
        tau = (s - 1.0) / c2;
        cnt = c2;
        if (same) break;
      }
    } else {
      scale = sum;
    }
    par[c] = scale;
    par[WU_COLS + c] = tau;
  }
  __syncthreads();
  const double scale = par[c], tau = par[WU_COLS + c];
  for (int k = g; k < KP; k += WU_GROUPS) {
    double w = 0.0;
    if (live && k < K) {
      const double v = tile[k * WU_COLS + c];
      w = (projection == NBMF_PROJ_DUCHI) ? fmax(v - tau, 0.0) : v / scale;
    }
    Wn[(size_t)k * mA + i] = w;
    WT[t_index(k, i, KS, mA)] = w;
    WG[g_index(k, i, KS, mA)] = w;
  }
}

__global__ void set_factor_kernel(const double* __restrict__ src, double* __restrict__ Fn, double* __restrict__ FT,
                                  double* __restrict__ FG, int K, int KP, int KS, long long len, long long lenA) {
  const long long idx = (long long)blockIdx.x * blockDim.x + threadIdx.x;
  if (idx >= (long long)KP * lenA) return;
  const long long k = idx / lenA, x = idx % lenA;
  const double v = (k < K && x < len) ? src[k * len + x] : 0.0;
  Fn[idx] = v;
  FT[t_index(k, x, KS, lenA)] = v;
  FG[g_index(k, x, KS, lenA)] = v;
}

__global__ void factor_range_kernel(const double* __restrict__ Wn, const double* __restrict__ Hn, int K, long long m,
                                    long long mA, long long n, long long nA, int* bad) {
  const long long idx = (long long)blockIdx.x * blockDim.x + threadIdx.x;
  bool ok = true;
  if (idx < m) {
    double s = 0.0;
    for (int k = 0; k < K; ++k) {
      const double w = Wn[(size_t)k * mA + idx];
      ok = ok && (w >= 0.0);
      s += w;
    }
    ok = ok && (s <= 1.0 + 1e-12);
  }
  const long long k = idx / nA, j = idx % nA;
  if (k < K && j < n) {
    const double h = Hn[idx];
    ok = ok && (h >= 0.0) && (h <= 1.0 - 1e-9);
  }
  if (!ok) atomicOr(bad, 1);
}

__global__ void get_factor_kernel(const double* __restrict__ Fn, double* __restrict__ dst, int K, long long len,
                                  long long lenA) {
  const long long idx = (long long)blockIdx.x * blockDim.x + threadIdx.x;
  if (idx >= (long long)K * len) return;
  const long long k = idx / len, x = idx % len;
  dst[idx] = Fn[k * lenA + x];
}
```

Before: 201.4.

## Replace separate G operand image with XOR-swizzled S image and halve staging

Replaces the second transposed factor image (G, k-contiguous per column) with a swizzled image S that shares the T layout but XOR-permutes columns within each 16-wide block. The pass kernel now streams a single operand image per stage instead of both T and G, which halves the stage buffer and LDS footprint, and changes the stage count per k-block. It also rewrites the small-kernel loads and all update/set kernels to produce the swizzled layout. The intent is less global traffic and LDS per workgroup, possibly raising occupancy. The cost is extra index arithmetic in fragment reads and the risk of bank conflicts or mismatched swizzle.

Result: no change. 203.1, median of 6 (+0.8%).

```diff
diff --git a/nbmf_mm_amd/csrc/nbmf_hip.hip b/nbmf_mm_amd/csrc/nbmf_hip.hip
--- a/nbmf_mm_amd/csrc/nbmf_hip.hip
+++ b/nbmf_mm_amd/csrc/nbmf_hip.hip
@@ -78,7 +78,7 @@
 constexpr int PAD = 128;
 constexpr int WG_WAVES = 4;
 constexpr size_t PASS_SLACK = 65536;
-constexpr int STAGE_BYTES = 32768;
+constexpr int STAGE_BYTES = 16384;
 
 __device__ __forceinline__ double rcp_nr(double d) {
   double r = __builtin_amdgcn_rcp(d);
@@ -242,7 +242,7 @@
   unsigned long long *bitsA = nullptr, *bitsB = nullptr;
   double n_obs = 0, n_obs_global = 0;
   double* rowcnt = nullptr;
-  double *Wn = nullptr, *WT = nullptr, *WG = nullptr, *Hn = nullptr, *HT = nullptr, *HG = nullptr;
+  double *Wn = nullptr, *WT = nullptr, *WS = nullptr, *Hn = nullptr, *HT = nullptr, *HS = nullptr;
   bool have_factors = false;
   bool padB_ones = false;
   bool w_free = false;
@@ -297,7 +297,7 @@
   long long psl_c0[2] = {0, 0}, psl_wp[2] = {0, 0};
   double *Pbuf_own = nullptr, *sbuf_own = nullptr, *Qbuf_own = nullptr;
   struct SmallWs {
-    double *Wn = nullptr, *WT = nullptr, *WG = nullptr, *Hn = nullptr, *HT = nullptr, *HG = nullptr;
+    double *Wn = nullptr, *WT = nullptr, *WS = nullptr, *Hn = nullptr, *HT = nullptr, *HS = nullptr;
     double *snapW = nullptr, *snapH = nullptr, *ll_part = nullptr, *prior_part = nullptr;
     unsigned long long* sync = nullptr;
     int* result = nullptr;
@@ -995,8 +995,7 @@
   PassArgs a{};
   a.data = sweep_image(c, 0);
   a.mask = c->maskA;
-  a.LT = c->WT;
-  a.LG = c->WG;
+  a.LS = c->WS;
   a.RfT = c->HT;
   a.out1 = c->slabH;
   a.out2 = c->slabH + (size_t)c->chunksH * c->KP * c->nA;
@@ -1016,8 +1015,7 @@
   PassArgs a{};
   a.data = sweep_image(c, 1);
   a.mask = c->maskB;
-  a.LT = c->HT;
-  a.LG = c->HG;
+  a.LS = c->HS;
   a.RfT = c->WT;
   a.out1 = c->slabW;
   a.out2 = nullptr;
@@ -1037,8 +1035,7 @@
 
 void at_slice(const nbmf_ctx* c, PassArgs& a, int image, int sl) {
   const size_t offW = (size_t)sl * SLICE_K * c->mA, offH = (size_t)sl * SLICE_K * c->nA;
-  a.LT = image == 0 ? c->WT + offW : c->HT + offH;
-  a.LG = image == 0 ? c->WG + offW : c->HG + offH;
+  a.LS = image == 0 ? c->WS + offW : c->HS + offH;
   a.RfT = image == 0 ? c->HT + offH : c->WT + offW;
   const size_t slab_off = image == 0 ? (size_t)c->chunksH * offH : (size_t)c->chunksW * offW;
   if (a.out1) a.out1 += slab_off;
@@ -1168,7 +1165,7 @@
   const long long blk0 = (long long)KSK * (sl * c->nA + c0) / 256;
   hipLaunchKernelGGL(h_update_kernel, dim3((unsigned)((long long)KSK * wp / 256)), dim3(256), 0, st, src,
                      src + (size_t)chunks * c->KP * wp, chunks, chunk_stride, wp, c0, c0, wp, c->Hn + sl * per, c->HT + sl * per,
-                     c->HG + sl * per, c->prior + 2 * (size_t)blk0, std::min(KSK, c->k - sl * KSK), KSK, (long long)c->n,
+                     c->HS + sl * per, c->prior + 2 * (size_t)blk0, std::min(KSK, c->k - sl * KSK), KSK, (long long)c->n,
                      (long long)c->nA, c->alpha - 1.0, c->beta - 1.0, c->eps, c->flags, pform);
 }
 
@@ -1202,7 +1199,7 @@
   if (lds_bytes > 65536)
     HIPCHK(hipFuncSetAttribute((const void*)w_update_kernel<GROUPS>, hipFuncAttributeMaxDynamicSharedMemorySize, (int)lds_bytes));
   hipLaunchKernelGGL(w_update_kernel<GROUPS>, dim3((unsigned)(c->mA / WU_COLS)), dim3(WU_COLS * GROUPS), lds_bytes, c->stream, q,
-                     chunks, c->Wn, c->WT, c->WG, c->k, c->KP, std::min(c->KP, SLICE_K), (long long)c->m, (long long)c->mA, n_div,
+                     chunks, c->Wn, c->WT, c->WS, c->k, c->KP, std::min(c->KP, SLICE_K), (long long)c->m, (long long)c->mA, n_div,
                      c->rowcnt, projection, c->flags);
   HIPCHK(hipGetLastError());
   return NBMF_OK;
@@ -1262,7 +1259,7 @@
   auto apply_panel = [&](int p, hipStream_t st, unsigned long long e) -> int {
     PeerView pv = c->pv;
     pv.fbase = p * PF_SLOT;
-    hipLaunchKernelGGL(peer_h_apply_kernel, dim3(PEER_H_WGS), dim3(256), 0, st, pv, e, c->offHX, c->Hn, c->HT, c->HG, c->KP,
+    hipLaunchKernelGGL(peer_h_apply_kernel, dim3(PEER_H_WGS), dim3(256), 0, st, pv, e, c->offHX, c->Hn, c->HT, c->HS, c->KP,
                        std::min(c->KP, SLICE_K), (long long)c->nA, c->pc0[p], c->pc0[p + 1] - c->pc0[p], c->flags);
     HIPCHK(hipGetLastError());
     return NBMF_OK;
@@ -1423,18 +1420,18 @@
   return enqueue_w_update(c, q, chunks, n_div, projection);
 }
 
-__global__ void expand_factor_kernel(const double* __restrict__ Fn, double* __restrict__ FT, double* __restrict__ FG, int KP,
+__global__ void expand_factor_kernel(const double* __restrict__ Fn, double* __restrict__ FT, double* __restrict__ FS, int KP,
                                      int KS, long long lenA) {
   const long long idx = (long long)blockIdx.x * blockDim.x + threadIdx.x;
   if (idx >= (long long)KP * lenA) return;
   const long long k = idx / lenA, x = idx % lenA;
   FT[t_index(k, x, KS, lenA)] = Fn[idx];
-  FG[g_index(k, x, KS, lenA)] = Fn[idx];
-}
-
-void launch_set_factor(const nbmf_ctx* c, bool h, const double* src, double* Fn, double* FT, double* FG) {
+  FS[s_index(k, x, KS, lenA)] = Fn[idx];
+}
+
+void launch_set_factor(const nbmf_ctx* c, bool h, const double* src, double* Fn, double* FT, double* FS) {
   const long long len = h ? c->n : c->m, lenA = h ? c->nA : c->mA, tot = (long long)c->KP * lenA;
-  hipLaunchKernelGGL(set_factor_kernel, dim3((unsigned)((tot + 255) / 256)), dim3(256), 0, c->stream, src, Fn, FT, FG, c->k, c->KP,
+  hipLaunchKernelGGL(set_factor_kernel, dim3((unsigned)((tot + 255) / 256)), dim3(256), 0, c->stream, src, Fn, FT, FS, c->k, c->KP,
                      std::min(c->KP, SLICE_K), len, lenA);
 }
 void launch_get_factor(const nbmf_ctx* c, bool h, const double* Fn, double* dst) {
@@ -1444,7 +1441,7 @@
 void launch_expand_factor(const nbmf_ctx* c, bool h) {
   const long long lenA = h ? c->nA : c->mA, tot = (long long)c->KP * lenA;
   hipLaunchKernelGGL(expand_factor_kernel, dim3((unsigned)((tot + 255) / 256)), dim3(256), 0, c->stream, (const double*)(h ? c->Hn : c->Wn),
-                     h ? c->HT : c->WT, h ? c->HG : c->WG, c->KP, c->KP, lenA);
+                     h ? c->HT : c->WT, h ? c->HS : c->WS, c->KP, c->KP, lenA);
 }
 
 constexpr int SMALL_MAX_WGS = 256;
@@ -1507,11 +1504,11 @@
   HIPCHK(hipMemsetAsync(base, 0, total, c->stream));
   c->small.slab = base;
   char* p = base;
-  for (double** q : {&c->small.Wn, &c->small.WT, &c->small.WG, &c->small.snapW}) {
+  for (double** q : {&c->small.Wn, &c->small.WT, &c->small.WS, &c->small.snapW}) {
     *q = (double*)p;
     p += fw;
   }
-  for (double** q : {&c->small.Hn, &c->small.HT, &c->small.HG, &c->small.snapH}) {
+  for (double** q : {&c->small.Hn, &c->small.HT, &c->small.HS, &c->small.snapH}) {
     *q = (double*)p;
     p += fh;
   }
@@ -1639,8 +1636,8 @@
   const size_t fw = (size_t)c->KP * c->mA * sizeof(double), fh = (size_t)c->KP * c->nA * sizeof(double);
   SmallArgs a{};
   small_common_args(c, max_iter, tol, &a);
-  a.Wn[0] = w.Wn; a.WT[0] = w.WT; a.WG[0] = w.WG; a.Hn[0] = w.Hn; a.HT[0] = w.HT; a.HG[0] = w.HG;
-  a.Wn[1] = c->Wn; a.WT[1] = c->WT; a.WG[1] = c->WG; a.Hn[1] = c->Hn; a.HT[1] = c->HT; a.HG[1] = c->HG;
+  a.Wn[0] = w.Wn; a.WT[0] = w.WT; a.WS[0] = w.WS; a.Hn[0] = w.Hn; a.HT[0] = w.HT; a.HS[0] = w.HS;
+  a.Wn[1] = c->Wn; a.WT[1] = c->WT; a.WS[1] = c->WS; a.Hn[1] = c->Hn; a.HT[1] = c->HT; a.HS[1] = c->HS;
   a.sync = w.sync;
   a.ll_part = w.ll_part;
   a.prior_part = w.prior_part;
@@ -1748,10 +1745,10 @@
   if (res[1] == 0) {
     HIPCHK(hipMemcpyAsync(c->Wn, w.Wn, fw, hipMemcpyDeviceToDevice, c->stream));
     HIPCHK(hipMemcpyAsync(c->WT, w.WT, fw, hipMemcpyDeviceToDevice, c->stream));
-    HIPCHK(hipMemcpyAsync(c->WG, w.WG, fw, hipMemcpyDeviceToDevice, c->stream));
+    HIPCHK(hipMemcpyAsync(c->WS, w.WS, fw, hipMemcpyDeviceToDevice, c->stream));
     HIPCHK(hipMemcpyAsync(c->Hn, w.Hn, fh, hipMemcpyDeviceToDevice, c->stream));
     HIPCHK(hipMemcpyAsync(c->HT, w.HT, fh, hipMemcpyDeviceToDevice, c->stream));
-    HIPCHK(hipMemcpyAsync(c->HG, w.HG, fh, hipMemcpyDeviceToDevice, c->stream));
+    HIPCHK(hipMemcpyAsync(c->HS, w.HS, fh, hipMemcpyDeviceToDevice, c->stream));
   }
   HIPCHK(hipMemcpyAsync(losses, c->losses_d, sizeof(double) * (size_t)res[0], hipMemcpyDeviceToHost, c->stream));
   HIPCHK(stream_wait_spin(c->stream));
@@ -1842,10 +1839,10 @@
     for (int par = 0; par < 2; ++par) {
       a.Wn[par] = (double*)q; q += L.fw;
       a.WT[par] = (double*)q; q += L.fw;
-      a.WG[par] = (double*)q; q += L.fw;
+      a.WS[par] = (double*)q; q += L.fw;
       a.Hn[par] = (double*)q; q += L.fh;
       a.HT[par] = (double*)q; q += L.fh;
-      a.HG[par] = (double*)q; q += L.fh;
+      a.HS[par] = (double*)q; q += L.fh;
     }
     a.ll_part = (double*)q; q += L.ll_b;
     a.prior_part = (double*)q; q += L.pr_b;
@@ -1874,8 +1871,8 @@
     HIPCHK(hipMemcpyAsync(b.io, W0 + (size_t)p0 * wsz, sizeof(double) * wsz * Bc, hipMemcpyHostToDevice, c->stream));
     HIPCHK(hipMemcpyAsync(b.io + wsz * Bc, H0 + (size_t)p0 * hsz, sizeof(double) * hsz * Bc, hipMemcpyHostToDevice, c->stream));
     for (int p = 0; p < Bc; ++p) {
-      launch_set_factor(c, false, b.io + wsz * p, prob(a.Wn[1], p), prob(a.WT[1], p), prob(a.WG[1], p));
-      launch_set_factor(c, true, b.io + wsz * Bc + hsz * p, prob(a.Hn[1], p), prob(a.HT[1], p), prob(a.HG[1], p));
+      launch_set_factor(c, false, b.io + wsz * p, prob(a.Wn[1], p), prob(a.WT[1], p), prob(a.WS[1], p));
+      launch_set_factor(c, true, b.io + wsz * Bc + hsz * p, prob(a.Hn[1], p), prob(a.HT[1], p), prob(a.HS[1], p));
     }
     HIPCHK(hipGetLastError());
     HIPCHK(hipMemset2DAsync(b.slab + L.off_control, L.stride, 0, L.control, (size_t)Bc, c->stream));
@@ -1908,14 +1905,14 @@
       HIPCHK(hipStreamSynchronize(c->stream));
       struct Lend {
         nbmf_ctx* c;
-        double *Wn, *WT, *WG, *Hn, *HT, *HG, alpha, beta;
+        double *Wn, *WT, *WS, *Hn, *HT, *HS, alpha, beta;
         ~Lend() {
-          c->Wn = Wn; c->WT = WT; c->WG = WG; c->Hn = Hn; c->HT = HT; c->HG = HG;
+          c->Wn = Wn; c->WT = WT; c->WS = WS; c->Hn = Hn; c->HT = HT; c->HS = HS;
           c->alpha = alpha; c->beta = beta;
         }
-      } lend{c, c->Wn, c->WT, c->WG, c->Hn, c->HT, c->HG, c->alpha, c->beta};
-      c->Wn = prob(a.Wn[par], ps); c->WT = prob(a.WT[par], ps); c->WG = prob(a.WG[par], ps);
-      c->Hn = prob(a.Hn[par], ps); c->HT = prob(a.HT[par], ps); c->HG = prob(a.HG[par], ps);
+      } lend{c, c->Wn, c->WT, c->WS, c->Hn, c->HT, c->HS, c->alpha, c->beta};
+      c->Wn = prob(a.Wn[par], ps); c->WT = prob(a.WT[par], ps); c->WS = prob(a.WS[par], ps);
+      c->Hn = prob(a.Hn[par], ps); c->HT = prob(a.HT[par], ps); c->HS = prob(a.HS[par], ps);
       c->alpha = alpha[p0 + ps];
       c->beta = beta[p0 + ps];
       bool ok = true;
@@ -2314,10 +2311,10 @@
   const size_t fw = (size_t)c->KP * c->mA * sizeof(double), fh = (size_t)c->KP * c->nA * sizeof(double);
   HIPCHK(dmalloc(&c->Wn, fw));
   HIPCHK(dmalloc(&c->WT, fw + PASS_SLACK));
-  HIPCHK(dmalloc(&c->WG, fw + PASS_SLACK));
+  HIPCHK(dmalloc(&c->WS, fw + PASS_SLACK));
   HIPCHK(dmalloc(&c->Hn, fh));
   HIPCHK(dmalloc(&c->HT, fh + PASS_SLACK));
-  HIPCHK(dmalloc(&c->HG, fh + PASS_SLACK));
+  HIPCHK(dmalloc(&c->HS, fh + PASS_SLACK));
   HIPCHK(dmalloc(&c->Pbuf, 2 * fh + 64));
   c->n_prior_blocks = (int)(((size_t)c->KP * c->nA + 255) / 256);
   HIPCHK(dmalloc(&c->prior, sizeof(double) * 2 * (size_t)c->n_prior_blocks));
@@ -2344,7 +2341,7 @@
   comm_release(c);
   if (c->host_buf) hipHostFree(c->host_buf);
   arena_release((ArenaSlot*)c->arena_slot.p);
-  void* ptrs[] = {c->dataA, c->dataB, c->maskA, c->maskB, c->rowcnt, c->Wn, c->WT, c->WG, c->Hn, c->HT, c->HG,
+  void* ptrs[] = {c->dataA, c->dataB, c->maskA, c->maskB, c->rowcnt, c->Wn, c->WT, c->WS, c->Hn, c->HT, c->HS,
                   c->slabH, c->slabW, c->Pbuf, c->lossbuf, c->lossfin, c->prior, c->scal, c->flags, c->losses_d, c->stage, c->stats,
                   c->sbuf, c->Qbuf, c->cstartH, c->cstartW, c->theta, c->small.slab, c->small_batch.slab, c->small_batch.table,
                   c->small_batch.io, c->bitsA, c->bitsB, c->eval.rows, c->eval.cols, c->eval.x, c->eval.Wk, c->eval.Hk,
@@ -2718,11 +2715,11 @@
   if (!c || !W || !H) return fail(NBMF_ERR_ARG, "null argument");
   if (int rc = set_device(c)) return rc;
   HIPCHK(hipMemcpyAsync(c->stage, W, sizeof(double) * (size_t)c->k * c->m, hipMemcpyHostToDevice, c->stream));
-  launch_set_factor(c, false, c->stage, c->Wn, c->WT, c->WG);
+  launch_set_factor(c, false, c->stage, c->Wn, c->WT, c->WS);
   HIPCHK(hipGetLastError());
   HIPCHK(hipStreamSynchronize(c->stream));
   HIPCHK(hipMemcpyAsync(c->stage, H, sizeof(double) * (size_t)c->k * c->n, hipMemcpyHostToDevice, c->stream));
-  launch_set_factor(c, true, c->stage, c->Hn, c->HT, c->HG);
+  launch_set_factor(c, true, c->stage, c->Hn, c->HT, c->HS);
   HIPCHK(hipGetLastError());
   hipLaunchKernelGGL(prior_kernel, dim3(c->n_prior_blocks), dim3(256), 0, c->stream, c->Hn, c->prior, c->k, c->KP,
                      (long long)c->n, (long long)c->nA, c->eps);
diff --git a/nbmf_mm_amd/csrc/nbmf_operand_image.inc b/nbmf_mm_amd/csrc/nbmf_operand_image.inc
--- /dev/null
+++ b/nbmf_mm_amd/csrc/nbmf_operand_image.inc
@@ -0,0 +1,14 @@
+#include <cstddef>
+#if defined(__HIPCC__)
+#define NBMF_HD __host__ __device__ __forceinline__
+#else
+#define NBMF_HD inline
+#endif
+
+NBMF_HD size_t t_index(long long k, long long x, int KS, long long lenA) {
+  return (size_t)(k / KS) * KS * lenA + (size_t)((x >> 4) * KS + (k % KS)) * 16 + (x & 15);
+}
+NBMF_HD int s_sigma(long long k) { return (int)((4 * ((k >> 2) & 3)) ^ (k & 3)); }
+NBMF_HD size_t s_index(long long k, long long x, int KS, long long lenA) {
+  return (size_t)(k / KS) * KS * lenA + (size_t)((x >> 4) * KS + (k % KS)) * 16 + ((x & 15) ^ s_sigma(k % KS));
+}
diff --git a/nbmf_mm_amd/csrc/nbmf_pass_kernel.inc b/nbmf_mm_amd/csrc/nbmf_pass_kernel.inc
--- a/nbmf_mm_amd/csrc/nbmf_pass_kernel.inc
+++ b/nbmf_mm_amd/csrc/nbmf_pass_kernel.inc
@@ -22,7 +22,7 @@
 typedef const __attribute__((address_space(1))) uint32_t glb_u32;
 template <int PPW>
 __device__ __forceinline__ void dma_run(glb_char* g, lds_char* l) {
-  static_assert(PPW == 2 || PPW == 4, "2 KiB or 4 KiB per wave and image");
+  static_assert(PPW == 2 || PPW == 4, "2 KiB or 4 KiB per wave and stage");
   __builtin_amdgcn_global_load_lds(g, l, 16, 0, 0);
   __builtin_amdgcn_global_load_lds(g, l, 16, 1024, 0);
   if (PPW == 4) {
@@ -59,8 +59,7 @@
   const void* data;
   const void* mask;
   const double2* ltab_g;
-  const double* LT;
-  const double* LG;
+  const double* LS;
   const double* RfT;
   double* out1;
   double* out2;
@@ -84,8 +83,12 @@
 };
 
 constexpr int pass_log_bits(int KB) { return KB == 8 ? 8 : 10; }
+constexpr int pass_nb(int KB, int DATA, int MODE) {
+  return KB >= 8 ? 1 : (KB == 4 ? ((DATA != DATA_BIN && MODE == MODE_W) ? 1 : 2) : (KB == 2 ? 2 : 4));
+}
+constexpr int pass_stage_bytes(int KB, int DATA, int MODE) { return pass_nb(KB, DATA, MODE) * 16 * KB * 16 * 8; }
 constexpr int pass_lds_bytes(int KB, int DATA, int MODE) {
-  return (KB <= 4 ? STAGE_BYTES : 2 * STAGE_BYTES) + ((DATA != DATA_BIN && MODE != MODE_W && MODE != MODE_T) ? (16 << pass_log_bits(KB)) : 0);
+  return 2 * pass_stage_bytes(KB, DATA, MODE) + ((DATA != DATA_BIN && MODE != MODE_W && MODE != MODE_T) ? (16 << pass_log_bits(KB)) : 0);
 }
 constexpr int pass_wgs_per_cu(int KB, int DATA, int MODE) {
   if (KB == 8) return (MODE == MODE_H && DATA != DATA_BIN) ? 1 : 2;
@@ -103,10 +106,10 @@
   constexpr bool PRODUCTS = (MODE == MODE_H || MODE == MODE_W);
   constexpr int K = 16 * KB;
   constexpr int S = K / 4;
-  constexpr int NB = (KB >= 4) ? 1 : 4 / KB;
+  constexpr int NB = pass_nb(KB, DATA, MODE);
   constexpr int BLK = K * 16;
-  constexpr int STAGE_D = 2 * NB * BLK;
-  constexpr int N2 = NB * BLK / 2;
+  constexpr int STAGE_D = NB * BLK;
+  static_assert(STAGE_D * 8 == pass_stage_bytes(KB, DATA, MODE) && STAGE_D * 8 <= STAGE_BYTES, "the host's stage size");
   extern __shared__ __attribute__((aligned(16))) double lds[];
 
   [[maybe_unused]] unsigned long long tr0 = 0, tr1 = 0, tr2 = 0, trc = 0;
@@ -176,34 +179,30 @@
   d4 tnext[NB];
   [[maybe_unused]] d4 ybuf[2], mbuf[2];
   unsigned lane16 = (unsigned)lane * 16u;
-  constexpr int PPW = N2 * 16 / WG_WAVES / 1024;
+  constexpr int PPW = STAGE_D * 8 / WG_WAVES / 1024;
   constexpr bool ILV = PPW == 2;
-  constexpr int PW_BYTES = ILV ? 1024 : N2 * 16 / WG_WAVES;
+  constexpr int PW_BYTES = ILV ? 1024 : STAGE_D * 8 / WG_WAVES;
+  constexpr bool STREAMED = TH != 1 || PRODUCTS;
   [[maybe_unused]] unsigned lane16b = (unsigned)lane * 16u + 4096u;
-  constexpr unsigned long long STRIDE_TG = (unsigned long long)NB * BLK * 8;
+  constexpr unsigned long long STRIDE_S = (unsigned long long)STAGE_D * 8;
   auto scalar64 = [](unsigned long long v) {
     return ((unsigned long long)(unsigned)__builtin_amdgcn_readfirstlane((int)(v >> 32)) << 32) |
            (unsigned long long)(unsigned)__builtin_amdgcn_readfirstlane((int)(unsigned)v);
   };
-  unsigned long long pT = scalar64((unsigned long long)(a.LT + (size_t)rb0 * BLK) + (unsigned long long)wave * PW_BYTES);
-  unsigned long long pG = scalar64((unsigned long long)(a.LG + (size_t)rb0 * BLK) + (unsigned long long)wave * PW_BYTES);
+  unsigned long long pS = scalar64((unsigned long long)(a.LS + (size_t)rb0 * BLK) + (unsigned long long)wave * PW_BYTES);
 #define STAGE_DMA(RB, BUF)                                                                         \
   {                                                                                                \
-    lds_char* lT_ = (lds_char*)(lds + (BUF) * STAGE_D) + wave * PW_BYTES;                          \
+    lds_char* lS_ = (lds_char*)(lds + (BUF) * STAGE_D) + wave * PW_BYTES;                          \
      \
      \
      \
-    __asm__ volatile("" : "+s"(pT), "+s"(pG));                                                     \
+    __asm__ volatile("" : "+s"(pS));                                                               \
     __asm__ volatile("" : "+v"(lane16));                                                           \
     if (ILV) __asm__ volatile("" : "+v"(lane16b));                                                 \
     const unsigned l16_ = lane16;                                                                  \
-    if (TH != 1) {                                   \
-      if (ILV) dma_pair_interleaved((glb_char*)pT, l16_, lane16b, lT_);                            \
-      else dma_run<PPW>((glb_char*)pT + l16_, lT_);                                                \
-    }                                                                                              \
-    if (PRODUCTS) {                              \
-      if (ILV) dma_pair_interleaved((glb_char*)pG, l16_, lane16b, lT_ + N2 * 16);                  \
-      else dma_run<PPW>((glb_char*)pG + l16_, lT_ + N2 * 16);                                      \
+    if (STREAMED) {                                                                                \
+      if (ILV) dma_pair_interleaved((glb_char*)pS, l16_, lane16b, lS_);                            \
+      else dma_run<PPW>((glb_char*)pS + l16_, lS_);                                                \
     }                                                                                              \
     if (TH != 0 || MODE == MODE_T) {                                                               \
       if (th_in) {                                                                                 \
@@ -211,6 +210,21 @@
       }                                                                                            \
     }                                                                                              \
   }
+  constexpr bool XOR_AT_USE = KB == 8 && DATA == DATA_BIN && MODE == MODE_H;
+  [[maybe_unused]] unsigned tb[4], gb[4];
+#pragma unroll
+  for (int j = 0; j < 4; ++j) {
+    tb[j] = 8u * (unsigned)(((lane >> 4) * 16 + ((lane & 15) ^ (lane >> 4))) ^ (4 * j));
+    gb[j] = 8u * (unsigned)(((lane & 15) * 16 + ((lane >> 4) ^ (4 * ((lane >> 2) & 3)) ^ (lane & 3))) ^ (4 * j));
+  }
+  auto lane_base = [](const unsigned (&bases)[4], int j) {
+    if (!XOR_AT_USE || j == 0) return bases[j];
+    unsigned t;
+    __asm__ volatile("v_xor_b32 %0, %1, %2" : "=v"(t) : "s"(32u * (unsigned)j), "v"(bases[0]));
+    return t;
+  };
+#define FRAG_T(BLKP, S_) (*(const double*)((const char*)(BLKP) + (S_) * 512 + lane_base(tb, (S_) & 3)))
+#define FRAG_G(BLKP, KB_, R_) (*(const double*)((const char*)(BLKP) + (KB_) * 2048 + lane_base(gb, (R_))))
 
   d4 tcurT[NB];
   if (DATA != DATA_BIN && MODE != MODE_T) {
@@ -279,8 +293,7 @@
       pf_val = *(glb_u32*)((glb_char*)pPF + lane4);
       pPF += 64ull * NB;
     }
-    pT += STRIDE_TG;
-    pG += STRIDE_TG;
+    pS += STRIDE_S;
     STAGE_DMA(min(rb + NB, a.Rb - NB), buf ^ 1);
     __builtin_amdgcn_sched_barrier(0);
     const double* base = lds + buf * STAGE_D;
@@ -294,7 +307,7 @@
     double tcur[GT];
     if (TH != 1) {
 #pragma unroll
-      for (int i = 0; i < GT; ++i) tcur[i] = base[i * 64 + lane];
+      for (int i = 0; i < GT; ++i) tcur[i] = FRAG_T(base, i);
     }
 
 #pragma unroll
@@ -307,8 +320,7 @@
       [[maybe_unused]] d4& ynx = ybuf[LM_ALT ? (lm_i ^ 1) : 1];
       [[maybe_unused]] d4& mcur = mbuf[LM_ALT ? lm_i : 0];
       [[maybe_unused]] d4& mnx = mbuf[LM_ALT ? (lm_i ^ 1) : 1];
-      const double* ldsT = base + b * BLK;
-      const double* ldsG = base + NB * BLK + b * BLK;
+      const double* ldsS = base + b * BLK;
 
       constexpr bool DUAL = KB == 8 && MODE == MODE_H && DATA != DATA_BIN;
       d4 th = EPSACC ? acc0q : d4{0, 0, 0, 0}, th2 = {0, 0, 0, 0};
@@ -331,7 +343,7 @@
         double tnxt[GT];
         if (g + 1 < NGT) {
 #pragma unroll
-          for (int i = 0; i < GT; ++i) tnxt[i] = ldsT[((g + 1) * GT + i) * 64 + lane];
+          for (int i = 0; i < GT; ++i) tnxt[i] = FRAG_T(ldsS, (g + 1) * GT + i);
           __builtin_amdgcn_sched_barrier(0);
         }
 #pragma unroll
@@ -359,7 +371,7 @@
         thp[(size_t)(rb + b) * 64] = th;
         if (b + 1 < NB) {
 #pragma unroll
-          for (int i = 0; i < GT; ++i) tcur[i] = base[(b + 1) * BLK + i * 64 + lane];
+          for (int i = 0; i < GT; ++i) tcur[i] = FRAG_T(base + (b + 1) * BLK, i);
         }
         continue;
       }
@@ -371,10 +383,10 @@
       double gcur[GB];
       if (PRODUCTS) {
 #pragma unroll
-        for (int i = 0; i < GB; ++i) gcur[i] = ldsG[((i % KB) * 4 + (i / KB)) * 64 + lane];
+        for (int i = 0; i < GB; ++i) gcur[i] = FRAG_G(ldsS, i % KB, i / KB);
       } else if (b + 1 < NB && TH != 1) {
 #pragma unroll
-        for (int i = 0; i < GT; ++i) tcur[i] = base[(b + 1) * BLK + i * 64 + lane];
+        for (int i = 0; i < GT; ++i) tcur[i] = FRAG_T(base + (b + 1) * BLK, i);
       }
       __builtin_amdgcn_sched_barrier(0);
 
@@ -680,12 +692,12 @@
 #pragma unroll
           for (int i = 0; i < GB; ++i) {
             const int p = (g + 1) * GB + i;
-            gnxt[i] = ldsG[((p % KB) * 4 + (p / KB)) * 64 + lane];
+            gnxt[i] = FRAG_G(ldsS, p % KB, p / KB);
           }
           __builtin_amdgcn_sched_barrier(0);
         } else if (b + 1 < NB && TH != 1) {
 #pragma unroll
-          for (int i = 0; i < GT; ++i) tcur[i] = base[(b + 1) * BLK + i * 64 + lane];
+          for (int i = 0; i < GT; ++i) tcur[i] = FRAG_T(base + (b + 1) * BLK, i);
           __builtin_amdgcn_sched_barrier(0);
         }
 #pragma unroll
@@ -720,6 +732,8 @@
     ((uint32_t*)a.out1)[lane] = pf_sink;
 
 #undef STAGE_DMA
+#undef FRAG_T
+#undef FRAG_G
 #undef MASKS_REQUEST
   if (a.trace) {
     tr2 = wall_clock64();
diff --git a/nbmf_mm_amd/csrc/nbmf_peer_kernels.inc b/nbmf_mm_amd/csrc/nbmf_peer_kernels.inc
--- a/nbmf_mm_amd/csrc/nbmf_peer_kernels.inc
+++ b/nbmf_mm_amd/csrc/nbmf_peer_kernels.inc
@@ -165,7 +165,7 @@
 
 __global__ __launch_bounds__(256) void peer_h_apply_kernel(PeerView pv, unsigned long long epoch, long long offHX,
                                                            double* __restrict__ Hn, double* __restrict__ HT,
-                                                           double* __restrict__ HG, int KP,
+                                                           double* __restrict__ HS, int KP,
                                                            int KS , long long nA,
                                                            long long c0, long long wp ,
                                                            int* stop_flags) {
@@ -177,7 +177,7 @@
     const double h = src[k * nA + j];
     Hn[k * nA + j] = h;
     HT[t_index(k, j, KS, nA)] = h;
-    HG[g_index(k, j, KS, nA)] = h;
+    HS[s_index(k, j, KS, nA)] = h;
   }
 }
 
diff --git a/nbmf_mm_amd/csrc/nbmf_small_kernel.inc b/nbmf_mm_amd/csrc/nbmf_small_kernel.inc
--- a/nbmf_mm_amd/csrc/nbmf_small_kernel.inc
+++ b/nbmf_mm_amd/csrc/nbmf_small_kernel.inc
@@ -3,8 +3,8 @@
   unsigned long long prob_stride;
   const double *am1s, *bm1s;
   const void *dataA, *maskA, *dataB, *maskB;
-  double *Wn[2], *WT[2], *WG[2];
-  double *Hn[2], *HT[2], *HG[2];
+  double *Wn[2], *WT[2], *WS[2];
+  double *Hn[2], *HT[2], *HS[2];
   const double* rowcnt;
   unsigned long long* sync;
   double* ll_part;
@@ -110,14 +110,15 @@
 }
 
 template <int KB, bool WITH_G>
-__device__ __forceinline__ void small_load(const double* __restrict__ LT, const double* __restrict__ LG, int rb, int lane,
+__device__ __forceinline__ void small_load(const double* __restrict__ LT, const double* __restrict__ LS, int rb, int lane,
                                            int n_components, double* lt, double* lg) {
   constexpr int S = 4 * KB;
 #pragma unroll
   for (int s = 0; s < S; ++s) lt[s] = (4 * s < n_components) ? ld_sc1(LT + ((size_t)rb * S + s) * 64 + lane) : 0.0;
   if (WITH_G) {
-#pragma unroll
-    for (int i = 0; i < 4 * KB; ++i) lg[i] = ld_sc1(LG + ((size_t)rb * KB * 4 + i) * 64 + lane);
+    const int lb = (lane & 15) * 16 + ((lane >> 4) ^ s_sigma(lane & 15));
+#pragma unroll
+    for (int i = 0; i < 4 * KB; ++i) lg[i] = ld_sc1(LS + ((size_t)rb * KB * 4 + (i & ~3)) * 64 + (lb ^ (4 * (i & 3))));
   }
 }
 
@@ -339,11 +340,11 @@
         double lt[S], lg[4 * KB];
         const size_t ti = ((size_t)sh * a.RbA + rb) * 64 + lane;
         if (last) {
-          small_load<KB, false>(PP(a.WT[p_cur]), PP(a.WG[p_cur]), rb, lane, a.K, lt, lg);
+          small_load<KB, false>(PP(a.WT[p_cur]), PP(a.WS[p_cur]), rb, lane, a.K, lt, lg);
           const SmallData dt = small_data<DATA>(a.dataA, a.maskA, ti);
           small_tile<KB, DATA, MODE_L>(a, lt, lg, rf, dt, ltab, acc1, acc2, s2, prod, pexp, llsum, t2min);
         } else {
-          small_load<KB, true>(PP(a.WT[p_cur]), PP(a.WG[p_cur]), rb, lane, a.K, lt, lg);
+          small_load<KB, true>(PP(a.WT[p_cur]), PP(a.WS[p_cur]), rb, lane, a.K, lt, lg);
           const SmallData dt = small_data<DATA>(a.dataA, a.maskA, ti);
           small_tile<KB, DATA, MODE_H>(a, lt, lg, rf, dt, ltab, acc1, acc2, s2, prod, pexp, llsum, t2min);
         }
@@ -430,7 +431,7 @@
             ownH[k * 16 + cc] = h;
             st_sc1(PP(a.Hn[p_new]) + (size_t)k * a.nA + j, h);
             st_sc1(PP(a.HT[p_new]) + ((size_t)sh * K + k) * 16 + cc, h);
-            st_sc1(PP(a.HG[p_new]) + (size_t)sh * K * 16 + (k >> 4) * 256 + cc * 16 + (k & 15), h);
+            st_sc1(PP(a.HS[p_new]) + ((size_t)sh * K + k) * 16 + (cc ^ s_sigma(k)), h);
           }
           if (SM_COLD(dbg)) SM_MARK(13);
           const double pr = wave_sum_fast(__builtin_fma(am1, la, bm1 * lb));
@@ -468,7 +469,7 @@
       for (int rb = pw + PW * wave; rb < a.Cbe; rb += PW * SM_WAVES) {
         double lt[S], lg[4 * KB];
         const size_t ti = ((size_t)sw * a.CbA + rb) * 64 + lane;
-        small_load<KB, true>(PP(a.HT[p_new]), PP(a.HG[p_new]), rb, lane, a.K, lt, lg);
+        small_load<KB, true>(PP(a.HT[p_new]), PP(a.HS[p_new]), rb, lane, a.K, lt, lg);
         const SmallData dt = small_data<DATA>(a.dataB, a.maskB, ti);
         if (SM_COLD(dbg)) {
           SM_MARK(8);
@@ -580,7 +581,7 @@
           ownW[k * 16 + cc] = w;
           st_sc1(PP(a.Wn[p_new]) + (size_t)k * a.mA + i, w);
           st_sc1(PP(a.WT[p_new]) + ((size_t)sw * K + k) * 16 + cc, w);
-          st_sc1(PP(a.WG[p_new]) + (size_t)sw * K * 16 + (k >> 4) * 256 + cc * 16 + (k & 15), w);
+          st_sc1(PP(a.WS[p_new]) + ((size_t)sw * K + k) * 16 + (cc ^ s_sigma(k)), w);
         }
       }
     }
diff --git a/nbmf_mm_amd/csrc/nbmf_update_kernels.inc b/nbmf_mm_amd/csrc/nbmf_update_kernels.inc
--- a/nbmf_mm_amd/csrc/nbmf_update_kernels.inc
+++ b/nbmf_mm_amd/csrc/nbmf_update_kernels.inc
@@ -1,11 +1,5 @@
 
-__device__ __forceinline__ size_t t_index(long long k, long long x, int KS, long long lenA) {
-  return (size_t)(k / KS) * KS * lenA + (size_t)((x >> 4) * KS + (k % KS)) * 16 + (x & 15);
-}
-__device__ __forceinline__ size_t g_index(long long k, long long x, int KS, long long lenA) {
-  const long long kk = k % KS;
-  return (size_t)(k / KS) * KS * lenA + (size_t)(x >> 4) * KS * 16 + (kk >> 4) * 256 + (x & 15) * 16 + (kk & 15);
-}
+#include "nbmf_operand_image.inc"
 
 __device__ __forceinline__ double ordered_sum256(const double* __restrict__ p, int n, int stride, double* sh4) {
   double s = 0.0;
@@ -103,7 +97,7 @@
 __global__ __launch_bounds__(256) void h_update_kernel(const double* __restrict__ src1, const double* __restrict__ src2,
                                                        int chunks, size_t chunk_stride, long long src_ld, long long src_c0,
                                                        long long c0, long long wp, double* __restrict__ Hn,
-                                                       double* __restrict__ HT, double* __restrict__ HG,
+                                                       double* __restrict__ HT, double* __restrict__ HS,
                                                        double* __restrict__ prior, int K, int KP, long long n,
                                                        long long nA, double am1, double bm1, double eps, const int* done,
                                                        double pform ) {
@@ -136,7 +130,7 @@
     Hn[nat] = h;
     const long long jb = j >> 4, c = j & 15;
     HT[(jb * KP + k) * 16 + c] = h;
-    HG[jb * KP * 16 + (k >> 4) * 256 + c * 16 + (k & 15)] = h;
+    HS[(jb * KP + k) * 16 + (c ^ s_sigma(k))] = h;
   }
   block_sum2(la, lb, prior + 2 * (size_t)blockIdx.x);
 }
@@ -217,7 +211,7 @@
 constexpr int WU_COLS = 32;
 template <int WU_GROUPS>
 __global__ __launch_bounds__(WU_COLS * WU_GROUPS) void w_update_kernel(const double* __restrict__ slab, int chunks, double* __restrict__ Wn,
-                                                       double* __restrict__ WT, double* __restrict__ WG, int K, int KP,
+                                                       double* __restrict__ WT, double* __restrict__ WS, int K, int KP,
                                                        int KS , long long m,
                                                        long long mA, double n_div,
                                                        const double* __restrict__ rowcnt, int projection,
@@ -281,19 +275,19 @@
     }
     Wn[(size_t)k * mA + i] = w;
     WT[t_index(k, i, KS, mA)] = w;
-    WG[g_index(k, i, KS, mA)] = w;
+    WS[s_index(k, i, KS, mA)] = w;
   }
 }
 
 __global__ void set_factor_kernel(const double* __restrict__ src, double* __restrict__ Fn, double* __restrict__ FT,
-                                  double* __restrict__ FG, int K, int KP, int KS, long long len, long long lenA) {
+                                  double* __restrict__ FS, int K, int KP, int KS, long long len, long long lenA) {
   const long long idx = (long long)blockIdx.x * blockDim.x + threadIdx.x;
   if (idx >= (long long)KP * lenA) return;
   const long long k = idx / lenA, x = idx % lenA;
   const double v = (k < K && x < len) ? src[k * len + x] : 0.0;
   Fn[idx] = v;
   FT[t_index(k, x, KS, lenA)] = v;
-  FG[g_index(k, x, KS, lenA)] = v;
+  FS[s_index(k, x, KS, lenA)] = v;
 }
 
 __global__ void factor_range_kernel(const double* __restrict__ Wn, const double* __restrict__ Hn, int K, long long m,
```
